# dkogan/libdogleg

Measured on AMD Instinct MI355X. Metric: trust-region steps/sec (fp64) at fixed (Nmeas,Nstate,nnz), higher is better.
Workload: dtype f64

## Files before the change

### include/dlg_backend.h

```cpp
#ifndef DLG_BACKEND_H
#define DLG_BACKEND_H

#include <stddef.h>

#ifdef __cplusplus
extern "C" {
#endif

typedef struct dlg_backend dlg_backend_t;

enum
{
  DLG_OK           = 0,
  DLG_ERR_HIP      = 1,
  DLG_ERR_ARG      = 2,
  DLG_ERR_STATE    = 3,
  DLG_ERR_NOMEM    = 4,
  DLG_ERR_NODEVICE = 5,
  DLG_ERR_COMM     = 6
};

enum { DLG_DENSE = 0, DLG_SPARSE = 1, DLG_DENSE_PRODUCTS = 2 };
enum { DLG_FLAG_JTJ_PACKED = 1, DLG_FLAG_JTJ_UPPER = 2 };
enum { DLG_KIND_CAUCHY_TO_EDGE = 0, DLG_KIND_GAUSSNEWTON = 1, DLG_KIND_INTERPOLATED = 2 };
// ... 15 lines not shown

typedef int (*dlg_allreduce_fn)(void* buf, size_t count, void* cookie);
int  dlg_backend_set_shard(dlg_backend_t* b, int row0, int row1,
                           dlg_allreduce_fn fn, void* cookie);
int  dlg_backend_set_allreduce(dlg_backend_t* b, dlg_allreduce_fn fn, void* cookie);
int  dlg_backend_set_partition(dlg_backend_t* b, int rank, int nranks);
int  dlg_partition_rows(dlg_backend_t* b, int* nrows, const int** rows);
int  dlg_point_gather_device(dlg_backend_t* b, int slot, const double* x_full_dev, const double* J_full_dev,
                             const int* colptr_host);
int  dlg_partition_stats(dlg_backend_t* b, long* stats, int nstats);
int  dlg_sparse_partition_probe(int N, int M, const int* colptr, const int* rowidx, int rank, int nranks,
                                long* stats, int nstats, char* row_owner);
int  dlg_rccl_unique_id(void* out128);
int  dlg_backend_init_rccl(dlg_backend_t* b, int rank, int nranks, const void* unique_id128);
int  dlg_backend_set_rccl(dlg_backend_t* b, void* nccl_comm);
int  dlg_backend_share_rccl(dlg_backend_t* b, dlg_backend_t* owner);
int  dlg_backend_comm_size(dlg_backend_t* b, int* nranks);
int  dlg_backend_has_rccl(dlg_backend_t* b);
int  dlg_backend_set_noop_comm(dlg_backend_t* b, int on);

int  dlg_run_steps(dlg_backend_t* b, int from, int to, int nsteps, int ncopy, const double* const* x_dev,
                   const double* const* J_dev, int first_copy, double trustregion, double lambda0,
                   double* out9, int* kind_out);

int  dlg_backend_reset(dlg_backend_t* b);
int  dlg_backend_device(dlg_backend_t* b);
int  dlg_sparse_pattern_matches(dlg_backend_t* b, const int* colptr, const int* rowidx);
int  dlg_sparse_drop_pattern(dlg_backend_t* b);

int  dlg_sparse_set_pattern(dlg_backend_t* b, const int* colptr, const int* rowidx);
int  dlg_sparse_stats(dlg_backend_t* b, long* nnz_JtJ_lower, long* nnz_L,
                      int* n_supernodes, int* n_levels, double* factor_flops);

int  dlg_sparse_region_probe(int N, int M, const int* colptr, const int* rowidx, int ncu, long* stats, int nstats);

int  dlg_sparse_schedule(dlg_backend_t* b, int* n_levels, int* persist_level0, int* persist_items);

int  dlg_sparse_symbolic_probe(int N, int M, const int* colptr, const int* rowidx, int row0,
                               int row1, long* stats, int nstats, int* perm_out);

int  dlg_point_set_p(dlg_backend_t* b, int slot, const double* p_host);
int  dlg_point_upload(dlg_backend_t* b, int slot, const double* x_host,
                      const double* J_host);
int  dlg_point_upload_products(dlg_backend_t* b, int slot, double norm2x,
                               const double* Jtx_host, const double* JtJ_host);
int  dlg_point_bind_device(dlg_backend_t* b, int slot, const double* x_dev,
                           const double* J_dev);
int  dlg_point_eval(dlg_backend_t* b, int slot, double* norm2_x, double* Jtx_absmax);
int  dlg_backend_set_speculation(dlg_backend_t* b, int on);
typedef void (*dlg_between_fn)(void* cookie);
int  dlg_backend_set_between(dlg_backend_t* b, dlg_between_fn fn, void* cookie);
int  dlg_backend_between_redone(dlg_backend_t* b);
int  dlg_point_eval_early(dlg_backend_t* b, int slot, const double* x_dev, const double* J_dev, int* done);
int  dlg_backend_set_defer_tail(dlg_backend_t* b, int on);
int  dlg_step_tail_pending(dlg_backend_t* b);
int  dlg_backend_ei_source(dlg_backend_t* b, int* from_solved_system, double* pivot_ratio);
int  dlg_step_tail(dlg_backend_t* b, double* expected_improvement);
int  dlg_backend_time_allreduce(dlg_backend_t* b, size_t count, int iters, double* us_each);

int  dlg_cauchy(dlg_backend_t* b, int slot, double* norm2_updateCauchy);

int  dlg_factorize(dlg_backend_t* b, int slot, double lambda, int* ok);

int  dlg_solve_gn(dlg_backend_t* b, int slot, double* norm2_updateGN);

int  dlg_gauss_newton(dlg_backend_t* b, int slot, double* lambda_io, double* norm2_updateGN);
// ... 92 lines not shown
```

### libdogleg_amd/capi.py

```python
import ctypes as C
import os
import numpy as np

from .ctypes_defs import (Parameters2, CholmodSparse, Trace, TraceBuffer, BatchResult, JacobianReport, JacobianEntry,
                          CB_SPARSE, CB_DENSE, CB_PRODUCTS, dptr, iptr)

HERE = os.path.dirname(os.path.abspath(__file__))
LIB_PATH = os.environ.get("DLG_TEST_LIB") or os.path.join(HERE, "libdogleg_amd.so")

DLG_OK = 0
DLG_DENSE, DLG_SPARSE, DLG_DENSE_PRODUCTS = 0, 1, 2
FLAG_PACKED, FLAG_UPPER = 1, 2
KIND_CAUCHY, KIND_GN, KIND_INTERP = 0, 1, 2
VEC_P, VEC_X, VEC_JTX, VEC_CAUCHY, VEC_GN, VEC_STEP, VEC_J, VEC_X_OWN, VEC_J_OWN = range(9)

ALLREDUCE_FN = C.CFUNCTYPE(C.c_int, C.c_void_p, C.c_size_t, C.c_void_p)

BACKEND_SYMBOLS = [
    "dlg_last_error", "dlg_device_count", "dlg_backend_create", "dlg_backend_destroy",
    "dlg_backend_set_stream", "dlg_backend_get_stream", "dlg_backend_set_shard",
    "dlg_sparse_set_pattern", "dlg_sparse_stats", "dlg_sparse_schedule", "dlg_point_set_p", "dlg_point_upload",
    "dlg_point_upload_products", "dlg_point_bind_device", "dlg_point_eval", "dlg_cauchy",
    "dlg_factorize", "dlg_solve_gn", "dlg_gauss_newton", "dlg_cauchy_gauss_newton", "dlg_make_step",
    "dlg_expected_improvement", "dlg_step", "dlg_take_step", "dlg_solve_with_factor",
    "dlg_point_download", "dlg_factor_download_dense", "dlg_point_device_ptr",
    "dlg_kernel_syrk_lower", "dlg_kernel_potrf_lower", "dlg_probe_mfma_f64", "dlg_probe_mfma_f64_clock", "dlg_probe_mfma_f64_waves",
    "dlg_probe_hbm_copy", "dlg_set_trace", "dlg_mem_alloc", "dlg_mem_free", "dlg_host_alloc",
    "dlg_host_free", "dlg_mem_upload",
    "dlg_mem_download", "dlg_mem_zero", "dlg_device_sync", "dlg_sparse_symbolic_probe",
    "dlg_backend_set_profiling", "dlg_backend_get_profile", "dlg_backend_get_profile_early",
    "dlg_backend_set_allreduce", "dlg_backend_set_partition", "dlg_partition_rows", "dlg_partition_stats",
    "dlg_sparse_partition_probe", "dlg_rccl_unique_id", "dlg_backend_init_rccl", "dlg_backend_set_rccl",
    "dlg_backend_comm_size", "dlg_backend_has_rccl", "dlg_backend_set_noop_comm", "dlg_solve_multi", "dlg_pseudoinverse_chunk", "dlg_backend_set_speculation", "dlg_backend_set_defer_tail", "dlg_step_tail",
    "dlg_step_tail_pending", "dlg_backend_ei_source", "dlg_backend_set_between", "dlg_backend_between_redone", "dlg_point_eval_early",
    "dlg_backend_share_rccl", "dlg_point_gather_device", "dlg_backend_reset", "dlg_backend_device",
    "dlg_sparse_pattern_matches", "dlg_sparse_drop_pattern", "dlg_sparse_region_probe", "dlg_run_steps", "dlg_backend_time_allreduce",
    "dlg_feature_leverage", "dlg_outlierness_factors", "dlg_leverage_query", "dlg_leverage_stats",
    "dlg_covariance_blocks", "dlg_marginal_variances", "dlg_covariance_stats", "dlg_covariance_plan_seconds",
    "dlg_covariance_plan_probe", "dlg_covariance_entries", "dlg_covariance_entries_stats", "dlg_covariance_entries_probe",
    "dlg_query_covariance", "dlg_query_covariance_stats", "dlg_query_covariance_plan_seconds", "dlg_query_covariance_plan_probe",
]
PROF_NAMES = ["K1_jtx", "K3K8_norm2Jv", "K4_kernel", "K4_total", "K5_factor", "K6_solve", "K7_step", "vec"]
DOGLEG_SYMBOLS = [
    "dogleg_getDefaultParameters", "dogleg_setMaxIterations",
    "dogleg_setTrustregionUpdateParameters", "dogleg_setDebug", "dogleg_setInitialTrustregion",
    "dogleg_setThresholds", "dogleg_optimize", "dogleg_optimize2", "dogleg_optimize_dense",
    "dogleg_optimize_dense2", "dogleg_optimize_dense_products", "dogleg_computeJtJfactorization",
    "dogleg_freeContext", "dogleg_testGradient", "dogleg_testGradient_dense",
    "dogleg_testGradient_dense_products",
    "dogleg_optimize_device2", "dogleg_amd_backend", "dogleg_amd_point_slot",
    "dogleg_amd_set_communicator", "dogleg_amd_set_allreduce", "dogleg_amd_clear_communicator",
    "dogleg_amd_rccl_unique_id", "dogleg_amd_rank", "dogleg_amd_release_cache",
    "dogleg_amd_id_file_publish", "dogleg_amd_id_file_wait", "dogleg_amd_last_solve_timing",
    "dogleg_getOutliernessFactors", "dogleg_markOutliers", "dogleg_reportOutliers",
    "dogleg_getOutliernessTrace_newFeature_sparse",
    "dogleg_amd_covariance_blocks", "dogleg_amd_marginal_variances", "dogleg_amd_covariance_entries",
    "dogleg_amd_query_covariance",
    "dogleg_amd_optimize_dense_batch", "dogleg_amd_batch_last_stats",
    "dogleg_amd_dense_batch_uncertainty", "dogleg_amd_batch_uncertainty_last_stats",
    "dogleg_amd_jacobian_colouring", "dogleg_amd_check_jacobian_device", "dogleg_amd_check_jacobian_device_batch",
    "dogleg_amd_testGradient_device", "dogleg_amd_check_jacobian_last_stats",
]

_lib = None


class DlgError(RuntimeError):
    pass


def lib():
    global _lib
    if _lib is not None:
# ... 99 lines not shown
    L.dogleg_getDefaultParameters.restype = None
    L.dogleg_optimize2.restype = C.c_double
    L.dogleg_optimize2.argtypes = [D, C.c_uint, C.c_uint, C.c_uint, V, V, PP, V]
    L.dogleg_optimize.restype = C.c_double
    L.dogleg_optimize.argtypes = [D, C.c_uint, C.c_uint, C.c_uint, V, V, V]
    L.dogleg_optimize_dense2.restype = C.c_double
    L.dogleg_optimize_dense2.argtypes = [D, C.c_uint, C.c_uint, V, V, PP, V]
    L.dogleg_optimize_dense.restype = C.c_double
    L.dogleg_optimize_dense.argtypes = [D, C.c_uint, C.c_uint, V, V, V]
    L.dogleg_optimize_dense_products.restype = C.c_double
    L.dogleg_optimize_dense_products.argtypes = [D, C.c_uint, V, V, PP, V]
    L.dogleg_freeContext.argtypes = [V]
    L.dogleg_freeContext.restype = None
    L.dogleg_optimize_device2.restype = C.c_double
    L.dogleg_optimize_device2.argtypes = [D, C.c_uint, C.c_uint, C.c_uint, I, I, V, V, PP, V]
    L.dogleg_amd_backend.restype = V
    L.dogleg_amd_backend.argtypes = [V]
    L.dogleg_amd_point_slot.restype = C.c_int
    L.dogleg_amd_point_slot.argtypes = [V, V]
    L.dogleg_amd_set_communicator.argtypes = [C.c_int, C.c_int, C.c_int, V]
    L.dogleg_amd_set_allreduce.argtypes = [C.c_int, C.c_int, C.c_int, V, V]
    L.dogleg_amd_clear_communicator.restype = None
    L.dogleg_amd_rccl_unique_id.argtypes = [V]
    L.dogleg_amd_rank.argtypes = [V, I]
    L.dogleg_amd_id_file_publish.argtypes = [C.c_char_p, V, C.c_char_p]
    L.dogleg_amd_id_file_wait.argtypes = [C.c_char_p, V, C.c_char_p, C.c_int]
    L.dlg_backend_share_rccl.argtypes = [V, V]
    L.dlg_sparse_region_probe.argtypes = [C.c_int, C.c_int, I, I, C.c_int, C.POINTER(C.c_long), C.c_int]
    L.dlg_run_steps.argtypes = [V, C.c_int, C.c_int, C.c_int, C.c_int, C.POINTER(V), C.POINTER(V), C.c_int, C.c_double, C.c_double, D, I]
    L.dlg_backend_reset.argtypes = [V]
    L.dlg_backend_device.argtypes = [V]
    L.dlg_sparse_pattern_matches.argtypes = [V, I, I]
    L.dlg_sparse_drop_pattern.argtypes = [V]
    L.dogleg_amd_release_cache.restype = None
    if hasattr(L, "dogleg_amd_optimize_dense_batch"):
        L.dogleg_amd_optimize_dense_batch.argtypes = [D, C.c_uint, C.c_uint, C.c_uint, V, V, PP, C.POINTER(BatchResult)]
        L.dogleg_amd_batch_last_stats.argtypes = [D, C.c_int]
    if hasattr(L, "dogleg_amd_dense_batch_uncertainty"):
        L.dogleg_amd_dense_batch_uncertainty.argtypes = [D, C.c_uint, C.c_uint, C.c_uint, V, V, D, D, D, D, D, C.c_int, I]
        L.dogleg_amd_batch_uncertainty_last_stats.argtypes = [D, C.c_int]
    if hasattr(L, "dogleg_amd_check_jacobian_device"):
        JR, JE = C.POINTER(JacobianReport), C.POINTER(JacobianEntry)
        L.dogleg_amd_jacobian_colouring.argtypes = [C.c_uint, C.c_uint, I, I, I]
        L.dogleg_amd_check_jacobian_device.argtypes = [D, C.c_uint, C.c_uint, C.c_uint, I, I, V, V, C.c_double, C.c_double,
                                                       C.c_double, C.c_int, JR, D, JE, C.c_int]
        L.dogleg_amd_check_jacobian_device_batch.argtypes = [D, C.c_uint, C.c_uint, C.c_uint, V, V, C.c_double, C.c_double,
                                                             C.c_double, JR, JE, C.c_int, C.POINTER(C.c_longlong)]
        L.dogleg_amd_testGradient_device.argtypes = [C.c_uint, D, C.c_uint, C.c_uint, C.c_uint, I, I, V, V]
        L.dogleg_amd_testGradient_device.restype = None
        L.dogleg_amd_check_jacobian_last_stats.argtypes = [D, C.c_int]
    L.dogleg_amd_last_solve_timing.argtypes = [D, I]
    L.dlg_point_gather_device.argtypes = [V, C.c_int, V, V, I]
    L.dogleg_setMaxIterations.argtypes = [C.c_int]
    L.dogleg_setDebug.argtypes = [C.c_int]
    L.dogleg_setInitialTrustregion.argtypes = [C.c_double]
    L.dogleg_setThresholds.argtypes = [C.c_double, C.c_double, C.c_double]
    L.dogleg_setTrustregionUpdateParameters.argtypes = [C.c_double] * 4
    _lib = L
    return L


def _ck(rc, what=""):
    if rc != DLG_OK:
        raise DlgError(f"{what} failed (code {rc}): {lib().dlg_last_error().decode()}")


# ... 165 lines not shown

def symbolic_probe(N, M, Jp, Ji, row0=0, row1=None, want_perm=False):
    L = lib()
    Jp = np.ascontiguousarray(Jp, dtype=np.int32)
    Ji = np.ascontiguousarray(Ji, dtype=np.int32)
    st = (C.c_long * len(SYM_STAT_NAMES))()
    perm = np.zeros(N, dtype=np.int32) if want_perm else None
    _ck(L.dlg_sparse_symbolic_probe(N, M, iptr(Jp), iptr(Ji), row0, M if row1 is None else row1,
                                    st, len(SYM_STAT_NAMES), iptr(perm) if want_perm else None),
        "symbolic probe")
    d = {k: st[i] for i, k in enumerate(SYM_STAT_NAMES)}
    return (d, perm) if want_perm else d


PART_STAT_NAMES = ["cut_level", "supernodes_above_cut", "supernodes_mine", "rows_mine", "reduced_doubles",
                   "panel_doubles", "nnz_mine"]


def partition_probe(N, M, Jp, Ji, rank, nranks):
    L = lib()
    Jp = np.ascontiguousarray(Jp, dtype=np.int32)
    Ji = np.ascontiguousarray(Ji, dtype=np.int32)
    st = (C.c_long * len(PART_STAT_NAMES))()
    own = np.zeros(M, dtype=np.uint8)
    _ck(L.dlg_sparse_partition_probe(N, M, iptr(Jp), iptr(Ji), rank, nranks, st, len(PART_STAT_NAMES),
                                     own.ctypes.data_as(C.c_char_p)), "partition probe")
    return {k: st[i] for i, k in enumerate(PART_STAT_NAMES)}, own.astype(bool)


REGION_STAT_NAMES = ["level0", "supernodes", "workgroups", "lds_bytes", "sliced_workgroups", "hbm_update_matrices",
                     "schedule_hash", "level_params_hash"]


def region_probe(N, M, Jp, Ji, ncu=256):
    L = lib()
    Jp = np.ascontiguousarray(Jp, dtype=np.int32)
    Ji = np.ascontiguousarray(Ji, dtype=np.int32)
    st = (C.c_long * len(REGION_STAT_NAMES))()
    _ck(L.dlg_sparse_region_probe(N, M, iptr(Jp), iptr(Ji), ncu, st, len(REGION_STAT_NAMES)), "region probe")
    return {k: (st[i] & (2**64 - 1) if k.endswith("_hash") else st[i]) for i, k in enumerate(REGION_STAT_NAMES)}


def rccl_unique_id():
    buf = (C.c_char * 128)()
    _ck(lib().dlg_rccl_unique_id(C.cast(buf, C.c_void_p)), "rccl_unique_id")
    return bytes(buf)


class DeviceArray:

    def __init__(self, arr=None, nbytes=None, dtype=np.float64):
        L = lib()
        if arr is not None:
            arr = np.ascontiguousarray(arr)
            nbytes, dtype = arr.nbytes, arr.dtype
        self.nbytes, self.dtype = nbytes, np.dtype(dtype)
        self.ptr = L.dlg_mem_alloc(nbytes)
        if not self.ptr:
            raise DlgError(L.dlg_last_error().decode())
        if arr is not None:
            _ck(L.dlg_mem_upload(self.ptr, arr.ctypes.data, nbytes), "upload")
        else:
            _ck(L.dlg_mem_zero(self.ptr, nbytes), "memset")

    def numpy(self, shape=None):
        out = np.zeros(self.nbytes // self.dtype.itemsize, dtype=self.dtype)
# ... 99 lines not shown
        rows = C.POINTER(C.c_int)()
        _ck(self.L.dlg_partition_rows(self.h, C.byref(n), C.byref(rows)), "partition_rows")
        return np.ctypeslib.as_array(rows, shape=(n.value,)).copy() if n.value else np.zeros(0, dtype=np.int32)

    def partition_stats(self):
        st = (C.c_long * len(PART_STAT_NAMES))()
        _ck(self.L.dlg_partition_stats(self.h, st, len(PART_STAT_NAMES)), "partition_stats")
        return {k: st[i] for i, k in enumerate(PART_STAT_NAMES)}

    def init_rccl(self, rank, nranks, unique_id):
        buf = C.create_string_buffer(unique_id, 128)
        _ck(self.L.dlg_backend_init_rccl(self.h, rank, nranks, C.cast(buf, C.c_void_p)), "init_rccl")

    def set_noop_comm(self, on=True):
        _ck(self.L.dlg_backend_set_noop_comm(self.h, 1 if on else 0), "set_noop_comm")

    def comm_size(self):
        n = C.c_int()
        _ck(self.L.dlg_backend_comm_size(self.h, C.byref(n)), "comm_size")
        return n.value

    def set_pattern(self, Jp, Ji):
        Jp = np.ascontiguousarray(Jp, dtype=np.int32)
        Ji = np.ascontiguousarray(Ji, dtype=np.int32)
        _ck(self.L.dlg_sparse_set_pattern(self.h, iptr(Jp), iptr(Ji)), "set_pattern")

    def stats(self):
        a, b = C.c_long(), C.c_long()
        c, d = C.c_int(), C.c_int()
        e = C.c_double()
        _ck(self.L.dlg_sparse_stats(self.h, C.byref(a), C.byref(b), C.byref(c), C.byref(d), C.byref(e)),
            "stats")
        return dict(nnz_JtJ_lower=a.value, nnz_L=b.value, n_supernodes=c.value, n_levels=d.value,
                    factor_flops=e.value)

    def schedule(self):
        a, b, c = C.c_int(), C.c_int(), C.c_int()
        _ck(self.L.dlg_sparse_schedule(self.h, C.byref(a), C.byref(b), C.byref(c)), "schedule")
        return dict(n_levels=a.value, persist_level0=b.value, persist_items=c.value)

    def set_p(self, slot, p):
        p = np.ascontiguousarray(p, dtype=np.float64)
        _ck(self.L.dlg_point_set_p(self.h, slot, dptr(p)), "set_p")

    def upload(self, slot, x, J):
        x = np.ascontiguousarray(x, dtype=np.float64)
        J = np.ascontiguousarray(J, dtype=np.float64)
        self._keep = [x, J]
        _ck(self.L.dlg_point_upload(self.h, slot, dptr(x), dptr(J)), "upload")

    def upload_products(self, slot, norm2x, Jtx, JtJ):
        Jtx = np.ascontiguousarray(Jtx, dtype=np.float64)
        JtJ = np.ascontiguousarray(JtJ, dtype=np.float64)
        self._keep = [Jtx, JtJ]
        _ck(self.L.dlg_point_upload_products(self.h, slot, norm2x, dptr(Jtx), dptr(JtJ)), "upload")

    def bind_device(self, slot, x_ptr, J_ptr):
        _ck(self.L.dlg_point_bind_device(self.h, slot, C.c_void_p(x_ptr), C.c_void_p(J_ptr)), "bind")

    def eval(self, slot):
        a, b = C.c_double(), C.c_double()
        _ck(self.L.dlg_point_eval(self.h, slot, C.byref(a), C.byref(b)), "eval")
        return a.value, b.value

    def cauchy(self, slot):
        a = C.c_double()
        _ck(self.L.dlg_cauchy(self.h, slot, C.byref(a)), "cauchy")
# ... 204 lines not shown
```

### libdogleg_amd/csrc/panel_factor.h

```cpp
#pragma once
#include <hip/hip_runtime.h>

#ifndef DLG_PF_STAMP
#define DLG_PF_DECL
#define DLG_PF_STAMP(i)
#define DLG_PF_PIN(x)
#define DLG_PF_DONE
#endif
#ifndef DLG_PF_EVT
#define DLG_PF_EVT(J, e)
#endif
#ifndef DLG_PF_WLOG
#define DLG_PF_WLOG(J, t, e)
#endif

__device__ __forceinline__ double dlg_rsqrt(double d)
{
  double y = __builtin_amdgcn_rsq(d);
  y = y*(1.5 - 0.5*d*y*y);
  y = y*(1.5 - 0.5*d*y*y);
  return y;
}

typedef double dlg_pf_v4d __attribute__((ext_vector_type(4)));
// ... 976 lines not shown
      case 2: badcol = bd_factor_member<2>(P, ldp, c0, rdiag); break;
      case 3: badcol = bd_factor_member<3>(P, ldp, c0, rdiag); break;
      case 4: badcol = bd_factor_member<4>(P, ldp, c0, rdiag); break;
      case 5: badcol = bd_factor_member<5>(P, ldp, c0, rdiag); break;
      case 6: badcol = bd_factor_member<6>(P, ldp, c0, rdiag); break;
      case 7: badcol = bd_factor_member<7>(P, ldp, c0, rdiag); break;
      default: badcol = bd_factor_member<8>(P, ldp, c0, rdiag); break;
    }
    if(badcol >= 0) atomicMin(info, col0 + c0 + badcol);
  }
  __syncthreads();
  for(int r = w + tid; r < nrows; r += NT)
  {
    for(int m = 0; m < nmem; m++)
    {
      const int c0 = mcol[m], nb = mcol[m+1] - c0;
      switch(nb)
      {
        case 1: bd_solve_row<1>(P, ldp, r, c0, rdiag); break;
        case 2: bd_solve_row<2>(P, ldp, r, c0, rdiag); break;
        case 3: bd_solve_row<3>(P, ldp, r, c0, rdiag); break;
        case 4: bd_solve_row<4>(P, ldp, r, c0, rdiag); break;
        case 5: bd_solve_row<5>(P, ldp, r, c0, rdiag); break;
        case 6: bd_solve_row<6>(P, ldp, r, c0, rdiag); break;
        case 7: bd_solve_row<7>(P, ldp, r, c0, rdiag); break;
        default: bd_solve_row<8>(P, ldp, r, c0, rdiag); break;
      }
    }
  }
  __syncthreads();
}

template <int NB, int DS = 8>
__device__ __forceinline__ int bd_factor_member_g(double* __restrict__ G, int ldg, int c0, double* rdiag,
                                                  double* __restrict__ Dg)
{
  double D[NB][NB];
#pragma unroll
  for(int c = 0; c < NB; c++)
#pragma unroll
    for(int q = 0; q <= c; q++) D[c][q] = G[(c0 + c) + (size_t)(c0 + q)*ldg];
  int badcol = -1;
#pragma unroll
  for(int c = 0; c < NB; c++)
  {
    double d = D[c][c];
    if(!(d > 0.0)) { if(badcol < 0) badcol = c; d = 1.0; }
    const double inv = dlg_rsqrt(d);
    rdiag[c0 + c] = inv;
#pragma unroll
    for(int i = c + 1; i < NB; i++) D[i][c] *= inv;
#pragma unroll
    for(int j = c + 1; j < NB; j++)
#pragma unroll
      for(int i = j; i < NB; i++) D[i][j] -= D[i][c]*D[j][c];
    D[c][c] = d*inv;
  }
#pragma unroll
  for(int c = 0; c < NB; c++)
#pragma unroll
    for(int q = 0; q <= c; q++) { G[(c0 + c) + (size_t)(c0 + q)*ldg] = D[c][q]; if(q < DS) Dg[(c0 + c)*DS + q] = D[c][q]; }
  return badcol;
}
template <int NB, int DS = 8>
__device__ __forceinline__ void bd_solve_row_c(double* Pb, int ldp, int r, int c0, const double* rdiag,
                                               const double* __restrict__ Dg)
{
  double x[NB], Lm[NB][NB], rd[NB];
#pragma unroll
  for(int c = 0; c < NB; c++)
  {
    x[c] = Pb[r + (c0 + c)*ldp]; rd[c] = rdiag[c0 + c];
#pragma unroll
    for(int q = 0; q < c; q++) Lm[c][q] = Dg[(c0 + c)*DS + q];
  }
#pragma unroll
  for(int c = 0; c < NB; c++)
  {
    double v = x[c];
#pragma unroll
    for(int q = 0; q < c; q++) v -= x[q]*Lm[c][q];
    x[c] = v*rd[c];
  }
#pragma unroll
  for(int c = 0; c < NB; c++) Pb[r + (c0 + c)*ldp] = x[c];
}
template <int NT, int DS = 8>
__device__ __forceinline__ void bd_compact_members(double* __restrict__ G, int ldg, int w, int tid,
                                                   const int* __restrict__ mcol_g, int nmem, int bdw,
                                                   int* mcol, double* rdiag, double* __restrict__ Dg,
                                                   int* __restrict__ info, int col0)
{
  for(int m = tid; m <= nmem; m += NT) mcol[m] = (m < nmem) ? (bdw > 0 ? m*bdw : mcol_g[m]) : w;
  for(int m = tid; m < nmem; m += NT)
  {
    const int c0 = bdw > 0 ? m*bdw : mcol_g[m];
    const int nb = (m + 1 < nmem ? (bdw > 0 ? (m + 1)*bdw : mcol_g[m + 1]) : w) - c0;
    int badcol;
    switch(nb)
    {
      case 1: badcol = bd_factor_member_g<1, DS>(G, ldg, c0, rdiag, Dg); break;
      case 2: badcol = bd_factor_member_g<2, DS>(G, ldg, c0, rdiag, Dg); break;
      case 3: badcol = bd_factor_member_g<3, DS>(G, ldg, c0, rdiag, Dg); break;
      case 4: badcol = bd_factor_member_g<4, DS>(G, ldg, c0, rdiag, Dg); break;
      case 5: badcol = bd_factor_member_g<5, DS>(G, ldg, c0, rdiag, Dg); break;
      case 6: badcol = bd_factor_member_g<6, DS>(G, ldg, c0, rdiag, Dg); break;
      case 7: badcol = bd_factor_member_g<7, DS>(G, ldg, c0, rdiag, Dg); break;
      default: badcol = bd_factor_member_g<8, DS>(G, ldg, c0, rdiag, Dg); break;
    }
    if(badcol >= 0) atomicMin(info, col0 + c0 + badcol);
  }
}
template <int NT, int NB, int DS>
__device__ __forceinline__ void bd_compact_rows_flat(double* Pb, int ldp, int nr, int w, int tid, int nmem,
                                                     const double* rdiag, const double* __restrict__ Dg)
{
  const int q = NT / nr, rem = NT - q*nr;
  int m = tid / nr, r = tid - m*nr;
  while(m < nmem)
  {
    bd_solve_row_c<NB, DS>(Pb, ldp, w + r, m*NB, rdiag, Dg);
    r += rem; m += q;
    if(r >= nr) { r -= nr; m++; }
  }
}
template <int NT, int DS = 8>
__device__ __forceinline__ void bd_compact_rows(double* Pb, int ldp, int nrows, int w, int tid, int nmem,
                                                const int* mcol, const double* rdiag, const double* __restrict__ Dg, int bdw = 0)
{
#ifndef DLG_BD_ROWS_BY_THREAD
  if(bdw > 0 && bdw <= 4 && w == nmem*bdw && nrows > w)
  {
    const int nr = nrows - w;
    switch(bdw)
    {
      case 1: bd_compact_rows_flat<NT, 1, DS>(Pb, ldp, nr, w, tid, nmem, rdiag, Dg); break;
      case 2: bd_compact_rows_flat<NT, 2, DS>(Pb, ldp, nr, w, tid, nmem, rdiag, Dg); break;
      case 3: bd_compact_rows_flat<NT, 3, DS>(Pb, ldp, nr, w, tid, nmem, rdiag, Dg); break;
      default: bd_compact_rows_flat<NT, 4, DS>(Pb, ldp, nr, w, tid, nmem, rdiag, Dg); break;
    }
    __syncthreads();
// ... 25 lines not shown
```

### libdogleg_amd/csrc/sparse_factor.hip

```cpp
#include "sparse_internal.h"
#include "panel_factor.h"
#include "factor_tail.h"

namespace {
#ifdef DLG_FL_PROFILE
constexpr int FL_PROF_WG = 4096;
__device__ long long g_fl_prof[32*FL_PROF_WG*8];
__device__ long long g_fl_add[FL_PROF_WG*4];
#define FL_ADD_STAMP(k) do { if(HANDOFF && threadIdx.x == 0 && blockIdx.x < FL_PROF_WG) g_fl_add[blockIdx.x*4 + (k)] = wall_clock64(); } while(0)
#define FL_STAMP(k) do { if(threadIdx.x == 0 && blockIdx.x < FL_PROF_WG) g_fl_prof[((prof_lvl & 31)*FL_PROF_WG + blockIdx.x)*8 + (k)] = wall_clock64(); } while(0)
#else
#define FL_STAMP(k)
#define FL_ADD_STAMP(k)
#endif

template <int NT, bool UT_LDS, bool HANDOFF = false>
__device__ __forceinline__ void mf_add_children(double* P, double* Wt, int ntri, int nch, int ch0,
                                                MfChild rc, const MfChild* __restrict__ mf_rec,
                                                const double* uscr, const uint16_t* __restrict__ mf_dst, int tid,
                                                int* pr_flag = nullptr, int pr_epoch = 0, DlgHandoff ho = DlgHandoff{nullptr, 0, 0}, int z0 = 0)
{
  constexpr int MF_SLOTS = (NT >= 512) ? 20 : 16;
  const int lane = tid & 63;
  for(int e = z0 + tid; e < ntri; e += NT) Wt[e] = 0.0;
// ... 170 lines not shown
  FL_ADD_STAMP(1);
#ifdef DLG_FL_PROFILE
  if(threadIdx.x == 0 && blockIdx.x < FL_PROF_WG) g_fl_add[blockIdx.x*4 + 3] = 1000 + (bup ? 1 : 0) + 10*cnB + 100*(fl[0] == want);
#endif
  if(!bup) wait_flags(ciB, cnB);
  __syncthreads();
  FL_ADD_STAMP(2);
  if(!bup) load_child(WB, npB, bX, bY);
  add_half(dB, npB, 0, bX); add_half(dB, npB, H, bY);
  __syncthreads();
}

template <int NT, bool LEAF = false>
__global__ void __launch_bounds__(NT, LEAF ? 4 : 1) k_factor_level(const FwItem* __restrict__ items,
                                                     const MfChild* __restrict__ mf_rec,
                                                     const int* __restrict__ sn_bd_col,
                                                     const uint16_t* __restrict__ mf_dst,
                                                     double* __restrict__ Lx,
                                                     double* __restrict__ top_scr,
                                                     int* __restrict__ info,
                                                     double* uscr, int mode,
                                                     int* pr_flag, int pr_epoch, DlgHandoff ho, int64_t pr_acc)
{
  extern __shared__ __attribute__((aligned(16))) double P[];
  __shared__ int sbad, s_skip;
  constexpr int DS = LEAF ? 4 : 8;
  constexpr int CP_FLIGHT = LEAF ? 16 : 32;
#ifdef DLG_FL_PROFILE
  const int prof_lvl = mode >> 8;
  FL_STAMP(0);
#endif
  const bool stage_leaf_u = (mode & 4) != 0;
  const bool b16 = (mode & 16) != 0;
  mode &= 3;
  const FwItem it = items[blockIdx.x];
  const int r0 = it.r0, w = it.w, nrows = it.nrows;
  double* G = Lx + it.lx;
  const int tid = threadIdx.x, lane = tid & 63;
  const int nloc = w + (it.r1 - r0);
  const int shift = r0;
  const int64_t top = it.top;
  const int mb = nloc - w, ntri = mb*(mb + 1)/2;
  const bool cmp = it.nbd > 0 && top < 0;
  const int ldp = cmp ? ((mb + 1) & ~1) : ((nloc + 1) & ~1);
  double* Pb = cmp ? P - w : P;
  const int row0c = cmp ? w : 0;
  const bool has_u = mode != 0 && top < 0;
  const bool sliced = !LEAF && it.sliced != 0;
  const bool u_lds = has_u && (sliced || ((it.nch > 0 || stage_leaf_u) &&
                     (cmp ? (size_t)(ldp*w + ntri + 1 + DS*w)*sizeof(double) <= (size_t)FAC_LDS_BUDGET : it.jsp >= 0)));
  const int usp = (u_lds && !cmp && !sliced) ? it.jsp : mb;
  const int sl_pad = sliced ? (it.eA & 1) : 0;
  const int nlin = sliced ? it.eB - it.eA + sl_pad : usp*mb - usp*(usp - 1)/2;
  double* Ug = has_u ? uscr + it.u_off : nullptr;
  double* Us = P + ldp*w;
  const int ush = sliced ? sl_pad - it.eA : 0;
  double* Dg = Us + (u_lds ? nlin + 1 : 0);
  __shared__ int s_mcol[LEAF ? 68 : 260];
  __shared__ double s_rdiag[LEAF ? 64 : 256];
  MfChild rc = {0, 0, 0, 0};
  const bool mf_acc = !LEAF && mode == 2 && it.nch > 0;
  if(mf_acc) rc = mf_rec[it.ch0 + min(lane, it.nch - 1)];
  if(tid == 0) { sbad = 0x7fffffff; s_skip = __hip_atomic_load(info, __ATOMIC_RELAXED, __HIP_MEMORY_SCOPE_AGENT) != 0x7fffffff; }
  if(pr_flag && tid == 0 && blockIdx.x == gridDim.x - 1)
    __hip_atomic_store(pr_flag + gridDim.x, pr_epoch, __ATOMIC_RELAXED, __HIP_MEMORY_SCOPE_AGENT);
  if(cmp)
  {
    __syncthreads();
    if(s_skip)
    {
      if(pr_flag && tid == 0) __hip_atomic_store(pr_flag + blockIdx.x, pr_epoch, __ATOMIC_RELAXED, __HIP_MEMORY_SCOPE_AGENT);
      return;
    }
    bd_compact_members<NT, DS>(G, nrows, w, tid, sn_bd_col + it.bd0, it.nbd, it.bdw, s_mcol, s_rdiag, Dg, &sbad, it.col0);
  }
  const int cp_rows = min(NT, (nloc - row0c + 63) & ~63), cp_ng = NT/cp_rows, cp_g = tid/cp_rows;
#ifndef DLG_LEAF_NO_GLDS
  if((LEAF && cmp) || (!LEAF && !cmp && !sliced && shift == 0))
  {
    const int ntot = ldp*w;
    const double* g0 = cmp ? G + (w + shift) : G;
    for(int k = tid >> 6; 128*k < ntot; k += NT/64)
    {
      const int e = 128*k + 2*lane;
      if(e < ntot)
      {
        const int j = e / ldp, r = e - j*ldp;
        __builtin_amdgcn_global_load_lds((const __attribute__((address_space(1))) void*)(g0 + (size_t)j*nrows + r),
                                         (__attribute__((address_space(3))) void*)(P + 128*k), 16, 0, 0);
      }
    }
  }
  else
#endif
  {
  for(int i = row0c + tid - cp_g*cp_rows; i < nloc && cp_g < cp_ng; i += cp_rows)
  {
    const double* gp = G + (i < w ? i : i + shift);
    for(int j0 = cp_g; j0 < w; j0 += CP_FLIGHT*cp_ng)
    {
      double v[CP_FLIGHT];
#pragma unroll
      for(int u = 0; u < CP_FLIGHT; u++) v[u] = (j0 + u*cp_ng < w) ? gp[(size_t)(j0 + u*cp_ng)*nrows] : 0.0;
#pragma unroll
      for(int u = 0; u < CP_FLIGHT; u++) if(j0 + u*cp_ng < w) Pb[i + (j0 + u*cp_ng)*ldp] = v[u];
    }
  }
  }
  __syncthreads();
  FL_STAMP(1);
  const int nrep = (pr_flag && it.rsv2 > 1) ? it.rsv2 : 1;
  if(nrep > 1 && it.rep < nrep - 1 && tid == 0) __hip_atomic_store(pr_flag + blockIdx.x, -pr_epoch, __ATOMIC_RELAXED, __HIP_MEMORY_SCOPE_AGENT);
  if(s_skip)
  {
    if(pr_flag && tid == 0) __hip_atomic_store(pr_flag + blockIdx.x, pr_epoch, __ATOMIC_RELAXED, __HIP_MEMORY_SCOPE_AGENT);
    return;
  }
  if(mf_acc && usp < mb)
    for(int jw = usp + (tid >> 6); jw < mb; jw += NT/64)
      for(int i = lane; i < mb - jw; i += 64) P[(mb - jw)*ldp + i] = 0.0;
  if(mf_acc)
  {
    const bool two = NT >= 512 && it.nch == 2 && __builtin_amdgcn_readlane(rc.npad, 0) <= 20*NT && __builtin_amdgcn_readlane(rc.npad, 1) <= 20*NT &&
                     (__builtin_amdgcn_readlane(rc.rsv, 0) >> 20) <= 8 && (__builtin_amdgcn_readlane(rc.rsv, 1) >> 20) <= 8;
    if(pr_flag && u_lds && two) mf_add_two_pipelined<NT>(P, Us, nlin, rc, uscr, mf_dst, tid, pr_flag, pr_epoch, ho);
    else if(pr_flag && u_lds) mf_add_children<NT, true, true>(P, Us, nlin, it.nch, it.ch0, rc, mf_rec, uscr, mf_dst, tid, pr_flag, pr_epoch, ho);
    else if(pr_flag)     mf_add_children<NT, false, true>(P, Ug + pr_acc, (nrep > 1 && !sliced) ? it.eB : ntri, it.nch, it.ch0, rc, mf_rec, uscr, mf_dst, tid, pr_flag, pr_epoch, ho,
                                                          (nrep > 1 && !sliced) ? it.eA : 0);
    else if(u_lds)  mf_add_children<NT, true >(P, Us, nlin, it.nch, it.ch0, rc, mf_rec, uscr, mf_dst, tid);
    else            mf_add_children<NT, false>(P, Ug, ntri, it.nch, it.ch0, rc, mf_rec, uscr, mf_dst, tid);
  }
  FL_STAMP(2);
  if(cmp) bd_compact_rows<NT, DS>(Pb, ldp, nloc, w, tid, it.nbd, s_mcol, s_rdiag, Dg, it.bdw);
  else if(LEAF) { }
  else if(it.nbd > 0) panel_factor_blockdiag<NT>(P, ldp, nloc, w, tid, sn_bd_col + it.bd0, it.nbd, &sbad, it.col0, s_mcol, s_rdiag);
  else if(NT >= 256 && b16 && nloc <= 16*PF_B16_MAXT) panel_factor_b16<(NT >= 256 ? NT : 256)>(P, ldp, nloc, w, tid, &sbad, it.col0);
// ... 59 lines not shown
      for(int i = lane; i < mb - jw; i += 64)
      {
        if(pr_flag) __hip_atomic_store((gwptr_t)(dst + i), src[i], __ATOMIC_RELAXED, __HIP_MEMORY_SCOPE_AGENT);
        else dst[i] = src[i];
      }
    }
  }
  if(pr_flag)
  {
    asm volatile("s_waitcnt vmcnt(0)" ::: "memory");
    __syncthreads();
    if(tid == 0) __hip_atomic_store(pr_flag + blockIdx.x, pr_epoch, __ATOMIC_RELAXED, __HIP_MEMORY_SCOPE_AGENT);
  }
  FL_STAMP(7);
  const bool store_panel = it.rep == nrep - 1;
  if(nrep > 1 && store_panel)
  {
    if(tid < nrep - 1)
    {
      int spins = 0;
      for(;;)
      {
        const int v = __hip_atomic_load(pr_flag + ((int)blockIdx.x - (nrep - 1) + tid), __ATOMIC_RELAXED, __HIP_MEMORY_SCOPE_AGENT);
        if(v == pr_epoch || v == -pr_epoch) break;
        __builtin_amdgcn_s_sleep(1);
        if(++spins > ho.spins) { atomicOr(ho.status, DLG_HANDOFF_FACTOR); break; }
      }
    }
    __syncthreads();
  }
  for(int i = row0c + tid - cp_g*cp_rows; i < nloc && cp_g < cp_ng && store_panel; i += cp_rows)
  {
    double* gp; size_t gs;
    if(i >= w)        { gp = G + (i + shift); gs = (size_t)nrows; }
    else if(top < 0)  { gp = G + i; gs = (size_t)nrows; }
    else if(r0 == 0)  { gp = top_scr + top + i; gs = (size_t)w; }
    else continue;
    const int jend = (usp < mb && i < w) ? i + 1 : w;
    for(int j0 = cp_g; j0 < jend; j0 += 16*cp_ng)
    {
      double v[16];
#pragma unroll
      for(int u = 0; u < 16; u++) v[u] = (j0 + u*cp_ng < jend) ? Pb[i + (j0 + u*cp_ng)*ldp] : 0.0;
#pragma unroll
      for(int u = 0; u < 16; u++) if(j0 + u*cp_ng < jend) gp[(size_t)(j0 + u*cp_ng)*gs] = v[u];
    }
  }
  FL_STAMP(5);
#ifdef DLG_FL_PROFILE
  if(threadIdx.x == 0 && blockIdx.x < FL_PROF_WG)
    g_fl_prof[((prof_lvl & 31)*FL_PROF_WG + blockIdx.x)*8 + 6] = (long long)w | ((long long)nrows << 12) | ((long long)it.nch << 24) | ((long long)(u_lds ? 1 : 0) << 36) | ((long long)(has_u ? 1 : 0) << 37) | ((long long)(it.r1 - it.r0) << 40) | ((long long)(it.rep & 15) << 52) | ((long long)(it.pad & 63) << 56);
#endif
}
__global__ void __launch_bounds__(TPB) k_copy_top(const int* __restrict__ ms_sn, const int* __restrict__ sn_c0,
                                                  const int* __restrict__ sn_rowptr,
                                                  const int64_t* __restrict__ sn_lx,
                                                  const int64_t* __restrict__ sn_top,
                                                  double* __restrict__ Lx,
                                                  const double* __restrict__ top_scr, const int* __restrict__ info)
{
  if(*info != 0x7fffffff) return;
  const int s = ms_sn[blockIdx.x];
  const int w = sn_c0[s+1] - sn_c0[s];
  const int nrows = sn_rowptr[s+1] - sn_rowptr[s];
  double* G = Lx + sn_lx[s];
  const double* T = top_scr + sn_top[s];
  for(int e = threadIdx.x; e < w*w; e += TPB) { const int j = e / w, i = e - j*w; G[i + (size_t)j*nrows] = T[e]; }
// ... 590 lines not shown
    }
    if(nwg == 0) continue;
    for(int g = FL_PROF_WG - 1, shown = 0; g >= 0 && shown < (getenv("DLG_FL_DUMP_ALL") ? FL_PROF_WG : 20); g--)
    {
      const long long* q = &h[(l*FL_PROF_WG + g)*8];
      if(q[5] == 0 || q[7] == 0) continue;
      shown++;
      {
        std::vector<long long> ha(FL_PROF_WG*4);
        static bool got = false; static std::vector<long long> hadd;
        if(!got) { hadd.resize(FL_PROF_WG*4); hipMemcpyFromSymbol(hadd.data(), HIP_SYMBOL(g_fl_add), sizeof(long long)*hadd.size()); got = true; }
        if(hadd[g*4 + 0]) fprintf(stderr, "   add %3d: child0 seen %6lld child0 added %6lld last child seen %6lld dbg %lld\n", g, hadd[g*4] - t0, hadd[g*4 + 1] - t0, hadd[g*4 + 2] - t0, hadd[g*4 + 3]);
      }
      fprintf(stderr, "   wg %3d (w %3lld rows %4lld nch %lld u_lds %lld lvl %lld rep %lld): start %6lld flag up %6lld panel in %6lld added %6lld factored %6lld tail %6lld flag+stored %6lld\n",
              g, q[6] & 4095, (q[6] >> 12) & 4095, (q[6] >> 24) & 4095, (q[6] >> 36) & 1, (q[6] >> 56) & 63, (q[6] >> 52) & 15, q[0] - t0, q[7] - t0, q[1] - t0, q[2] - t0, q[3] - t0, q[4] - t0, q[5] - t0);
    }
    const long long* q = &h[(l*FL_PROF_WG + last)*8];
    fprintf(stderr, "level %2d: %3d wg, span %7lld | last wg %3d (w %3lld rows %4lld slice %4lld nch %2lld u_lds %lld has_u %lld): start +%6lld load %6lld add %6lld factor %6lld tail %6lld store %6lld | mean: load %6.0f add %6.0f factor %6.0f tail %6.0f store %6.0f\n",
            l, nwg, tend - t0, last, q[6] & 4095, (q[6] >> 12) & 4095, (q[6] >> 40) & 4095, (q[6] >> 24) & 4095, (q[6] >> 36) & 1, (q[6] >> 37) & 1,
            q[0] - t0, q[1] - q[0], q[2] - q[1], q[3] - q[2], q[4] - q[3], q[5] - q[4],
            mean[0]/nwg, mean[1]/nwg, mean[2]/nwg, mean[3]/nwg, mean[4]/nwg);
  }
  std::vector<long long> z(h.size(), 0);
  hipMemcpyToSymbol(HIP_SYMBOL(g_fl_prof), z.data(), sizeof(long long)*z.size());
}
#endif
int sparse_factor_levels(dlg_backend* b, int part)
{
  SparseSym* Y = b->sym;
  const SymHost& H = Y->H;
  hipStream_t st = b->stream;
  const bool split = Y->top.level0 > 0 && H.nlevels >= 2 && H.part_nranks <= 1 && H.fw_lvl_ptr[1] > H.fw_lvl_ptr[0];
  if(part == 2 && !split) return DLG_OK;
  if(part != 2)
  {
  if(H.part_nranks > 1 && H.cut_level < 0) DLG_CHECK(sparse_partition_reduce(b));
  if(Y->top.level0 == 0 || H.nlevels < 2) DLG_CHECK(sparse_fin_side_gate(b));
  }
  for(int l = 0; l < H.nlevels; l++)
  {
    const bool launched_before = part == 2 && l == 0;

    const int n = H.fw_lvl_ptr[l+1] - H.fw_lvl_ptr[l];
    const bool gate_here = (l == Y->top.level0 && Y->top.flag) || (l == Y->lo.level0 && Y->lo.flag);
    if(l > 0 && n < 256 && !gate_here) dlg_fork_point(b);
    if(l == Y->lo.level0 && Y->lo.flag)
    {
      PrRegion& R = Y->lo;
      ++R.epoch;
      if(l > 0 && n < 256) dlg_fork_gate(b, R.flag + R.nwg, R.epoch);
      {
        DlgRegionTurn turn(b);
        launch_region(b, R, l);
      }
      l = R.level1;
      if(H.part_nranks > 1 && l == H.cut_level) { DLG_LAUNCH_CHECK(); DLG_CHECK(sparse_partition_reduce(b)); }
      continue;
    }
    if(l == Y->top.level0)
    {
      PrRegion& R = Y->top;
      ++R.epoch;
      if(gate_here && l > 0) dlg_fork_gate(b, R.flag + R.nwg, R.epoch);
      DlgRegionTurn turn(b);
      launch_region(b, R, l);
      break;
    }
    if(n > 0 && !launched_before)
    {
      const int fmode = ((l >= H.mf_level0) ? 2 : Y->fac.syrk_fused[l]) + 4*Y->fac.stage[l] + FMODE_B16 + 256*(l & 31);
      launch_factor_level(Y->fac.nt[l], Y->fac.leaf[l], n, Y->fac.lds[l], st, Y, Y->fw_item + H.fw_lvl_ptr[l], Y->mf_rec, Y->mf_dst,
                          fmode, (int*)nullptr, 0, DlgHandoff{nullptr, 0, 0}, (int64_t)0);
    }
    if(part == 1 && split && l == 0) { Y->fac_pending = true; DLG_LAUNCH_CHECK(); return DLG_OK; }
    const int nu = H.uw_lvl_ptr[l+1] - H.uw_lvl_ptr[l];
    const bool gather_next = nu > 0 && H.upd_syrk[l] && Y->fac.upd_nw[l] > 0;
    const int fin_ep = (l == 0 && gather_next) ? Y->fin_side_owed : 0;
    if(fin_ep) Y->fin_side_owed = 0;
    if(l == 0) DLG_CHECK(sparse_fin_side_gate(b));
    if(gather_next)
    {
      const int ns = H.xl_ptr[l+1] - H.xl_ptr[l];
      if(Y->fac.syrk_fused[l] || ns == 0) {  }
      else if(Y->fac.syrk_nt[l] == 256)
        hipLaunchKernelGGL(HIP_KERNEL_NAME(k_update_syrk<256>), dim3(ns), dim3(256), Y->fac.syrk_lds[l], st,
                           Y->xl_sn + H.xl_ptr[l], Y->sn_c0, Y->sn_rowptr, Y->sn_lx, Y->u_off, Y->Lx, Y->uscr,
                           Y->fac.syrk_kc[l]);
      else
        hipLaunchKernelGGL(HIP_KERNEL_NAME(k_update_syrk<1024>), dim3(ns), dim3(1024), Y->fac.syrk_lds[l], st,
                           Y->xl_sn + H.xl_ptr[l], Y->sn_c0, Y->sn_rowptr, Y->sn_lx, Y->u_off, Y->Lx, Y->uscr,
                           Y->fac.syrk_kc[l]);
      hipLaunchKernelGGL(HIP_KERNEL_NAME(k_update_gather<TPB>), dim3(nu), dim3(TPB), Y->fac.upd_lds[l], st, H.uw_lvl_ptr[l],
                         Y->uw_flat, Y->usub, Y->usub_u, Y->relpos, Y->Lx, Y->upart, Y->uscr,
                         Y->fac.upd_nw[l], Y->d_info,
                         fin_ep ? (const int*)(Y->fin_flag + 1) : (const int*)nullptr, fin_ep,
                         reinterpret_cast<int*>(b->d_scal + (dlg_backend::NSCAL - 2)));
    }
    else if(nu > 0 && Y->fac.upd_coop[l] == 2)
      hipLaunchKernelGGL(k_update_mfma, dim3(nu), dim3(TPB), Y->fac.upd_lds[l], st, H.uw_lvl_ptr[l],
                         Y->uw_item, Y->uw_s0, Y->uw_s1, Y->uw_part, Y->ui_t, Y->ui_col, Y->ui_nc,
                         Y->usub, Y->relpos, Y->sn_rowptr, Y->sn_lx, Y->Lx, Y->upart, Y->fac.upd_nw[l], (const int*)Y->d_info);
    else if(nu > 0 && Y->fac.upd_coop[l])
      hipLaunchKernelGGL(k_update_coop, dim3(nu), dim3(TPB), 0, st, H.uw_lvl_ptr[l],
                         Y->uw_item, Y->uw_s0, Y->uw_s1, Y->uw_part, Y->ui_t, Y->ui_col, Y->ui_nc,
                         Y->usub, Y->relpos, Y->sn_rowptr, Y->sn_lx, Y->Lx, Y->upart, (const int*)Y->d_info);
    else if(nu > 0)
      hipLaunchKernelGGL(k_update_level, dim3(nu), dim3(TPB), Y->fac.upd_lds[l], st, H.uw_lvl_ptr[l],
                         Y->uw_item, Y->uw_s0, Y->uw_s1, Y->uw_part, Y->ui_t, Y->ui_col, Y->ui_nc,
                         Y->usub, Y->relpos, Y->sn_rowptr, Y->sn_lx, Y->Lx, Y->upart, Y->fac.upd_nw[l], (const int*)Y->d_info);
// ... 31 lines not shown
```

### libdogleg_amd/csrc/sparse_host.hip

```cpp
#include "sparse_internal.h"
#include <thread>
#include <mutex>
#include <memory>
#include <string>
#include <algorithm>
#include <cstring>
#include <chrono>

int sparse_create(dlg_backend* b) { (void)b; return DLG_OK; }

size_t sparse_local_nnz(const dlg_backend* b) { return b->sym ? b->sym->nnz_loc : (size_t)b->nnz; }

void sparse_destroy(dlg_backend* b)
{
  SparseSym* Y = b->sym;
  if(!Y) return;
  if(b->aux_stream) (void)hipStreamSynchronize(b->aux_stream);
  if(Y->ev_spec) (void)hipEventDestroy(Y->ev_spec);
  if(Y->ev_spec_fork) (void)hipEventDestroy(Y->ev_spec_fork);
  for(void* p : Y->allocs) if(p) (void)hipFree(p);
  sparse_leverage_free(Y);
  if(b->cov) { if(b->stream) (void)hipStreamSynchronize(b->stream); for(int i = 0; i < COV_NPLAN; i++) cov_plan_release(b->cov[i]); }
  b->cov_last = -1;
  selinv_release(b);
// ... 106 lines not shown
  {
    key = pattern_key(b, colptr, rowidx);
    Y->pat_key = key;
    std::lock_guard<std::mutex> lk(g_sym_mu);
    const SymCacheEntry* c = g_sym_cache.get();
    if(c && c->key == key && c->N == b->N && c->M == b->M && c->nnz == b->nnz && c->row0 == b->row0 && c->row1 == b->row1 &&
       c->part_rank == b->part_rank && c->part_nranks == b->part_nranks &&
       !memcmp(c->cp.data(), colptr, sizeof(int)*((size_t)b->M + 1)) && !memcmp(c->ri.data(), rowidx, sizeof(int)*(size_t)b->nnz))
    { Y->H = c->H; cached = true; }
  }
  if(!cached)
  {
    if(sym_analyze(Y->H, b->N, b->M, colptr, rowidx, b->row0, b->row1, err, sizeof(err), b->part_rank, b->part_nranks))
    { dlg_set_error("symbolic analysis: %s", err); return DLG_ERR_ARG; }
    if(use_cache)
    {
      std::unique_ptr<SymCacheEntry> e(new (std::nothrow) SymCacheEntry());
      if(e)
      {
        e->key = key; e->N = b->N; e->M = b->M; e->nnz = b->nnz; e->row0 = b->row0; e->row1 = b->row1;
        e->part_rank = b->part_rank; e->part_nranks = b->part_nranks;
        e->cp.assign(colptr, colptr + b->M + 1); e->ri.assign(rowidx, rowidx + b->nnz);
        e->H = Y->H;
        std::lock_guard<std::mutex> lk(g_sym_mu);
        g_sym_cache = std::move(e);
      }
    }
  }
  SymHost& H = Y->H;
  lap(cached ? "symbolic analysis (copied: same pattern as the last one)" : "symbolic analysis (host)");
  const bool partition = H.part_nranks > 1;
  if(partition) b->mloc = (int)H.part_rows.size();
  UP(sn_c0); UP(sn_rowptr); UP(sn_rows); UP(sn_scr); UP(lvl_sn); UP(sn_lx); UP(diagpos);
  UP(ui_t); UP(ui_col); UP(ui_nc); UP(ui_ptr); UP(usub); UP(relpos); UP(u_off); UP(usub_u); UP(fw_item); UP(mf_rec); UP(mf_dst);
  UP(uw_item); UP(uw_s0); UP(uw_s1); UP(uw_part); UP(uf_item); UP(uf_n); UP(uf_off);
  UP(oblk); UP(contrib); UP(jtx_task); UP(jtx_fin_ptr); UP(jtx_fin_blk);
  UP(asm_rho); UP(asm_pair); UP(asm_slot); UP(asm_batch); UP(asm_ctask); UP(asm_cfin);
  if(H.asm_jtx_ok)
  {
    UP(jf_ptr); UP(jf_ent); UP(jf_var0); UP(jf_w); UP(jf_short);
    {
      std::vector<int> rec(4*H.jf_long.size());
      for(size_t k = 0; k < H.jf_long.size(); k++)
      { const int v = H.jf_long[k]; rec[4*k] = H.jf_ptr[v]; rec[4*k+1] = H.jf_ptr[v+1]; rec[4*k+2] = H.jf_var0[v]; rec[4*k+3] = H.jf_w[v]; }
      DLG_CHECK(upload(Y->jf_long, rec)); Y->allocs.push_back(Y->jf_long);
      const size_t nl = std::max<size_t>(1, H.jf_long.size());
      DLG_HIP(hipMalloc(&Y->jf_lpart, sizeof(double)*16*JFL_SEG*nl)); Y->allocs.push_back(Y->jf_lpart);
      DLG_HIP(hipMalloc(&Y->jf_lcnt, sizeof(int)*nl)); Y->allocs.push_back(Y->jf_lcnt);
      DLG_HIP(hipMemset(Y->jf_lcnt, 0, sizeof(int)*nl));
    }
    DLG_HIP(hipMalloc(&Y->jtp, sizeof(double)*16*std::max<size_t>(1, H.asm_mtask.size()))); Y->allocs.push_back(Y->jtp);
  }
  UP(asm_shape); UP(asm_kg); UP(asm_mtask); UP(asm_tdest); UP(asm_fin2); UP(asm_fin2_list); UP(asm_run); UP(asm_pdest);
  {
    std::vector<uint32_t> pent(128*std::max<size_t>(1, H.asm_shape.size()), 0u);
    Y->asm_pent_ok = true;
    for(size_t q = 0; q < H.asm_shape.size(); q++)
    {
      const AsmShape& sh = H.asm_shape[q];
      std::vector<uint32_t> e;
      bool fits = true;
      auto word = [&](int kind, int mm, int n) {
        if(sh.pa[mm] > 15 || sh.pnI[mm] > 15 || sh.pslot[mm] > 15) fits = false;
        return (uint32_t)kind | (uint32_t)mm << 2 | (uint32_t)n << 6 | (uint32_t)(sh.pslot[mm] & 15) << 10 | (uint32_t)(sh.pa[mm] & 15) << 14 |
               (uint32_t)sh.paccoff[mm] << 18 | (uint32_t)(sh.pnI[mm] & 15) << 26 |
               (uint32_t)((sh.pslot[mm] == sh.dslot && sh.pa[mm] < n) ? 1u : 0u) << 30; };
// ... 30 lines not shown
      for(int s2 = 0; s2 < H.nsn; s2++)
      {
        const bool keep = H.sn_level[s2] == 0 && H.sn_bd_ptr[s2+1] > H.sn_bd_ptr[s2] && H.sn_top[s2] < 0 && H.nlevels >= 2;
        if(keep) { kept += H.sn_lx[s2+1] - H.sn_lx[s2]; continue; }
        if(!off.empty() && off.back() + len.back() == H.sn_lx[s2]) len.back() += H.sn_lx[s2+1] - H.sn_lx[s2];
        else { off.push_back(H.sn_lx[s2]); len.push_back(H.sn_lx[s2+1] - H.sn_lx[s2]); }
      }
      if(!off.empty() && off.back() + len.back() == H.lx_size) len.back() += 8;
      else { off.push_back(H.lx_size); len.push_back(8); }
      Y->n_clr = (int)off.size();
      Y->clr_partial_ok = kept*2 > H.lx_size && Y->n_clr <= 65535 && H.asm_cfin.empty() && H.asm_ctask.empty() && !getenv("DOGLEG_AMD_FULL_CLEAR");
      DLG_CHECK(upload(Y->clr_off, off)); Y->allocs.push_back(Y->clr_off);
      DLG_CHECK(upload(Y->clr_len, len)); Y->allocs.push_back(Y->clr_len);
    }
    {
      std::vector<int64_t> dp; std::vector<int> dc;
      for(int k = 0; k < H.N; k++) if(H.sn_level[H.col_sn[k]] == 0) { dp.push_back(H.diagpos[k]); dc.push_back(k); }
      Y->n_leaf_diag = (int)dp.size();
      if(Y->n_leaf_diag > 0)
      {
        DLG_CHECK(upload(Y->leaf_diag, dp)); Y->allocs.push_back(Y->leaf_diag);
        DLG_CHECK(upload(Y->leaf_diag_col, dc)); Y->allocs.push_back(Y->leaf_diag_col);
      }
    }
    DLG_HIP(hipMalloc(&Y->fin_flag, sizeof(int)*2)); Y->allocs.push_back(Y->fin_flag);
    DLG_HIP(hipMemsetAsync(Y->fin_flag, 0, sizeof(int)*2, b->stream));
  }
  UP(rl_ptr); UP(rl_pos); UP(perm); UP(col_sn); UP(sn_owner); UP(xl_sn); UP(fw_sn); UP(fw_r0); UP(fw_r1); UP(ms_sn); UP(sn_top); UP(sn_bd_ptr); UP(sn_bd_col);
  {
    std::vector<int64_t> ap((size_t)H.N);
    for(int k = 0; k < H.N; k++)
    {
      const int s2 = H.col_sn[k];
      const int64_t nrows = H.sn_rowptr[s2+1] - H.sn_rowptr[s2];
      ap[k] = H.sn_lx[s2] + (nrows - 1) + (int64_t)(k - H.sn_c0[s2])*nrows;
    }
    DLG_CHECK(upload(Y->augpos, ap)); Y->allocs.push_back(Y->augpos);
    std::vector<int64_t> av((size_t)H.N);
    for(int k = 0; k < H.N; k++) av[(size_t)H.perm[k]] = ap[k];
    std::vector<char> listed((size_t)H.N, 0);
    for(int pass = 0; pass < 2; pass++)
      for(int v : (pass ? H.jf_long : H.jf_short))
        for(int q = 0; q < H.jf_w[v]; q++) listed[(size_t)H.jf_var0[v] + q] = 1;
    DLG_CHECK(upload(Y->aug_of_var, av)); Y->allocs.push_back(Y->aug_of_var);
    DLG_CHECK(upload(Y->jf_listed, listed)); Y->allocs.push_back(Y->jf_listed);
  }
  {
    std::vector<int> fs, fl;
    for(int f = 0; f + 1 < (int)H.jtx_fin_ptr.size(); f++)
      (H.jtx_fin_ptr[f+1] - H.jtx_fin_ptr[f] > 256 ? fl : fs).push_back(f);
    Y->n_fin_short = (int)fs.size(); Y->n_fin_long = (int)fl.size();
    DLG_CHECK(upload(Y->jtx_fin_short, fs)); Y->allocs.push_back(Y->jtx_fin_short);
    DLG_CHECK(upload(Y->jtx_fin_long, fl)); Y->allocs.push_back(Y->jtx_fin_long);
  }
  {
    const int mloc = dlg_mloc(b);
    std::vector<int> jp(mloc + 1), ji;
    if(partition)
    {
      jp[0] = 0;
      for(int k = 0; k < mloc; k++) { const int r = H.part_rows[k]; jp[k+1] = jp[k] + (colptr[r+1] - colptr[r]); }
      ji.resize((size_t)jp[mloc]);
      for(int k = 0; k < mloc; k++) { const int r = H.part_rows[k]; memcpy(&ji[jp[k]], rowidx + colptr[r], sizeof(int)*(size_t)(colptr[r+1] - colptr[r])); }
      Y->nnz_loc = (size_t)jp[mloc];
    }
    else
    {
      const int q0 = colptr[b->row0], q1 = colptr[b->row1];
// ... 240 lines not shown
      (void)sparse_note_breakdown(b);
      b->factor_doomed = true;
      *ok = 0;
      return DLG_OK;
    }
  }
  DLG_CHECK(sparse_factor_levels(b, b->factor_ahead ? 1 : 0));
  if(pf.e) { dlg_prof_end(b, pf.id, pf.e); pf.e = nullptr; }
  if(b->defer_factor_sync) { *ok = 1; return DLG_OK; }
  DLG_HIP(hipMemcpyAsync(Y->h_info, Y->d_info, sizeof(int), hipMemcpyDeviceToHost, st));
  DLG_HIP(hipStreamSynchronize(st));
  *ok = sparse_factor_ok(b);
  return DLG_OK;
}
bool sparse_factor_pending(const dlg_backend* b) { return b->sym && b->sym->fac_pending; }
int sparse_norm2_chunks(const dlg_backend* b) { return b->sym ? b->sym->n_nv_chunks : 0; }
int sparse_factorize_rest(dlg_backend* b, bool* was_pending)
{
  SparseSym* Y = b->sym;
  *was_pending = Y && Y->fac_pending;
  if(!*was_pending) return DLG_OK;
  Y->fac_pending = false;
  b->prof_cont = true;
  struct Cont { dlg_backend* b; ~Cont() { b->prof_cont = false; } } cont{b};
  DlgProfScope pf(b, DLG_PROF_K5_FACTOR);
  return sparse_factor_levels(b, 2);
}
double sparse_current_lambda(const dlg_backend* b) { return b->sym ? b->sym->cur_lambda : 0.0; }
const double* sparse_pivot_minmax(const dlg_backend* b, int* n)
{
  *n = b->sym ? b->sym->n_diag_mm : 0;
  return (b->sym && b->sym->n_diag_mm > 0) ? b->sym->diag_mm : nullptr;
}
void sparse_hold_factor(dlg_backend* b)
{
  SparseSym* Y = b->sym;
  Y->held_Lx = Y->Lx; Y->held_aug = Y->aug_rhs; Y->held_lambda = Y->cur_lambda;
}
void sparse_release_held(dlg_backend* b) { if(b->sym) b->sym->held_Lx = nullptr; }
int sparse_restore_factor(dlg_backend* b, bool* restored, bool rearm)
{
  SparseSym* Y = b->sym;
  *restored = false;
  Y->fac_pending = false;
  if(!Y->held_Lx || Y->held_Lx != Y->Lx_spec) { Y->held_Lx = nullptr; return DLG_OK; }
  std::swap(Y->Lx, Y->Lx_spec);
  Y->spare_zeroed = false; Y->spare_dirty = true;
  Y->aug_rhs = Y->held_aug; Y->cur_lambda = Y->held_lambda; Y->held_Lx = nullptr;
  static const int k_armed = 0x7fffffff;
  if(rearm) DLG_HIP(hipMemcpyAsync(Y->d_info, &k_armed, sizeof(int), hipMemcpyHostToDevice, b->stream));
  Y->info_clean = false; Y->info_armed = false;
  *restored = true;
  return DLG_OK;
}
bool sparse_factor_ok(const dlg_backend* b) { return *b->sym->h_info == 0x7fffffff; }
namespace { __global__ void k_lower_word(int* word, int v) { if(threadIdx.x == 0) __hip_atomic_store(word, v, __ATOMIC_RELAXED, __HIP_MEMORY_SCOPE_AGENT); } }
int sparse_abandon_enqueued(dlg_backend* b)
{
  SparseSym* Y = b->sym;
  if(!Y || !Y->d_info || !b->copy_stream || !b->ev_copy) return DLG_OK;
  hipLaunchKernelGGL(k_lower_word, dim3(1), dim3(64), 0, b->copy_stream, Y->d_info, 0);
  DLG_LAUNCH_CHECK();
  DLG_HIP(hipEventRecord(b->ev_copy, b->copy_stream));
  DLG_HIP(hipStreamWaitEvent(b->stream, b->ev_copy, 0));
  hipLaunchKernelGGL(k_lower_word, dim3(1), dim3(64), 0, b->stream, Y->d_info, 0x7fffffff);
  DLG_LAUNCH_CHECK();
  Y->info_clean = false; Y->info_armed = false; Y->fac_pending = false;
  return DLG_OK;
}

extern "C" int dlg_sparse_symbolic_probe(int N, int M, const int* colptr, const int* rowidx, int row0,
                                         int row1, long* stats, int nstats, int* perm_out)
{
  SymHost H;
  char err[512];
  if(sym_analyze(H, N, M, colptr, rowidx, row0, row1, err, sizeof(err)))
  { dlg_set_error("symbolic analysis: %s", err); return DLG_ERR_ARG; }
  const long v[] = { (long)H.nvb, (long)H.nsn, (long)H.nlevels, (long)H.nnz_JtJ_lower, (long)H.nnz_L,
                     (long)H.lx_size, (long)H.factor_flops, (long)H.max_panel, (long)H.asm_ctask.size(),
                     (long)H.ui_t.size(), (long)H.relpos.size(), (long)H.oblk.size(),
                     (long)H.contrib.size(), (long)H.usub.size(), (long)H.scr_size,
                     (long)H.jtx_task.size(), (long)H.asm_mtask.size(), (long)H.asm_kg.size(),
                     (long)H.asm_shape.size() };
  if(getenv("DOGLEG_AMD_SYM_DEBUG"))
    for(int l = 0; l + 1 < (int)H.uw_lvl_ptr.size(); l++)
    {
      long nu = 0, direct = 0, part = 0, subs = 0;
      for(int u = H.uw_lvl_ptr[l]; u < H.uw_lvl_ptr[l+1]; u++)
      {
        const int item = H.uw_item[u], t = H.ui_t[item];
        const long slab = (long)(H.sn_rowptr[t+1] - H.sn_rowptr[t])*H.ui_nc[item];
        nu++; subs += H.uw_s1[u] - H.uw_s0[u];
        (H.uw_part[u] < 0 ? direct : part) += slab;
      }
      if(nu) fprintf(stderr, "update level %d: %ld units, %ld sub-tasks, slabs applied directly %ld doubles, partial slabs %ld doubles, U scratch %ld doubles, two-phase %d\n",
                     l, nu, subs, direct, part, (long)H.uscr_size, (int)H.upd_syrk[l]);
    }
  for(int i = 0; i < nstats && i < (int)(sizeof(v)/sizeof(v[0])); i++) stats[i] = v[i];
  if(perm_out) memcpy(perm_out, H.perm.data(), sizeof(int)*(size_t)N);
  return DLG_OK;
// ... 2 lines not shown
```

### libdogleg_amd/csrc/sparse_internal.h

```cpp
#pragma once
#include "dlg_internal.h"
#include "sparse_symbolic.h"
#include "sparse_region.h"

namespace {
constexpr int JFL_SEG = 16;
constexpr int NV_CHUNK = 2048;

constexpr int TPB = 256;
constexpr int LDS_BUDGET = SYM_LDS_BUDGET;
constexpr int FAC_LDS_BUDGET = SYM_FAC_LDS_BUDGET;

__device__ __forceinline__ double wave_sum(double v)
{
#pragma unroll
  for(int o = 32; o > 0; o >>= 1) v += __shfl_down(v, o, 64);
  return v;
}

template <int NT, int U, class LoadF, class StoreF>
__device__ __forceinline__ void batched_copy(int total, int tid, LoadF ld, StoreF st)
{
  for(int base = 0; base < total; base += U*NT)
  {
// ... 2 lines not shown
    for(int u = 0; u < U; u++) { const int idx = base + u*NT + tid; v[u] = (idx < total) ? ld(idx) : 0.0; }
#pragma unroll
    for(int u = 0; u < U; u++) { const int idx = base + u*NT + tid; if(idx < total) st(idx, v[u]); }
  }
}

template <class T> int upload(T*& dev, const std::vector<T>& h)
{
  dev = nullptr;
  const size_t bytes = sizeof(T)*(h.size() ? h.size() : 1);
  DLG_HIP(hipMalloc(&dev, bytes));
  if(!h.empty()) DLG_HIP(hipMemcpy(dev, h.data(), sizeof(T)*h.size(), hipMemcpyHostToDevice));
  return DLG_OK;
}

}

struct GatherUnit { int64_t lt, part; int s0, s1, nrows_t, nc; };
struct SolveItem { int c0, w, nrows, rowoff; int64_t lx; int bd0, nbd; int pflag, rsv; };

struct PrRegion
{
  int level0 = 1 << 30, level1 = -1, lds = 0, stage = 0, nwg = 0;
  FwItem* item = nullptr; MfChild* rec = nullptr; uint16_t* dst = nullptr;
  int* flag = nullptr; int epoch = 0;
};

struct SparseSym
{
  SymHost H;
  uint64_t pat_key = 0;
  int *sn_c0 = nullptr, *sn_rowptr = nullptr, *sn_rows = nullptr, *sn_scr = nullptr, *lvl_sn = nullptr;
  int64_t *sn_lx = nullptr, *diagpos = nullptr;
  int *ui_t = nullptr, *ui_col = nullptr, *ui_nc = nullptr, *ui_ptr = nullptr;
  SymSub* usub = nullptr; int* relpos = nullptr;
  int *uw_item = nullptr, *uw_s0 = nullptr, *uw_s1 = nullptr, *uf_item = nullptr, *uf_n = nullptr;
  int64_t *uw_part = nullptr, *uf_off = nullptr;
  GatherUnit* uw_flat = nullptr;
  double* upart = nullptr; double* uscr = nullptr; int64_t *u_off = nullptr, *usub_u = nullptr;
  SolveItem* slv_item = nullptr; FwItem* fw_item = nullptr; MfChild* mf_rec = nullptr; uint16_t* mf_dst = nullptr;
  SymOutBlock* oblk = nullptr; SymContrib* contrib = nullptr;
  SymTask *jtx_task = nullptr;
  int *jtx_fin_ptr = nullptr, *jtx_fin_blk = nullptr;
  int *jtx_fin_short = nullptr, *jtx_fin_long = nullptr; int n_fin_short = 0, n_fin_long = 0;
  AsmRho* asm_rho = nullptr; AsmPair* asm_pair = nullptr; AsmSlot* asm_slot = nullptr;
  AsmBatch* asm_batch = nullptr; AsmTask* asm_ctask = nullptr; AsmFin* asm_cfin = nullptr;
  bool asm_pent_ok = false;
  uint32_t* asm_pent = nullptr;
  AsmShape* asm_shape = nullptr; AsmKG* asm_kg = nullptr; AsmMTask* asm_mtask = nullptr; int* asm_tdest = nullptr;
  int *jf_ptr = nullptr, *jf_ent = nullptr, *jf_var0 = nullptr, *jf_w = nullptr, *jf_short = nullptr, *jf_long = nullptr;
  double* jf_lpart = nullptr; int* jf_lcnt = nullptr;
  const double* fin_pending_rhs = nullptr; const double* spec_aug_rhs = nullptr; bool info_clean = false;
  double* fin_pending_Lx = nullptr;
  bool spare_dirty = false, spare_zeroed = false; hipStream_t spare_stream = nullptr;
  double* jtp = nullptr;
  AsmFin2* asm_fin2 = nullptr; int64_t* asm_fin2_list = nullptr; AsmRun* asm_run = nullptr; int* asm_pdest = nullptr;
  int *rl_ptr = nullptr, *rl_pos = nullptr, *perm = nullptr, *col_sn = nullptr;
  int *fw_sn = nullptr, *fw_r0 = nullptr, *fw_r1 = nullptr, *ms_sn = nullptr; int64_t* sn_top = nullptr;
  int *sn_bd_ptr = nullptr, *sn_bd_col = nullptr;
  double* top_scr = nullptr;
  const double* aug_rhs = nullptr;
  int *Jp = nullptr, *Ji = nullptr;
  int *gat_rows = nullptr, *gat_src = nullptr;
  int *nv_chunk = nullptr; int n_nv_chunks = 0;
  double *Lx = nullptr, *scr = nullptr, *ywork = nullptr, *asm_part = nullptr, *jtx_part = nullptr;
  int *d_info = nullptr, *h_info = nullptr;
// ... 12 lines not shown
  int64_t* augpos = nullptr;
  int *xl_sn = nullptr;
  double* held_Lx = nullptr; const double* held_aug = nullptr; double held_lambda = 0.0;
  double cur_lambda = 0.0;
  double *ms_scr = nullptr, *ms_y = nullptr; int ms_lds_f = 0, ms_lds_b = 0;
  typedef ReachPlan LevPlan;
  LevPlan lev[2];
  int* lev_iperm = nullptr; std::vector<int> lev_jp, lev_ji; int lev_lds = 0;
  double* Lx_spec = nullptr; hipEvent_t ev_spec = nullptr, ev_spec_fork = nullptr;
  bool spec_inflight = false, spec_valid = false; int spec_slot = -1; const double* spec_J = nullptr;
  int64_t touch_off = 0, touch_n = 0;
  int bw_level0 = 1 << 30, bw_lds = 0, bw_n = 0;
  SolveItem* slv_item_pr = nullptr; int* bwd_flag = nullptr; int bwd_epoch = 0; double* bwd_xh = nullptr;
  PrRegion top, lo; double* pr_acc = nullptr;
  int64_t* clr_off = nullptr; int64_t* clr_len = nullptr; int n_clr = 0; bool clr_partial_ok = false; double* lz_ok[2] = {nullptr, nullptr};
  int64_t* aug_of_var = nullptr; char* jf_listed = nullptr;
  int aug_fused_epoch = 0; const double* spec_aug_fused = nullptr;
  int* fin_flag = nullptr; int fin_epoch = 0, fin_side_owed = 0; bool fin_side_sched_ok = false; hipStream_t fin_main = nullptr;
  int bwd_xb_cap = 12288;
  double* diag_mm = nullptr; int n_diag_mm = 0;
  std::vector<void*> allocs;
};

int sparse_assemble(dlg_backend* b, int s, double lambda);
int sparse_partition_reduce(dlg_backend* b);
int sparse_assemble_speculative(dlg_backend* b, int s);
int sparse_eval_assemble(dlg_backend* b, int s, int* done);
int sparse_assemble_finish(dlg_backend* b);
int sparse_zero_spare(dlg_backend* b, hipStream_t ordered_for);
void sparse_spec_invalidate(dlg_backend* b, int s);
int sparse_factor_setup(dlg_backend* b);
int sparse_factor_levels(dlg_backend* b, int part = 0);
int sparse_solve_setup(dlg_backend* b);
```

### libdogleg_amd/csrc/sparse_multi.hip

```cpp
#include "sparse_internal.h"
#include <algorithm>
#include <cfloat>
#include <cstdint>

namespace {
constexpr int MR = 16;
constexpr int MS_WMAX = 128;
typedef double ms_v4d __attribute__((ext_vector_type(4)));
__device__ __forceinline__ int tri(int i, int j) { return i*(i + 1)/2 + j; }

__device__ __forceinline__ void ms_stage_top(const double* __restrict__ L, int nrows, int w, double* Lt, double* dinv, int tid)
{
  for(int e = tid; e < w*w; e += TPB)
  {
    const int j = e / w, i = e - j*w;
    if(i >= j) { const double v = L[i + (size_t)j*nrows]; Lt[tri(i, j)] = v; if(i == j) dinv[j] = 1.0/v; }
  }
}

__global__ void __launch_bounds__(TPB) k_msolve_fwd_level(const int* __restrict__ lvl_sn,
                                                          const int* __restrict__ sn_c0,
                                                          const int* __restrict__ sn_rowptr,
                                                          const int64_t* __restrict__ sn_lx,
                                                          const int* __restrict__ sn_scr,
// ... 418 lines not shown
  const size_t e = (size_t)blockIdx.x*TPB + threadIdx.x;
  if(e >= (size_t)N*MR) return;
  const int k = (int)(e / MR), c = (int)(e % MR);
  il[e] = (var[(size_t)ch*MR + c] == k) ? 1.0 : 0.0;
}
__global__ void __launch_bounds__(TPB) k_cov_pick(const int* __restrict__ var, const int* __restrict__ pptr,
                                                  const int* __restrict__ prod, const int64_t* __restrict__ goff, int ch,
                                                  const double* __restrict__ X, double* __restrict__ gram)
{
  const int t = threadIdx.x, q0 = pptr[ch];
  if(t >= pptr[ch+1] - q0) return;
  const int a = prod[q0 + t] / MR, c = prod[q0 + t] % MR;
  gram[goff[ch] + t] = X[(size_t)var[(size_t)ch*MR + a]*MR + c];
}

size_t ms_lds_fwd(int w) { return sizeof(double)*(size_t)(((w*(w + 1)/2 + 1) & ~1) + ((w + 1) & ~1) + 2*w*MR); }
size_t ms_lds_bwd(int w) { return ms_lds_fwd(w) + sizeof(double)*(size_t)(w*(MS_CH + 1) + MS_CH*MR); }
}

int sparse_multi_width_ok(const dlg_backend* b)
{
  const SymHost& H = b->sym->H;
  for(int s = 0; s < H.nsn; s++) if(H.sn_c0[s+1] - H.sn_c0[s] > MS_WMAX) return 0;
  return H.part_nranks <= 1;
}
int sparse_multi_rhs() { return MR; }

int sparse_solve_multi(dlg_backend* b, double* d_il)
{
  SparseSym* Y = b->sym;
  if(!Y) { dlg_set_error("dlg_sparse_set_pattern must be called first"); return DLG_ERR_STATE; }
  const SymHost& H = Y->H;
  hipStream_t st = b->stream;
  if(!Y->ms_scr)
  {
    DLG_HIP(hipMalloc(&Y->ms_scr, sizeof(double)*((size_t)H.scr_size + 1)*MR)); Y->allocs.push_back(Y->ms_scr);
    DLG_HIP(hipMalloc(&Y->ms_y, sizeof(double)*(size_t)H.N*MR)); Y->allocs.push_back(Y->ms_y);
    int wmax = 1;
    for(int s = 0; s < H.nsn; s++) wmax = std::max(wmax, H.sn_c0[s+1] - H.sn_c0[s]);
    Y->ms_lds_f = (int)ms_lds_fwd(wmax); Y->ms_lds_b = (int)ms_lds_bwd(wmax);
    DLG_HIP(hipFuncSetAttribute(reinterpret_cast<const void*>(&k_msolve_fwd_level), hipFuncAttributeMaxDynamicSharedMemorySize, Y->ms_lds_f));
    DLG_HIP(hipFuncSetAttribute(reinterpret_cast<const void*>(&k_msolve_bwd_level), hipFuncAttributeMaxDynamicSharedMemorySize, Y->ms_lds_b));
  }
  for(int l = 0; l < H.nlevels; l++)
  {
    const int n = H.xl_ptr[l+1] - H.xl_ptr[l];
    if(n > 0)
      hipLaunchKernelGGL(k_msolve_fwd_level, dim3(n), dim3(TPB), Y->ms_lds_f, st, Y->xl_sn + H.xl_ptr[l], Y->sn_c0,
                         Y->sn_rowptr, Y->sn_lx, Y->sn_scr, Y->rl_ptr, Y->rl_pos, Y->perm, Y->Lx, d_il, Y->ms_scr, Y->ms_y);
  }
  for(int l = H.nlevels - 1; l >= 0; l--)
  {
    const int n = H.xl_ptr[l+1] - H.xl_ptr[l];
    if(n > 0)
      hipLaunchKernelGGL(k_msolve_bwd_level, dim3(n), dim3(TPB), Y->ms_lds_b, st, Y->xl_sn + H.xl_ptr[l], Y->sn_c0,
                         Y->sn_rowptr, Y->sn_rows, Y->sn_lx, Y->perm, Y->Lx, Y->ms_y, d_il);
  }
  DLG_LAUNCH_CHECK();
  return DLG_OK;
}
int multi_cols_to_interleaved(dlg_backend* b, const double* d_cols, int ncols, double* d_il)
{
  hipLaunchKernelGGL(k_cols_to_interleaved, dim3(dlg_cdiv((long)b->N*MR, TPB)), dim3(TPB), 0, b->stream, d_cols, b->N, ncols, d_il);
  DLG_LAUNCH_CHECK();
  return DLG_OK;
}
int multi_interleaved_to_cols(dlg_backend* b, const double* d_il, int ncols, double* d_cols)
{
  hipLaunchKernelGGL(k_interleaved_to_cols, dim3(dlg_cdiv((long)b->N*ncols, TPB)), dim3(TPB), 0, b->stream, d_il, b->N, ncols, d_cols);
  DLG_LAUNCH_CHECK();
  return DLG_OK;
}
int sparse_jt_chunk_interleaved(dlg_backend* b, int s, int row0, int ncols, double* d_il)
{
  SparseSym* Y = b->sym;
  DLG_HIP(hipMemsetAsync(d_il, 0, sizeof(double)*(size_t)b->N*MR, b->stream));
  hipLaunchKernelGGL(k_jt_chunk_sparse, dim3(ncols), dim3(TPB), 0, b->stream, Y->Jp, Y->Ji, b->slot[s].Jin(), row0, ncols, d_il);
  DLG_LAUNCH_CHECK();
  return DLG_OK;
}

void reach_plan_release(ReachPlan& P)
{
  for(void* q : {(void*)P.pair_sn, (void*)P.pair_ch, (void*)P.cp_ptr, (void*)P.wl, (void*)P.pair_off, (void*)P.gram, (void*)P.scr})
    if(q) (void)hipFree(q);
  P = ReachPlan();
}
namespace {
constexpr int64_t LEV_BATCH_ROWS = (int64_t)1 << 21;
// ... 93 lines not shown
  for(int c = 0; c < MR; c++) { const int x = K.var[(size_t)ch*MR + c]; if(x >= 0) st.push_back(H.col_sn[H.iperm[x]]); }
}
void query_starts(const SymHost& H, const CovPack& K, int ch, std::vector<int>& st)
{
  for(int q = K.qrp[K.crow[ch]]; q < K.qrp[K.crow[ch+1]]; q++) st.push_back(H.col_sn[H.iperm[K.qvar[q]]]);
}
template <class F> int reach_slots(dlg_backend* b, CovPlan& P, F starts)
{
  const SymHost& H = b->sym->H;
  const CovPack& K = P.K;
  DLG_CHECK(reach_setup(b));
  ReachHost R;
  reach_build(H, K.nch, [&](int ch, std::vector<int>& st) { starts(H, K, ch, st); }, R);
  DLG_CHECK(reach_upload(R, K.nch, P.R));
  std::vector<int64_t> goff(R.pair_sn.size() + 1, 0);
  for(size_t q = 0; q < R.pair_sn.size(); q++) { const int ch = R.pair_ch[q]; goff[q+1] = goff[q] + (K.pptr[ch+1] - K.pptr[ch]); }
  DLG_CHECK(upload(P.goff, goff));
  DLG_HIP(hipMalloc(&P.gram, sizeof(double)*(size_t)std::max<int64_t>(goff.back(), 1)));
  return DLG_OK;
}
int chunk_slots(CovPlan& P)
{
  const CovPack& K = P.K;
  std::vector<int> slot_ptr(K.nch + 1);
  std::vector<int64_t> goff(K.nch + 1);
  for(int ch = 0; ch <= K.nch; ch++) { slot_ptr[ch] = ch; goff[ch] = K.pptr[ch]; }
  DLG_CHECK(upload(P.slot_ptr, slot_ptr)); DLG_CHECK(upload(P.goff, goff));
  DLG_HIP(hipMalloc(&P.gram, sizeof(double)*(size_t)std::max(K.pptr.back(), 1)));
  return DLG_OK;
}
template <class Rhs> int reach_run(dlg_backend* b, CovPlan& P, const Rhs& rhs)
{
  SparseSym* Y = b->sym;
  DLG_CHECK(reach_setup(b));
  const ReachPlan& R = P.R;
  reach_for_each_level(R, Y->H.nlevels, [&](const int* wl, int n) {
    hipLaunchKernelGGL(k_cov_fwd_level<Rhs>, dim3(n), dim3(TPB), Y->lev_lds, b->stream, wl, R.pair_sn, R.pair_ch, R.pair_off,
                       R.cp_ptr, Y->sn_c0, Y->sn_rowptr, Y->sn_rows, Y->sn_lx, Y->Lx, rhs, P.pptr, P.prod, P.goff, R.scr, P.gram);
  });
  DLG_LAUNCH_CHECK();
  return DLG_OK;
}

int lev_plan_build(dlg_backend* b, int fs, int nf)
{
  SparseSym* Y = b->sym;
  const SymHost& H = Y->H;
  SparseSym::LevPlan& P = Y->lev[fs - 1];
  if(P.nf == nf) return DLG_OK;
  DLG_HIP(hipStreamSynchronize(b->stream));
  reach_plan_release(P);
  DLG_CHECK(reach_setup(b));
  const int nrow = nf*fs, nch = dlg_cdiv(nrow, MR);
  ReachHost R;
  reach_build(H, nch, [&](int ch, std::vector<int>& st) {
    for(int row = ch*MR; row < std::min(nrow, ch*MR + MR); row++)
      for(int q = Y->lev_jp[row]; q < Y->lev_jp[row+1]; q++) st.push_back(H.col_sn[H.iperm[Y->lev_ji[q]]]);
  }, R);
  DLG_CHECK(reach_upload(R, nch, P));
  DLG_HIP(hipMalloc(&P.gram, sizeof(double)*LEV_NP*(size_t)std::max(P.npair, 1)));
  P.nf = nf;
  return DLG_OK;
}

void cov_req_vars(int r0, int nr, int c0, int nc, std::vector<int>& v)
{
  v.clear();
  for(int i = 0; i < nr; i++) v.push_back(r0 + i);
  for(int j = 0; j < nc; j++) v.push_back(c0 + j);
  std::sort(v.begin(), v.end());
  v.erase(std::unique(v.begin(), v.end()), v.end());
// ... 246 lines not shown
    DLG_CHECK(reach_slots(b, P, query_starts));
    std::vector<int> pv(K.qvar.size());
    for(size_t q = 0; q < pv.size(); q++) pv[q] = H.iperm[K.qvar[q]];
    return upload(P.qvar, pv);
  }
  DLG_CHECK(upload(P.qvar, K.qvar));
  if(route == ROUTE_DENSE) DLG_CHECK(dense_cov_setup(b, P));
  return chunk_slots(P);
}
int sparse_query_reach_run(dlg_backend* b, CovPlan& P) { return reach_run(b, P, RhsCsr{P.crow, P.qrp, P.qvar, P.qval}); }
extern "C" int dlg_query_covariance_plan_probe(int N, int M, const int* colptr, const int* rowidx, int nq, const int* qrow,
                                               const int* rowptr, const int* var, int* chunk_of_query, long* stats, int nstats)
{
  SymHost H;
  char err[512];
  if(sym_analyze(H, N, M, colptr, rowidx, 0, M, err, sizeof(err))) { dlg_set_error("symbolic analysis: %s", err); return DLG_ERR_ARG; }
  CovPack K;
  DLG_CHECK(query_pack(N, nq, qrow, rowptr, var, K, "dlg_query_covariance_plan_probe"));
  ReachHost R;
  reach_build(H, K.nch, [&](int ch, std::vector<int>& st) { query_starts(H, K, ch, st); }, R);
  if(chunk_of_query) for(int k = 0; k < nq; k++) chunk_of_query[k] = K.req_ch[k];
  const long v[] = { (long)K.nch, (long)R.pair_sn.size(), (long)K.maxvar };
  for(int i = 0; i < nstats && i < 3; i++) stats[i] = v[i];
  return DLG_OK;
}

void sparse_leverage_free(SparseSym* Y) { for(auto& P : Y->lev) reach_plan_release(P); }

int sparse_leverage_reach(dlg_backend* b, int s, int fs, int nf, double** d_gram, const int** d_slot_ptr, long* visits)
{
  SparseSym* Y = b->sym;
  if(!Y) { dlg_set_error("dlg_sparse_set_pattern must be called first"); return DLG_ERR_STATE; }
  DLG_CHECK(lev_plan_build(b, fs, nf));
  SparseSym::LevPlan& P = Y->lev[fs - 1];
  reach_for_each_level(P, Y->H.nlevels, [&](const int* wl, int n) {
    hipLaunchKernelGGL(k_lev_fwd_level, dim3(n), dim3(TPB), Y->lev_lds, b->stream, wl, P.pair_sn, P.pair_ch, P.pair_off,
                       P.cp_ptr, Y->sn_c0, Y->sn_rowptr, Y->sn_rows, Y->sn_lx, Y->lev_iperm, Y->Jp, Y->Ji, b->slot[s].Jin(),
                       Y->Lx, nf*fs, fs, P.scr, P.gram);
  });
  DLG_LAUNCH_CHECK();
  *d_gram = P.gram; *d_slot_ptr = P.cp_ptr;
  if(visits) *visits = P.visits;
  return DLG_OK;
}
int sparse_leverage_stats(const dlg_backend* b, int fs, long* nchunks, long* visits, int* nsn)
{
  const SparseSym* Y = b->sym;
  if(!Y || fs < 1 || fs > 2 || Y->lev[fs - 1].nf < 0) { dlg_set_error("no leverage plan is held for feature size %d", fs); return DLG_ERR_STATE; }
  *nchunks = Y->lev[fs - 1].nch; *visits = Y->lev[fs - 1].visits; *nsn = Y->H.nsn;
  return DLG_OK;
}
int lev_gram_rows(dlg_backend* b, int s, int row0, int nrows, int fs, const double* d_il, double* d_gram)
{
  SparseSym* Y = b->sym;
  hipLaunchKernelGGL(k_lev_gram_rows, dim3(1), dim3(64), 0, b->stream, Y->Jp, Y->Ji, b->slot[s].Jin(), row0, nrows, fs, d_il, d_gram);
  DLG_LAUNCH_CHECK();
  return DLG_OK;
}
int lev_finish(dlg_backend* b, int s, int nf, int fs, const int* d_slot_ptr, const double* d_gram, double scale, int mode, double* d_out)
{
  if(nf <= 0) return DLG_OK;
  hipLaunchKernelGGL(k_lev_finish, dim3(dlg_cdiv(nf, TPB)), dim3(TPB), 0, b->stream, nf, fs, d_slot_ptr, d_gram, b->slot[s].xin(),
                     scale, mode, d_out);
  DLG_LAUNCH_CHECK();
  return DLG_OK;
}
```

### libdogleg_amd/csrc/sparse_region.cpp

```cpp
#include "sparse_region.h"
#include <algorithm>
#include <cstdio>
#include <cstdlib>

namespace {
constexpr int FAC_LDS = SYM_FAC_LDS_BUDGET;
long panel_doubles(long w, long rows, bool cmp, bool leaf)
{
  return cmp ? ((rows - w + 1) & ~1L)*w + (leaf ? 4 : 8)*w : ((rows + 1) & ~1L)*w;
}

std::vector<int> cut_tile_columns(int T, int want)
{
  std::vector<int> cut;
  for(int cap = (T*(T + 1)/2 + want - 1)/std::max(want, 1); ; cap++)
  {
    cut.assign(1, 0);
    int load = 0;
    for(int t = 0; t < T; t++)
    {
      if(load > 0 && load + (T - t) > cap) { cut.push_back(t); load = 0; }
      load += T - t;
    }
    cut.push_back(T);
// ... 228 lines not shown
          cut = cut_tile_columns(T, want_h);
          nrep = std::max(1, (int)cut.size() - 1);
          hbm_rep = nrep > 1;
        }
      }
      first[i] = (int)R.item.size(); count[i] = nrep;
      for(int r = 0; r < nrep; r++)
      {
        it = H.fw_item[i];
        it.rep = r; it.tj0 = (nrep == 1) ? 0 : cut[r]; it.tj1 = (nrep == 1 || r == nrep - 1) ? (1 << 20) : cut[r+1];
        it.rsv2 = nrep;
        it.pad = l;
        if(hbm_rep || (nrep > 1 && slice_ok))
        {
          const long jA = col(it.tj0), jB = (r == nrep - 1) ? mb : col(it.tj1);
          const long eA = sym_w_linear(mb, jA), eB = sym_w_linear(mb, jB);
          it.eA = (int)eA; it.eB = (int)eB;
          if(hbm_rep)
          {
            it.sliced = 0;
            lds_need = std::max(lds_need, (pan + 2)*8);
            it.ch0 = write_children(H, it, jA, jB, pan, [&](long jw, long df) { return 0x8000 | (sym_w_linear(mb, jw) + df); },
                                    first, count, R.rec, R.dst);
          }
          else
          {
            const long slp = eA & 1, wt = pan + slp;
            it.sliced = 1;
            lds_need = std::max(lds_need, (pan + slp + (eB - eA) + 2)*8);
            it.ch0 = write_children(H, it, jA, jB, wt + (eB - eA), [&](long jw, long df) { return wt + (sym_w_linear(mb, jw) - eA) + df; },
                                    first, count, R.rec, R.dst);
          }
        }
        R.item.push_back(it);
      }
    }
  }
  for(size_t k = 0; k < H.mf_rec.size(); k++) R.rec[k].rsv = child_workgroups(R.rec[k].rsv, first, count);
  R.nwg = (int)R.item.size();
  R.lds = (int)std::max<long>(lds, lds_need);
  if(K.timing) fprintf(stderr, "%d workgroups, %d bytes of LDS, multifrontal from level %d)\n", R.nwg, R.lds, H.mf_level0);
  return R;
}

int region_check(const SymHost& H, const RegionPlan& R, long* stats, char* err, size_t len)
{
  long nsliced = 0, nhbm = 0;
  auto fail = [&](const char* what, size_t g) { snprintf(err, len, "one-launch region: %s (workgroup %zu)", what, g); return 1; };
  std::vector<long> covered;
  for(size_t g = 0; g < R.item.size(); g++)
  {
    const FwItem& it = R.item[g];
    const long mb = it.nrows - it.w, pan = panel_doubles(it.w, it.nrows, false, false), ntri = mb*(mb + 1)/2;
    const long T = (mb + 15) >> 4;
    const long jA = std::min<long>(16L*it.tj0, mb), jB = it.tj1 >= T ? mb : std::min<long>(16L*it.tj1, mb);
    const bool stretch_ok = it.eA == jA*mb - jA*(jA - 1)/2 && it.eB == jB*mb - jB*(jB - 1)/2;
    if(it.rep == 0) covered.assign((size_t)std::max<long>(T, 1), 0);
    for(long t = std::min<long>(it.tj0, T); t < std::min<long>(it.tj1, T); t++) covered[(size_t)t]++;
    long lds_end;
    if(it.sliced)
    {
      nsliced++;
      if(!stretch_ok) return fail("slice bounds do not match its tile columns", g);
      lds_end = pan + (it.eA & 1) + (it.eB - it.eA) + 1;
    }
    else
    {
// ... 9 lines not shown
    if(lds_end*8 > R.lds) return fail("its LDS need exceeds the launch's", g);
    if(R.lds > FAC_LDS) return fail("the launch's LDS exceeds the budget", g);
    for(int k = 0; k < it.nch; k++)
    {
      if((size_t)(it.ch0 + k) >= R.rec.size()) return fail("children record out of range", g);
      const MfChild& rc2 = R.rec[it.ch0 + k];
      if(rc2.rsv >= 0)
      {
        const long ci = rc2.rsv & 0xfffff, cn = rc2.rsv >> 20;
        if(cn < 1 || ci + cn > (long)g) return fail("a child's workgroups do not precede their parent", g);
      }
      if(rc2.dst_off < 0 || (size_t)(rc2.dst_off + rc2.npad) > R.dst.size()) return fail("destination list out of range", g);
      if(rc2.u_off < 0 || rc2.u_off + rc2.npad > H.uscr_size) return fail("a child's update matrix outside the scratch", g);
      for(long e = 0; e < rc2.npad; e++)
      {
        const long d = R.dst[(size_t)(rc2.dst_off + e)];
        if(it.sliced || it.jsp >= 0) { if(d >= pan + (it.sliced ? (it.eA & 1) + (it.eB - it.eA) : sym_w_linear(mb, it.jsp)) + 1) return fail("a destination behind the workgroup's LDS", g); }
        else if(!(d & 0x8000) ? d >= pan + 1 : (d & 0x7fff) > ntri) return fail("a destination outside panel / update matrix", g);
        else if((d & 0x8000) && it.rsv2 > 1 && ((d & 0x7fff) < it.eA || (d & 0x7fff) >= it.eB)) return fail("an HBM replica adds to an entry it does not own", g);
      }
    }
    const bool last = g + 1 == R.item.size() || R.item[g + 1].rep == 0;
    if(last && mb > 0 && it.u_off >= 0)
      for(long t = 0; t < T; t++) if(covered[(size_t)t] != 1) return fail("a tile column of the update matrix is not formed exactly once", g);
  }
  if(stats) { stats[0] = nsliced; stats[1] = nhbm; }
  return 0;
}

uint64_t region_plan_hash(const RegionPlan& R)
{
  Fnv f;
  f.add(R.level0, R.lds, R.stage, R.nwg);
  for(const FwItem& it : R.item)
    f.add(it.s, it.r0, it.r1, it.w, it.nrows, it.col0, it.bd0, it.nbd, it.lx, it.top, it.u_off, it.ch0, it.nch, it.bdw, it.jsp,
          it.rep, it.tj0, it.tj1, it.pad, it.sliced, it.eA, it.eB, it.rsv2);
  for(const MfChild& r : R.rec) f.add(r.u_off, r.dst_off, r.npad, r.rsv);
  for(uint16_t d : R.dst) f.add(d);
  return f.h;
}

uint64_t fac_levels_hash(const FacLevels& L)
{
  Fnv f;
  for(size_t l = 0; l < L.nt.size(); l++)
    f.add(L.nt[l], L.lds[l], L.leaf[l], L.stage[l], L.upd_coop[l], L.upd_lds[l], L.upd_nw[l],
          L.syrk_lds[l], L.syrk_nt[l], L.syrk_kc[l], L.syrk_fused[l], L.fin_ny[l]);
  return f.h;
}
```

### libdogleg_amd/csrc/sparse_region.h

```cpp
#pragma once
#include "sparse_symbolic.h"
#include <cstddef>

struct RegionKnobs
{
  int ncu, cap, rmax;
  bool slices, persist;
  bool lower, timing;
};
RegionKnobs region_knobs_env(int ncu);

struct FacLevels { std::vector<int> nt, lds, leaf, stage, upd_coop, upd_lds, upd_nw, syrk_lds, syrk_nt, syrk_kc, syrk_fused, fin_ny; };
int fac_level_params(const SymHost& H, FacLevels& L, char* err, size_t len);

struct RegionPlan
{
  int level0 = 0, level1 = -1, lds = 0, stage = 0, nwg = 0;
  bool acc_any = false;
  std::vector<FwItem> item;
  std::vector<MfChild> rec;
  std::vector<uint16_t> dst;
};
RegionPlan region_plan(const SymHost& H, const FacLevels& L, int lo_min, int hi, const RegionKnobs& K);
int region_check(const SymHost& H, const RegionPlan& R, long* stats, char* err, size_t len);
uint64_t region_plan_hash(const RegionPlan& R);
uint64_t fac_levels_hash(const FacLevels& L);
```

### libdogleg_amd/csrc/sparse_selinv.hip

```cpp
#include "sparse_internal.h"
#include <algorithm>
#include <chrono>
#include <cstdint>

namespace {
constexpr int SMR = 16;
constexpr int SEL_WLDS = 128;
typedef double sel_v4d __attribute__((ext_vector_type(4)));
__device__ __forceinline__ int sel_tri(int i, int j) { return i*(i + 1)/2 + j; }

size_t sel_prep_lds(int w)
{
  const size_t lt = w <= SEL_WLDS ? (size_t)((w*(w + 1)/2 + 1) & ~1) : 0;
  return sizeof(double)*(lt + (size_t)((w + 1) & ~1) + 2*(size_t)w*SMR);
}

__global__ void __launch_bounds__(TPB) k_selinv_prep(const SelTask* __restrict__ task, const int* __restrict__ sn_c0,
                                                     const int* __restrict__ sn_rowptr, const int64_t* __restrict__ sn_lx,
                                                     const double* __restrict__ Lx, double* __restrict__ Yb)
{
  extern __shared__ __attribute__((aligned(16))) double lds[];
  const SelTask T = task[blockIdx.x];
  const int s = T.s, cb = T.ti;
  const int w = sn_c0[s+1] - sn_c0[s], nrows = sn_rowptr[s+1] - sn_rowptr[s], r = nrows - w - 1;
// ... 134 lines not shown
}

__global__ void __launch_bounds__(TPB) k_selinv_pick(long n, const int64_t* __restrict__ pos, const double* __restrict__ src,
                                                     double* __restrict__ out)
{
  const long e = (long)blockIdx.x*TPB + threadIdx.x;
  if(e < n) out[e] = src[pos[e]];
}

int64_t sel_pos(const SymHost& H, int u, int v)
{
  const int pu = H.iperm[u], pv = H.iperm[v], c = std::min(pu, pv), rr = std::max(pu, pv);
  const int s = H.col_sn[c], c0 = H.sn_c0[s], w = H.sn_c0[s+1] - c0, nrows = H.sn_rowptr[s+1] - H.sn_rowptr[s];
  const int jc = c - c0;
  int ir;
  if(rr < c0 + w)
  {
    ir = rr - c0;
    const int b0 = H.sn_bd_ptr[s], b1 = H.sn_bd_ptr[s+1];
    if(b1 > b0)
    {
      const int* m0 = H.sn_bd_col.data() + b0;
      const int* m1 = H.sn_bd_col.data() + b1;
      if(std::upper_bound(m0, m1, ir) != std::upper_bound(m0, m1, jc)) return -1;
    }
  }
  else
  {
    const int* rows = H.sn_rows.data() + H.sn_rowptr[s];
    const int* it = std::lower_bound(rows + w, rows + nrows - 1, rr);
    if(it == rows + nrows - 1 || *it != rr) return -1;
    ir = (int)(it - rows);
  }
  return H.sn_lx[s] + ir + (int64_t)jc*nrows;
}

int sel_lookup(const dlg_backend* b, long n, const int* row, const int* col, std::vector<int64_t>& pos, const char* who)
{
  const int N = b->N;
  const SymHost* H = b->type == DLG_SPARSE ? &b->sym->H : nullptr;
  pos.resize(n);
  for(long e = 0; e < n; e++)
  {
    const int u = row[e], v = col[e];
    if(u < 0 || v < 0 || u >= N || v >= N)
    { dlg_set_error("%s: entry %ld (%d, %d) is outside the %d variables", who, e, u, v, N); return DLG_ERR_ARG; }
    if(!H) { pos[e] = (int64_t)std::max(u, v) + (int64_t)std::min(u, v)*N; continue; }
    pos[e] = sel_pos(*H, u, v);
    if(pos[e] < 0)
    {
      dlg_set_error("%s: entry %ld (%d, %d) is not in the structure of the factor; take blocks off it from dlg_covariance_blocks",
                    who, e, u, v);
      return DLG_ERR_ARG;
    }
  }
  return DLG_OK;
}

int sel_plan(dlg_backend* b, SelInv& X)
{
  SparseSym* Y = b->sym;
  const SymHost& H = Y->H;
  const int nsn = H.nsn;
  std::vector<int> parent(nsn, -1), dep(nsn, 0), nchild(nsn, 0), prel(nsn, -1);
  for(int s = nsn - 1; s >= 0; s--)
  {
    const int w = H.sn_c0[s+1] - H.sn_c0[s], r = H.sn_rowptr[s+1] - H.sn_rowptr[s] - w - 1;
// ... 11 lines not shown
  X.tb_ptr.assign(1, 0); X.tc_ptr.assign(1, 0);
  X.fsize[0] = X.fsize[1] = 0;
  int wmax = 1;
  for(int d = 0; d < nd; d++)
  {
    int64_t at = 0;
    for(int s : by[d])
      if(nchild[s] > 0) { const int64_t ns = H.sn_rowptr[s+1] - H.sn_rowptr[s] - 1; foff[s] = at; at += ns*ns; }
    X.fsize[d & 1] = std::max(X.fsize[d & 1], at);
    for(int s : by[d])
    {
      const int w = H.sn_c0[s+1] - H.sn_c0[s], r = H.sn_rowptr[s+1] - H.sn_rowptr[s] - w - 1;
      for(int ti = 0; 16*ti < r; ti++) for(int tj = 0; 16*tj < w; tj++) task.push_back({s, ti, tj, 0});
    }
    X.tb_ptr.push_back((int)task.size());
    for(int s : by[d])
    {
      const int w = H.sn_c0[s+1] - H.sn_c0[s];
      for(int ti = 0; 16*ti < w; ti++) for(int tj = 0; tj <= ti; tj++) task.push_back({s, ti, tj, 0});
    }
    X.tc_ptr.push_back((int)task.size());
  }
  for(int s = 0; s < nsn; s++)
  {
    const int w = H.sn_c0[s+1] - H.sn_c0[s];
    wmax = std::max(wmax, w);
    for(int cb = 0; cb < w; cb += SMR) prep.push_back({s, cb, 0, 0});
  }
  X.ndepth = nd; X.nprep = (int)prep.size();
  X.prep_lds = (int)std::max(sel_prep_lds(std::min(wmax, SEL_WLDS)), sel_prep_lds(wmax));
  DLG_HIP(hipFuncSetAttribute(reinterpret_cast<const void*>(&k_selinv_prep), hipFuncAttributeMaxDynamicSharedMemorySize, X.prep_lds));
  DLG_CHECK(upload(X.prep, prep)); DLG_CHECK(upload(X.task, task));
  DLG_CHECK(upload(X.par, parent)); DLG_CHECK(upload(X.prel, prel)); DLG_CHECK(upload(X.foff, foff));
  X.sx_n = H.lx_size;
  DLG_HIP(hipMalloc(&X.Sx, sizeof(double)*(size_t)std::max<int64_t>(X.sx_n, 1)));
  DLG_HIP(hipMalloc(&X.Yb, sizeof(double)*(size_t)std::max<int64_t>(X.sx_n, 1)));
  for(int i = 0; i < 2; i++) DLG_HIP(hipMalloc(&X.F[i], sizeof(double)*(size_t)std::max<int64_t>(X.fsize[i], 1)));
  X.sparse_ready = true;
  return DLG_OK;
}

int sel_sweep(dlg_backend* b, SelInv& X)
{
  SparseSym* Y = b->sym;
  hipStream_t st = b->stream;
  hipLaunchKernelGGL(k_selinv_prep, dim3(X.nprep), dim3(TPB), X.prep_lds, st, X.prep, Y->sn_c0, Y->sn_rowptr, Y->sn_lx, Y->Lx, X.Yb);
  for(int d = 0; d < X.ndepth; d++)
  {
    const int nb = X.tb_ptr[d+1] - X.tc_ptr[d], nc = X.tc_ptr[d+1] - X.tb_ptr[d+1];
    const int wpg = TPB/64;
    if(nb > 0)
      hipLaunchKernelGGL(k_selinv_level, dim3(dlg_cdiv(nb, wpg)), dim3(TPB), 0, st, X.task + X.tc_ptr[d], nb, 0, Y->sn_c0,
                         Y->sn_rowptr, Y->sn_lx, Y->relpos, X.par, X.prel, X.foff, X.F[(d + 1) & 1], X.F[d & 1], X.Yb, X.Sx);
    if(nc > 0)
      hipLaunchKernelGGL(k_selinv_level, dim3(dlg_cdiv(nc, wpg)), dim3(TPB), 0, st, X.task + X.tb_ptr[d+1], nc, 1, Y->sn_c0,
                         Y->sn_rowptr, Y->sn_lx, Y->relpos, X.par, X.prel, X.foff, X.F[(d + 1) & 1], X.F[d & 1], X.Yb, X.Sx);
  }
  DLG_LAUNCH_CHECK();
  return DLG_OK;
}

void sel_free_query(SelInv& X)
{
  if(X.qpos) (void)hipFree(X.qpos);
  if(X.qout) (void)hipFree(X.qout);
  X.qpos = nullptr; X.qout = nullptr; X.qkey.clear(); X.nq = 0;
}
}

void selinv_release(dlg_backend* b)
{
  if(!b->selinv) return;
  if(b->stream) (void)hipStreamSynchronize(b->stream);
  SelInv& X = *b->selinv;
  sel_free_query(X);
  for(void* q : {(void*)X.prep, (void*)X.task, (void*)X.par, (void*)X.prel, (void*)X.foff, (void*)X.Sx, (void*)X.Yb,
                 (void*)X.F[0], (void*)X.F[1], (void*)X.dvar, (void*)X.dystart, (void*)X.Linv_rm, (void*)X.Sig, (void*)X.dwork})
    if(q) (void)hipFree(q);
  delete b->selinv;
  b->selinv = nullptr;
}

int selinv_entries(dlg_backend* b, long n, const int* row, const int* col, double* out_host, const char* who)
{
  if(!b->selinv) b->selinv = new SelInv;
  SelInv& X = *b->selinv;
  const bool sparse = b->type == DLG_SPARSE;
  const auto t0 = std::chrono::steady_clock::now();
  bool built = false;
// ... 82 lines not shown
```

### libdogleg_amd/csrc/sparse_solve.hip

```cpp
#include "sparse_internal.h"

namespace {
#ifdef DLG_FL_PROFILE
__device__ long long g_bw_prof[64*8];
__device__ long long g_bw_chain[256*8];
#define BW_STAMP(k) do { if(threadIdx.x == 0 && blockIdx.x == 0) g_bw_prof[(prof_lvl & 63)*8 + (k)] = clock64(); \
                         if(threadIdx.x == 0 && pr_flag && blockIdx.x < 256) g_bw_chain[blockIdx.x*8 + (k)] = wall_clock64(); } while(0)
#else
#define BW_STAMP(k)
#endif

__global__ void __launch_bounds__(TPB) k_solve_fwd_level(const int* __restrict__ lvl_sn,
                                                         const int* __restrict__ sn_c0,
                                                         const int* __restrict__ sn_rowptr,
                                                         const int64_t* __restrict__ sn_lx,
                                                         const int* __restrict__ sn_scr,
                                                         const int* __restrict__ rl_ptr,
                                                         const int* __restrict__ rl_pos,
                                                         const int* __restrict__ perm,
                                                         const double* __restrict__ Lx,
                                                         const double* __restrict__ rhs,
                                                         double* __restrict__ scr,
                                                         double* __restrict__ ywork)
{
// ... 63 lines not shown
}
template <int BWD_NT, bool BD_ONLY>
__global__ void __launch_bounds__(BWD_NT, BD_ONLY ? 4 : 1) k_solve_bwd_level(const SolveItem* __restrict__ items,
                                                            const int* __restrict__ sn_rows,
                                                            const int* __restrict__ perm,
                                                            const double* __restrict__ Lx,
                                                            double* __restrict__ ywork,
                                                            double* __restrict__ out, int use_aug,
                                                            const int* __restrict__ sn_bd_col, int top_lds, int xb_cap,
                                                            int* pr_flag, int pr_epoch, const int* __restrict__ info, DlgHandoff ho,
                                                            double* xh, int xh_n, double* __restrict__ mm)
{
  extern __shared__ __attribute__((aligned(16))) double lds[];
  __shared__ int s_skip;
  double dmin = 1e300, dmax = 0.0;
  if(threadIdx.x == 0) s_skip = *info != 0x7fffffff;
  constexpr int NW = BWD_NT/64;
  typedef const __attribute__((address_space(1))) double* gcd_t;
  typedef __attribute__((address_space(1))) double* gd_t;
  auto ldx = [&](const double* p) -> double { return pr_flag ? __hip_atomic_load((gcd_t)p, __ATOMIC_RELAXED, __HIP_MEMORY_SCOPE_AGENT) : *p; };
  constexpr unsigned long long X_EMPTY = 0x7FF8DEADBEEF0002ull;
  typedef __attribute__((address_space(1))) unsigned long long* gu_t;
  const bool xh_on = pr_flag != nullptr && xh != nullptr && ho.skew == 0;
  unsigned long long* xcur = reinterpret_cast<unsigned long long*>(xh) + (size_t)(pr_epoch & 1)*xh_n;
  auto put_xh = [&](int col, double v) {
    if(xh_on) __hip_atomic_store((gu_t)(xcur + col), (unsigned long long)__double_as_longlong(v), __ATOMIC_RELAXED, __HIP_MEMORY_SCOPE_AGENT); };
  auto take_xh = [&](int col) -> double {
    unsigned long long u; int spins = 0;
    while((u = __hip_atomic_load((gu_t)(xcur + col), __ATOMIC_RELAXED, __HIP_MEMORY_SCOPE_AGENT)) == X_EMPTY)
    { __builtin_amdgcn_s_sleep(1); if(++spins > ho.spins) { atomicOr(ho.status, DLG_HANDOFF_SOLVE); u = 0; break; } }
    return __longlong_as_double((long long)u); };

  const int prof_lvl = top_lds >> 8; (void)prof_lvl;
  top_lds &= 1;
  BW_STAMP(0);
  const SolveItem it = items[blockIdx.x];
  const int c0 = it.c0, w = it.w, nrows = it.nrows;
  if(xh_on && (int)threadIdx.x < w) reinterpret_cast<unsigned long long*>(xh)[(size_t)(1 - (pr_epoch & 1))*xh_n + c0 + threadIdx.x] = X_EMPTY;
  const int* rows = sn_rows + it.rowoff;
  const double* L = Lx + it.lx;
  const int tid = threadIdx.x, lane = tid & 63, wv = tid >> 6;
  const int r = nrows - w - 1;
  const int nblk = (w + 7) >> 3;
  const bool xb_lds = r <= xb_cap;
  double* xb = lds;
  double* xs = lds + (xb_lds ? ((r + 1) & ~1) : 0);
  double* T = xs + 256;
  double* rhs = T + nblk*64;
  double* xp = rhs + 16;
  double* Lt = xp + 8*256;
  const int ldt = w | 1;
  const int MW = (w + 15) & ~15;
  double* Mx = Lt + (top_lds ? w*ldt : 0);
  const int nmem = BD_ONLY ? max(it.nbd, 1) : it.nbd;
  const int myrow = (tid < r) ? rows[w + tid] : 0;
  double myrhs = 0.0; int myperm = 0;
  if(tid < w) { myrhs = use_aug ? L[(nrows - 1) + (size_t)tid*nrows] : ywork[c0 + tid]; myperm = perm[c0 + tid]; }
  constexpr bool LEAN = BWD_NT == 256;
  constexpr int MV_SLOTS = LEAN ? 20 : 24;
  const int mv_cols = min(BWD_NT, max(w, 64)), mv_parts = BWD_NT/mv_cols;
  const int mv_j = tid % mv_cols, mv_p = tid/mv_cols;
  const int mv_len = (r + mv_parts - 1)/mv_parts;
  const int mv_i0 = mv_p*mv_len, mv_i1 = min(r, mv_i0 + mv_len);
  const bool mv_thread = mv_len <= MV_SLOTS && xb_lds;
  const bool mv_on = mv_thread && mv_j < w && mv_p < mv_parts;
  const double* mv_L = L + (size_t)min(mv_j, w - 1)*nrows + w;
  double mv[MV_SLOTS];
  {
    typedef double bw_v2d __attribute__((ext_vector_type(2)));
    typedef bw_v2d bw_v2d_u __attribute__((aligned(8)));
#pragma unroll
    for(int q = 0; q < MV_SLOTS; q += 2)
    {
      if(mv_on && mv_i0 + q + 1 < mv_i1) { const bw_v2d t = *reinterpret_cast<const bw_v2d_u*>(mv_L + mv_i0 + q); mv[q] = t.x; mv[q + 1] = t.y; }
      else { mv[q] = (mv_on && mv_i0 + q < mv_i1) ? mv_L[mv_i0 + q] : 0.0; mv[q + 1] = 0.0; }
    }
  }
  if(!BD_ONLY)
  for(int e = tid; e < (nmem > 0 ? 0 : nblk*64); e += BWD_NT)
  {
    const int j0 = (e >> 6)*8, a = (e >> 3) & 7, b = e & 7;
    const bool valid = a >= b && j0 + a < w;
    double v = valid ? L[(j0 + a) + (size_t)(j0 + b)*nrows] : 0.0;
    if(a == b && valid) { dmin = fmin(dmin, v); dmax = fmax(dmax, v); }
    if(a == b) v = valid ? 1.0/v : 1.0;
    T[e] = v;
  }
  if(!BD_ONLY && top_lds && nmem == 0)
  {
    const int cp_rows = min(BWD_NT, (w + 63) & ~63), cp_ng = BWD_NT/cp_rows, cp_g = tid/cp_rows;
    for(int i = tid - cp_g*cp_rows; i < w && cp_g < cp_ng; i += cp_rows)
      for(int j0 = cp_g; j0 <= i; j0 += 16*cp_ng)
      {
        double v[16];
#pragma unroll
        for(int u = 0; u < 16; u++) v[u] = (j0 + u*cp_ng <= i) ? L[i + (size_t)(j0 + u*cp_ng)*nrows] : 0.0;
#pragma unroll
        for(int u = 0; u < 16; u++) if(j0 + u*cp_ng <= i) Lt[i + (j0 + u*cp_ng)*ldt] = v[u];
      }
  }
  double Lm[8][8];
  int m0 = 0, nbm = 0;
  if(nmem > 0 && tid < nmem)
  {
    if(it.rsv > 0) { m0 = tid*it.rsv; nbm = it.rsv; }
    else
    {
      const int* mcol = sn_bd_col + it.bd0;
      m0 = mcol[tid]; nbm = ((tid + 1 < nmem) ? mcol[tid + 1] : w) - m0;
    }
  }
  if(nmem > 0)
  {
#pragma unroll
    for(int a = 0; a < 8; a++)
#pragma unroll
      for(int b = 0; b <= a; b++) Lm[a][b] = (a < nbm) ? L[(m0 + a) + (size_t)(m0 + b)*nrows] : (a == b ? 1.0 : 0.0);
    if(mm)
    {
#pragma unroll
      for(int a = 0; a < 8; a++) if(a < nbm) { dmin = fmin(dmin, Lm[a][a]); dmax = fmax(dmax, Lm[a][a]); }
    }
  }
  if(mm && (nmem > 0 ? 64*wv < nmem : wv < nblk))
  {
#pragma unroll
    for(int o = 32; o > 0; o >>= 1) { dmin = fmin(dmin, __shfl_down(dmin, o, 64)); dmax = fmax(dmax, __shfl_down(dmax, o, 64)); }
    if(lane == 0) { mm[(8*blockIdx.x + wv)*2] = dmin; mm[(8*blockIdx.x + wv)*2 + 1] = dmax; }
  }
  BW_STAMP(1);
  const bool premul = it.rsv != 0 && !BD_ONLY && nmem == 0 && pr_flag != nullptr && it.pflag >= 0;
  if(premul)
  {
    __syncthreads();
    double ti[8];
    const bool ton = tid < 8*nblk;
    if(ton)
    {
      const double* Tb = T + (tid >> 3)*64;
      const int c = tid & 7;
      double Lb[8][8];
#pragma unroll
      for(int a = 0; a < 8; a++)
#pragma unroll
        for(int b2 = 0; b2 <= a; b2++) Lb[a][b2] = Tb[a*8 + b2];
#pragma unroll
      for(int i = 0; i < 8; i++)
      {
        double v = 0.0;
#pragma unroll
// ... 71 lines not shown
  BW_STAMP(2);
  double tinv[8];
  const bool tinv_on = !BD_ONLY && nmem == 0 && tid < 8*nblk && !premul;
  if(tinv_on)
  {
    const double* Tb = T + (tid >> 3)*64;
    const int c = tid & 7;
    double Lb[8][8];
#pragma unroll
    for(int a = 0; a < 8; a++)
#pragma unroll
      for(int b = 0; b <= a; b++) Lb[a][b] = Tb[a*8 + b];
#pragma unroll
    for(int i = 0; i < 8; i++)
    {
      double v = 0.0;
#pragma unroll
      for(int k = 0; k < i; k++) v -= (k >= c) ? Lb[i][k]*tinv[k] : 0.0;
      tinv[i] = (i == c) ? Lb[i][i] : ((i > c) ? v*Lb[i][i] : 0.0);
    }
  }
  if(mv_thread)
  {
    double acc = 0.0;
#pragma unroll
    for(int q = 0; q < MV_SLOTS; q++) acc += mv[q]*((mv_i0 + q < mv_i1) ? xb[mv_i0 + q] : 0.0);
    if(mv_on) xp[mv_p*256 + mv_j] = acc;
  }
  else
  {
    for(int e = 256 + tid; e < mv_parts*256; e += BWD_NT) xp[e] = 0.0;
    for(int jg = 4*wv; jg < w; jg += 4*NW)
    {
      const double* Lj = L + (size_t)jg*nrows + w;
      const int nc = min(4, w - jg);
      double acc[4] = {0.0, 0.0, 0.0, 0.0};
#pragma unroll 2
      for(int i = lane; i < r; i += 64)
      {
        const double x = xb_lds ? xb[i] : ldx(ywork + rows[w + i]);
#pragma unroll
        for(int c = 0; c < 4; c++) acc[c] += ((c < nc) ? Lj[i + (size_t)c*nrows] : 0.0)*x;
      }
#pragma unroll
      for(int c = 0; c < 4; c++)
      {
        const double sum = wave_sum(acc[c]);
        if(lane == 0 && c < nc) xp[jg + c] = sum;
      }
    }
  }
  __syncthreads();
  BW_STAMP(3);
  if(tinv_on)
  {
    double* Tb = T + (tid >> 3)*64;
    const int c = tid & 7;
#pragma unroll
    for(int i = 0; i < 8; i++) if(i >= c) Tb[i*8 + c] = tinv[i];
  }
  if(nmem > 0)
  {
    if(tid < w)
    {
      double sum = 0.0;
      for(int p = 0; p < mv_parts; p++) sum += xp[p*256 + tid];
      xs[tid] = myrhs - sum;
    }
    __syncthreads();
    if(LEAN)
    {
      if(tid < nmem)
        for(int a = nbm - 1; a >= 0; a--)
        {
          const double* Lc = L + (size_t)(m0 + a)*nrows + m0;
          double v = xs[m0 + a];
          for(int b = a + 1; b < nbm; b++) v -= Lc[b]*xs[m0 + b];
          xs[m0 + a] = v/Lc[a];
        }
    }
    else if(tid < nmem)
    {
      double xk[8];
#pragma unroll
      for(int a = 7; a >= 0; a--)
      {
        double v = (a < nbm) ? xs[m0 + a] : 0.0;
#pragma unroll
        for(int b = a + 1; b < 8; b++) v -= Lm[b][a]*xk[b];
        xk[a] = v/Lm[a][a];
      }
#pragma unroll
      for(int a = 0; a < 8; a++) if(a < nbm) xs[m0 + a] = xk[a];
    }
    __syncthreads();
    if(tid < w)
    {
      put_xh(c0 + tid, xs[tid]);
      if(pr_flag) __hip_atomic_store((gd_t)(ywork + c0 + tid), xs[tid], __ATOMIC_RELAXED, __HIP_MEMORY_SCOPE_AGENT);
      else ywork[c0 + tid] = xs[tid];
      out[myperm] = xs[tid];
    }
    if(pr_flag)
    {
      asm volatile("s_waitcnt vmcnt(0)" ::: "memory");
      __syncthreads();
      if(tid == 0) __hip_atomic_store(pr_flag + blockIdx.x, pr_epoch, __ATOMIC_RELAXED, __HIP_MEMORY_SCOPE_AGENT);
    }
// ... 196 lines not shown
  SparseSym* Y = b->sym;
  const SymHost& H = Y->H;
  const long xb_cap = env_int("DOGLEG_AMD_BWD_XB_CAP", 12288);
  Y->bwd_xb_cap = (int)xb_cap;
  Y->slv_lds.assign(H.nlevels, 0); Y->bwd_lds.assign(H.nlevels, 0); Y->bwd_nt.assign(H.nlevels, 512); Y->bwd_bd.assign(H.nlevels, 0); Y->bwd_pmx.assign(H.nlevels, 0);
  for(int l = 0; l < H.nlevels; l++)
  {
    long maxw = 0, mb = 0;
    for(int i = H.lvl_ptr[l]; i < H.lvl_ptr[l+1]; i++)
    {
      const int s = H.lvl_sn[i];
      const long wv = H.sn_c0[s+1] - H.sn_c0[s], nr = H.sn_rowptr[s+1] - H.sn_rowptr[s];
      if(wv > maxw) maxw = wv;
      const long rb = nr - wv - 1;
      const long need = (rb <= xb_cap ? rb + 3 : 0) + 256 + ((wv + 7)/8)*64 + 16 + 8*256;
      if(need > mb) mb = need;
    }
    if(maxw > 256) { dlg_set_error("supernode of width %ld is too wide for the backward-solve kernel", maxw); return DLG_ERR_ARG; }
    Y->slv_lds[l] = (int)(maxw*(maxw | 1)*8);
    if(Y->slv_lds[l] > LDS_BUDGET) { dlg_set_error("supernode of width %ld is too wide for the solve kernels", maxw); return DLG_ERR_ARG; }
    if(mb*8 > LDS_BUDGET) { dlg_set_error("supernode too large for the backward-solve kernel (%ld doubles)", mb); return DLG_ERR_ARG; }
    Y->bwd_lds[l] = (int)(mb*8);
    Y->bwd_pmx[l] = 0;
    {
      long pm = 0;
      for(int i = H.lvl_ptr[l]; i < H.lvl_ptr[l+1]; i++)
      {
        const int s = H.lvl_sn[i];
        const long wv = H.sn_c0[s+1] - H.sn_c0[s];
        if(H.sn_bd_ptr[s+1] == H.sn_bd_ptr[s]) pm = std::max(pm, ((wv + 7)/8)*8*((wv + 15) & ~15L));
      }
      if(pm > 0 && !getenv("DOGLEG_AMD_NO_PREMUL") && (long)Y->bwd_lds[l] + pm*8 <= LDS_BUDGET) Y->bwd_pmx[l] = (int)(pm*8);
    }
    Y->bwd_nt[l] = (maxw <= 128 && H.lvl_ptr[l+1] - H.lvl_ptr[l] >= 512) ? 256 : 512;
    bool allbd = true;
    for(int i = H.lvl_ptr[l]; i < H.lvl_ptr[l+1]; i++) { const int s = H.lvl_sn[i]; if(H.sn_bd_ptr[s+1] == H.sn_bd_ptr[s]) allbd = false; }
    Y->bwd_bd[l] = allbd ? 1 : 0;
    if(Y->bwd_nt[l] != 512 || Y->bwd_bd[l]) Y->bwd_pmx[l] = 0;
    Y->bwd_lds[l] += Y->bwd_pmx[l];
  }
  {
    std::vector<SolveItem> items(H.xl_sn.size());
    for(int k = 0; k < (int)H.xl_sn.size(); k++)
    {
      const int s = H.xl_sn[k];
      SolveItem& it = items[k];
      it = solve_item(H, s);
      it.rsv = Y->bwd_pmx[H.sn_level[s]] ? 1 : 0;
      if(it.nbd > 0)
      {
        const int* mc = &H.sn_bd_col[it.bd0];
        const int wd0 = (it.nbd > 1 ? mc[1] : it.w) - mc[0];
        bool same = mc[0] == 0;
        for(int m = 0; m < it.nbd && same; m++) if(((m + 1 < it.nbd) ? mc[m+1] : it.w) - mc[m] != wd0 || mc[m] != m*wd0) same = false;
        it.rsv = same ? wd0 : 0;
      }
    }
    DLG_CHECK(upload(Y->slv_item, items)); Y->allocs.push_back(Y->slv_item);
    std::vector<double> none(16*std::max<size_t>(items.size(), 1));
    for(size_t i = 0; i < none.size(); i += 2) { none[i] = 1e300; none[i + 1] = 0.0; }
    DLG_CHECK(upload(Y->diag_mm, none)); Y->allocs.push_back(Y->diag_mm);
    Y->n_diag_mm = 8*(int)items.size();
  }
  {
    int64_t lo = -1, hi = 0;
    for(int i = H.lvl_ptr[0]; i < H.lvl_ptr[1]; i++)
    {
      const int s = H.lvl_sn[i];
      const int64_t a = H.sn_lx[s], e = a + (int64_t)(H.sn_rowptr[s+1] - H.sn_rowptr[s])*(H.sn_c0[s+1] - H.sn_c0[s]);
      if(lo < 0 || a < lo) lo = a;
      if(e > hi) hi = e;
    }
    Y->touch_off = 0; Y->touch_n = 0;
    if(lo >= 0 && H.nlevels >= 3 && hi - lo >= (1 << 20) && (hi - lo)*8 <= (int64_t)200 << 20)
    { Y->touch_off = lo & ~(int64_t)1; Y->touch_n = (hi - Y->touch_off) & ~(int64_t)1; }
  }
  Y->bw_level0 = H.nlevels; Y->bw_n = 0;
  if(!getenv("DOGLEG_AMD_NO_PERSIST") && H.nlevels >= 2)
  {
    int ncu = 256;
    { int dev = 0; if(hipGetDevice(&dev) == hipSuccess) (void)hipDeviceGetAttribute(&ncu, hipDeviceAttributeMultiprocessorCount, dev); }
    const int cap = env_int("DOGLEG_AMD_PERSIST_MAX", 2*ncu);
    int total = 0, l0 = H.nlevels, ldsb = 0;
    for(int l = H.nlevels - 1; l >= 1; l--)
    {
      const int n = H.xl_ptr[l+1] - H.xl_ptr[l];
      if(n == 0 || total + n > cap || Y->bwd_nt[l] != 512 || Y->bwd_bd[l]) break;
      total += n; l0 = l; ldsb = std::max(ldsb, Y->bwd_lds[l]);
    }

    if(H.nlevels - l0 >= 2)
    {
      std::vector<SolveItem> items;
      std::vector<int> pos(H.nsn, -1);
      for(int l = H.nlevels - 1; l >= l0; l--)
        for(int k = H.xl_ptr[l]; k < H.xl_ptr[l+1]; k++)
        {
          const int s = H.xl_sn[k];
          SolveItem it = solve_item(H, s);
          it.rsv = Y->bwd_pmx[l] ? 1 : 0;
          if(it.nbd > 0) it.rsv = 0;
          if(it.nrows - it.w - 1 > 0)
// ... 2 lines not shown
            const int ps = H.col_sn[prow];
            it.pflag = pos[ps];
            if(it.pflag < 0) { dlg_set_error("internal error: the parent of supernode %d is not part of the persistent backward launch", s); return DLG_ERR_ARG; }
          }
          pos[s] = (int)items.size();
          items.push_back(it);
        }
      Y->bw_level0 = l0; Y->bw_n = (int)items.size(); Y->bw_lds = std::max(ldsb, 84*1024);
      DLG_CHECK(upload(Y->slv_item_pr, items)); Y->allocs.push_back(Y->slv_item_pr);
      std::vector<unsigned long long> empty(2*(size_t)H.N, 0x7FF8DEADBEEF0002ull);
      DLG_HIP(hipMalloc(&Y->bwd_xh, sizeof(double)*empty.size())); Y->allocs.push_back(Y->bwd_xh);
      DLG_HIP(hipMemcpy(Y->bwd_xh, empty.data(), sizeof(double)*empty.size(), hipMemcpyHostToDevice));
      DLG_HIP(hipMalloc(&Y->bwd_flag, sizeof(int)*items.size())); Y->allocs.push_back(Y->bwd_flag);
      DLG_HIP(hipMemsetAsync(Y->bwd_flag, 0, sizeof(int)*items.size(), b->stream));
      Y->bwd_epoch = 0;
    }
  }
  for(const void* k : { (const void*)&k_solve_fwd_level, (const void*)&k_solve_bwd_level<256, false>,
                        (const void*)&k_solve_bwd_level<256, true>, (const void*)&k_solve_bwd_level<512, false> })
    DLG_HIP(hipFuncSetAttribute(k, hipFuncAttributeMaxDynamicSharedMemorySize, LDS_BUDGET));
  return DLG_OK;
}

static double* bwd_diag_mm(const dlg_backend* b, int l)
{
  const SparseSym* Y = b->sym;
  return (Y->diag_mm && !b->knobs.ei_jpass) ? Y->diag_mm + 16*(size_t)Y->H.xl_ptr[l] : (double*)nullptr;
}
static void launch_bwd_level(dlg_backend* b, int nt, bool bd, int grid, int lds, const SolveItem* items, double* out, int use_aug,
                             int l, int* flag, int epoch, double* xh, int nxh)
{
  SparseSym* Y = b->sym;
  double* mm = bwd_diag_mm(b, l);
#define DLG_BW_LAUNCH(...) hipLaunchKernelGGL(HIP_KERNEL_NAME(k_solve_bwd_level<__VA_ARGS__>), dim3(grid), dim3(nt), lds, b->stream, \
                                              items, Y->sn_rows, Y->perm, Y->Lx, Y->ywork, out, use_aug, Y->sn_bd_col, 256*l, Y->bwd_xb_cap, \
                                              flag, epoch, Y->d_info, dlg_handoff(b, 1 << 21), xh, nxh, mm)
  if(nt == 256 && bd) DLG_BW_LAUNCH(256, true);
  else if(nt == 256) DLG_BW_LAUNCH(256, false);
  else { nt = 512; DLG_BW_LAUNCH(512, false); }
#undef DLG_BW_LAUNCH
}

int sparse_solve(dlg_backend* b, const double* rhs, double* out)
{
  SparseSym* Y = b->sym;
  if(!Y) { dlg_set_error("dlg_sparse_set_pattern must be called first"); return DLG_ERR_STATE; }
  const SymHost& H = Y->H;
  hipStream_t st = b->stream;
  const int use_aug = (Y->aug_rhs != nullptr && Y->aug_rhs == rhs) ? 1 : 0;
  if(H.part_nranks > 1 && !use_aug)
  { dlg_set_error("with a subtree partition only the right-hand side that rode along with the factorisation (Jt x) can be solved for"); return DLG_ERR_STATE; }
  for(int l = 0; l < H.nlevels && !use_aug; l++)
  {
    const int n = H.xl_ptr[l+1] - H.xl_ptr[l];
    if(n > 0)
      hipLaunchKernelGGL(k_solve_fwd_level, dim3(n), dim3(TPB), Y->slv_lds[l], st, Y->xl_sn + H.xl_ptr[l],
                         Y->sn_c0, Y->sn_rowptr, Y->sn_lx, Y->sn_scr, Y->rl_ptr, Y->rl_pos, Y->perm,
                         Y->Lx, rhs, Y->scr, Y->ywork);
  }
  if(H.part_nranks > 1) DLG_HIP(hipMemsetAsync(out, 0, sizeof(double)*(size_t)H.N, st));
  int ltop = H.nlevels - 1;
  if(Y->bw_level0 < H.nlevels)
  {
    DlgRegionTurn turn(b);
    launch_bwd_level(b, 512, false, Y->bw_n, Y->bw_lds, Y->slv_item_pr, out, use_aug, Y->bw_level0, Y->bwd_flag, ++Y->bwd_epoch, Y->bwd_xh, H.N);
    ltop = Y->bw_level0 - 1;
  }
  for(int l = ltop; l >= 0; l--)
  {
    const int n = H.xl_ptr[l+1] - H.xl_ptr[l];
    if(n > 0) launch_bwd_level(b, Y->bwd_nt[l], Y->bwd_bd[l], n, Y->bwd_lds[l], Y->slv_item + H.xl_ptr[l], out, use_aug, l, (int*)nullptr, 0, (double*)nullptr, 0);
  }
  DLG_LAUNCH_CHECK();
  if(H.part_nranks > 1)
  {
    const bool room = out == b->slot[0].gn || out == b->slot[1].gn;
    const double* extra = room ? b->fold_scalar : nullptr;
    hipLaunchKernelGGL(k_mask_vec, dim3(dlg_cdiv(H.N, TPB)), dim3(TPB), 0, st, out, Y->colmask, H.N, extra);
    DLG_LAUNCH_CHECK();
    DLG_CHECK(dlg_allreduce_dev(b, out, (size_t)H.N + (extra ? 1 : 0)));
    if(extra) { b->fold_result = out + H.N; b->fold_scalar = nullptr; }
  }
  return DLG_OK;
}
```

### libdogleg_amd/csrc/sparse_symbolic.cpp

```cpp
#include "sparse_symbolic.h"
#include <algorithm>
#include <cstdio>
#include <cstdlib>
#include <cstring>
#include <chrono>
#include <thread>
#include <map>
#include <cmath>
#include <numeric>
#include <queue>
#include <array>

int env_int(const char* name, int dflt)
{
  const char* s = getenv(name);
  return (s && *s) ? atoi(s) : dflt;
}

namespace {

constexpr int VB_MAX   = 8;
constexpr int RB_MAX   = 8;
constexpr int CH_JTX   = 128;
constexpr int MAXCH_JTX = 2048;
constexpr int PANEL_CAP = 16384;
constexpr int SN_WMAX  = 256;

static int slice_cap() { return env_int("DOGLEG_AMD_SLICE_CAP", SYM_FAC_LDS_BUDGET/8 - 40); }

struct RowBlock { int r0, nrows, len, base, vptr, nvb; bool local; int lbase, lr0; };

struct Graph
{
// ... 163 lines not shown
      long pre = 0; int best = -1; double bestscore = 0;
      for(int l = 0; l < nl; l++)
      {
        const double before = (double)pre/(double)wt, after = (double)(wt - pre - lw[l])/(double)wt;
        pre += lw[l];
        if(l == 0 || l == nl-1) continue;
        if(before < 0.25 || after < 0.25) continue;
        const double score = (double)lw[l]*(1.0 + 0.5*fabs(before - after));
        if(best < 0 || score < bestscore) { best = l; bestscore = score; }
      }
      if(best < 0)
      {
        pre = 0;
        for(int l = 0; l < nl; l++) { pre += lw[l]; if(2*pre >= wt) { best = l; break; } }
        if(best <= 0) best = 1;
        if(best >= nl-1) best = nl-2;
      }
      std::vector<int> A(order.begin(), order.begin() + lvl_start[best]);
      std::vector<int> Sp(order.begin() + lvl_start[best], order.begin() + lvl_start[best+1]);
      std::vector<int> B(order.begin() + lvl_start[best+1], order.end());
      if(A.empty() || B.empty()) { std::sort(nodes.begin(), nodes.end()); order_leaf(nodes); continue; }
      std::sort(Sp.begin(), Sp.end());
      stack.push_back({std::move(Sp), true});
      stack.push_back({std::move(B), false});
      stack.push_back({std::move(A), false});
    }
  }
};

}

#define SYM_FAIL(...) do { snprintf(err, errlen, __VA_ARGS__); return 1; } while(0)

int sym_analyze(SymHost& S, int N, int M, const int* cp, const int* ri, int row0, int row1,
                char* err, int errlen, int part_rank, int part_nranks)
{
  const bool partition = part_nranks > 1;
  if(partition) { row0 = 0; row1 = M; }
  const bool sym_time = env_int("DOGLEG_AMD_SYM_DEBUG", 0) >= 2;
  auto sym_t0 = std::chrono::steady_clock::now();
  const char* sym_what = "setup";
  bool sym_parallel = false;
  auto sym_tick = [&](const char* next) {
    if(sym_parallel) return;
    if(sym_time)
    {
      const auto t1 = std::chrono::steady_clock::now();
      fprintf(stderr, "sym_analyze: %-40s %8.1f ms\n", sym_what, std::chrono::duration<double, std::milli>(t1 - sym_t0).count());
      sym_t0 = t1;
    }
    sym_what = next; };
#define SYM_TICK(name) sym_tick(name)

  S = SymHost();
  S.N = N; S.M = M; S.nnz = cp[M]; S.row0 = row0; S.row1 = row1;
  S.part_rank = partition ? part_rank : 0; S.part_nranks = partition ? part_nranks : 1;
  if(cp[0] != 0) SYM_FAIL("Jt column pointers must start at 0");

  SYM_TICK("1 var-blocks");
  std::vector<char> cut(N + 1, 0);
  cut[0] = cut[N] = 1;
  for(int r = 0; r < M; r++)
  {
    const int a = cp[r], b = cp[r+1];
    if(b < a) SYM_FAIL("Jt column pointers must be non-decreasing (row %d)", r);
    if(b - a > 65535) SYM_FAIL("measurement row %d has %d non-zeros; at most 65535 are supported", r, b - a);
    for(int q = a; q < b; q++)
    {
// ... 469 lines not shown
        }
        if(nsl > 1) { S.sn_top[s] = S.top_size; S.top_size += (int64_t)w*w; if(mine(s)) S.ms_sn.push_back(s); }
        if(!mine(s)) continue;
        const int per = (below + nsl - 1)/nsl;
        for(int k = 0; k < nsl; k++)
        {
          S.fw_sn.push_back(s); S.fw_r0.push_back(std::min(below, k*per)); S.fw_r1.push_back(std::min(below, (k+1)*per));
        }
        S.fw_lvl_ptr[l+1] += nsl;
      }
    }
    for(int l = 0; l < S.nlevels; l++) S.fw_lvl_ptr[l+1] += S.fw_lvl_ptr[l];
  }

  if(env_int("DOGLEG_AMD_SYM_DEBUG", 0))
  {
    for(int l = 0; l < S.nlevels; l++)
    {
      long n = 0, wsum = 0, rsum = 0, nofit = 0; int wmin = 1 << 30, wmax = 0, rmax = 0;
      for(int i = S.lvl_ptr[l]; i < S.lvl_ptr[l+1]; i++)
      {
        const int s = S.lvl_sn[i];
        const int w = S.sn_c0[s+1] - S.sn_c0[s], nr = S.sn_rowptr[s+1] - S.sn_rowptr[s];
        n++; wsum += w; rsum += nr; wmin = std::min(wmin, w); wmax = std::max(wmax, w); rmax = std::max(rmax, nr);
        const long mb = nr - w;
        (void)mb;
        if(sym_w_split(w, nr) < 0) nofit++;
      }
      fprintf(stderr, "level %2d: %5ld supernodes  w min/avg/max %d/%.1f/%d  nrows avg/max %.1f/%d  slices %d  update matrix not in LDS: %ld\n", l, n, wmin,
              (double)wsum/n, wmax, (double)rsum/n, rmax, S.fw_lvl_ptr[l+1] - S.fw_lvl_ptr[l], nofit);
    }
  }

  auto step8 = [&](char* err, int errlen) -> int {
  {
    struct Sub { int lvl, t, q, d, ka, rel; };
    std::vector<Sub> subs;
    S.mf_level0 = S.nlevels;
    {
      const int mf_req = env_int("DOGLEG_AMD_MF_LEVEL", 1), mf_maxm = 255;
      for(int l = S.nlevels - 1; mf_req >= 0 && l >= mf_req; l--)
      {
        bool ok = true;
        for(int i = S.lvl_ptr[l]; i < S.lvl_ptr[l+1] && ok; i++)
        {
          const int d = S.lvl_sn[i];
          const int mb = S.sn_rowptr[d+1] - S.sn_rowptr[d] - (S.sn_c0[d+1] - S.sn_c0[d]);
          if(S.sn_top[d] >= 0 || mb > mf_maxm) ok = false;
        }
        if(!ok) break;
        S.mf_level0 = l;
      }
    }
    S.sn_prel.assign(nsn, -1);
    std::vector<int> sn_parent(nsn, -1);
    for(int d = 0; d < nsn; d++)
    {
      const std::vector<int>& bl = st[sn_last(d)];
      if(bl.empty()) continue;
      const bool mf_src = S.sn_level[d] >= S.mf_level0;
      const int wd = S.sn_c0[d+1] - S.sn_c0[d];
      const int nrows_d = S.sn_rowptr[d+1] - S.sn_rowptr[d];
      size_t i = 0;
      int krow = wd;
      while(i < bl.size())
      {
// ... 141 lines not shown
        if(it.nbd > 0)
        {
          const int* mc = &S.sn_bd_col[it.bd0];
          const int wd0 = (it.nbd > 1 ? mc[1] : it.w) - mc[0];
          bool same = mc[0] == 0;
          for(int m = 0; m < it.nbd && same; m++) if(((m + 1 < it.nbd) ? mc[m+1] : it.w) - mc[m] != wd0) same = false;
          if(same) it.bdw = wd0;
        }
      }
    }
    std::sort(subs.begin(), subs.end(), [](const Sub& a, const Sub& b) {
      if(a.lvl != b.lvl) return a.lvl < b.lvl;
      if(a.t != b.t) return a.t < b.t;
      if(a.q != b.q) return a.q < b.q;
      return a.d < b.d; });
    S.ui_lvl_ptr.assign(S.nlevels + 1, 0);
    S.ui_ptr.push_back(0);
    std::vector<int> item_lvl;
    for(size_t i = 0; i < subs.size(); i++)
    {
      const Sub& u = subs[i];
      const bool newitem = (i == 0) || subs[i-1].lvl != u.lvl || subs[i-1].t != u.t || subs[i-1].q != u.q;
      if(newitem)
      {
        if(i != 0) S.ui_ptr.push_back((int)i);
        S.ui_t.push_back(u.t);
        S.ui_col.push_back(colstart[u.q] - S.sn_c0[u.t]);
        S.ui_nc.push_back(G.w[border[u.q]]);
        S.ui_lvl_ptr[u.lvl + 1]++;
        item_lvl.push_back(u.lvl);
      }
      const int nrows_d = S.sn_rowptr[u.d+1] - S.sn_rowptr[u.d];
      SymSub ss;
      ss.src = S.sn_lx[u.d] + u.ka; ss.rel = u.rel; ss.nrows_d = nrows_d;
      ss.wd = S.sn_c0[u.d+1] - S.sn_c0[u.d]; ss.m = nrows_d - u.ka;
      S.usub.push_back(ss);
      if(S.upd_syrk[u.lvl])
      {
        const int64_t mb = nrows_d - ss.wd, k0 = u.ka - ss.wd;
        S.usub_u.push_back(S.u_off[u.d] + k0*mb - k0*(k0 - 1)/2);
      }
      else S.usub_u.push_back(-1);
    }
    if(!subs.empty()) S.ui_ptr.push_back((int)subs.size());
    for(int l = 0; l < S.nlevels; l++) S.ui_lvl_ptr[l+1] += S.ui_lvl_ptr[l];
    S.uw_lvl_ptr.assign(S.nlevels + 1, 0); S.uf_lvl_ptr.assign(S.nlevels + 1, 0);
    S.upart_size = 0;
    const int nitems = (int)S.ui_t.size();
    const int unit_cost = 1024;
    const int unit_cost_gather = std::max(1, unit_cost/64);
    std::vector<int> cuts;
    for(int it = 0; it < nitems; it++)
    {
      const int s0 = S.ui_ptr[it], s1 = S.ui_ptr[it+1];
      const int lvl = item_lvl[it];
      const int t = S.ui_t[it];
      const int64_t slab = (int64_t)(S.sn_rowptr[t+1] - S.sn_rowptr[t])*S.ui_nc[it];
      cuts.clear(); cuts.push_back(s0);
      long acc = 0;
      for(int st = s0; st < s1; st++)
      {
        const SymSub& u = S.usub[st];
        const long c = S.upd_syrk[lvl] ? unit_cost_gather : ((u.wd <= 8) ? 1 : 64 + (long)u.wd*((u.m + 255)/256));
        if(acc > 0 && acc + c > unit_cost) { cuts.push_back(st); acc = 0; }
        acc += c;
      }
      cuts.push_back(s1);
// ... 12 lines not shown
          S.uw_item.push_back(it); S.uw_s0.push_back(cuts[k]); S.uw_s1.push_back(cuts[k+1]);
          S.uw_part.push_back(S.upart_size + (int64_t)k*slab);
          S.uw_lvl_ptr[lvl + 1]++;
        }
        S.upart_size += (int64_t)nch*slab;
      }
    }
    for(int l = 0; l < S.nlevels; l++) { S.uw_lvl_ptr[l+1] += S.uw_lvl_ptr[l]; S.uf_lvl_ptr[l+1] += S.uf_lvl_ptr[l]; }
  }

  return 0; };
  auto step9a = [&](char* err, int errlen) -> int {
  {
    std::vector<int> rptr(nvb + 1, 0);
    for(const RowBlock& b : rbs) if(b.local) for(int x = 0; x < b.nvb; x++) rptr[rb_vb[b.vptr + x] + 1]++;
    for(int v = 0; v < nvb; v++) rptr[v+1] += rptr[v];
    S.oblk.resize(nvb);
    S.contrib.resize(rptr[nvb]);
    std::vector<int> nx(rptr.begin(), rptr.end() - 1);
    for(int bi = 0; bi < nrb; bi++)
    {
      const RowBlock& b = rbs[bi];
      if(!b.local) continue;
      for(int x = 0; x < b.nvb; x++)
      {
        SymContrib c; c.base = b.lbase; c.r0 = b.lr0; c.len = (uint16_t)b.len;
        c.nrows = (uint8_t)b.nrows; c.pad = 0; c.offI = c.offJ = (uint16_t)rb_off[b.vptr + x];
        S.contrib[nx[rb_vb[b.vptr + x]]++] = c;
      }
    }
    for(int v = 0; v < nvb; v++)
    {
      const int q = bpos[v], t = sn_of_b[q];
      const int ld = S.sn_rowptr[t+1] - S.sn_rowptr[t];
      const int lc = colstart[q] - S.sn_c0[t];
      SymOutBlock o; memset(&o, 0, sizeof(o));
      o.dest = S.sn_lx[t] + lc + (int64_t)lc*ld; o.ld = ld; o.var0 = S.vb_start[v];
      o.nI = o.nJ = (uint8_t)G.w[v]; o.diag = 1;
      S.oblk[v] = o;
    }
    S.jtx_nparts = 0; S.jtx_fin_ptr.assign(1, 0); S.jtx_fin_blk.clear();
    S.jtx_covers_all = true;
    for(int v = 0; v < nvb; v++)
    {
      const int c0 = rptr[v], c1 = rptr[v+1];
      if(c1 == c0) { S.jtx_covers_all = false; continue; }
      int chunk = CH_JTX;
      if((c1 - c0 + chunk - 1)/chunk > MAXCH_JTX) chunk = (c1 - c0 + MAXCH_JTX - 1)/MAXCH_JTX;
      const int nch = (c1 - c0 + chunk - 1)/chunk;
      if(nch == 1) S.jtx_task.push_back({v, c0, c1, -1, S.vb_start[v], G.w[v]});
      else
      {
        for(int k = 0; k < nch; k++)
          S.jtx_task.push_back({v, c0 + k*chunk, std::min(c1, c0 + (k+1)*chunk), S.jtx_nparts + k, S.vb_start[v], G.w[v]});
        S.jtx_nparts += nch;
        S.jtx_fin_blk.push_back(v); S.jtx_fin_ptr.push_back(S.jtx_nparts);
      }
    }
  }

  return 0; };
  auto step9b = [&](char* err, int errlen) -> int {
  {
    constexpr int ACC_CAP = 256, SLOT_CAP = 32, STAGE_CAP = 512, TASK_BATCHES = 16;
    constexpr int RHO_PER_BATCH = 32, PAIRS_PER_BATCH = 256;
    std::vector<int> rptr(nvb + 1, 0);
    for(const RowBlock& b : rbs) if(b.local) for(int x = 0; x < b.nvb; x++) rptr[rb_vb[b.vptr + x] + 1]++;
    for(int v = 0; v < nvb; v++) rptr[v+1] += rptr[v];
    std::vector<int> rrb(rptr[nvb]), rx(rptr[nvb]);
    {
// ... 273 lines not shown
        const int fin0 = (int)S.asm_fin2.size();
        fin_lists.clear();
        for(int k = first_task; k < first_task + ntask; k++)
        {
          AsmMTask& T = S.asm_mtask[k];
          T.part = S.asm_part_size; S.asm_part_size += mtask_acc[k];
        }
        for(const Cls& C : classes)
        {
          int sidx = 0;
          for(const Ord& o : C.ords) if(o.P)
          {
            const AsmSlot& sl = S.asm_slot[C.slot0 + sidx]; sidx++;
            int f;
            if(fin_of[o.I] >= fin0 && fin_of[o.I] < (int)S.asm_fin2.size() && S.asm_fin2[fin_of[o.I]].dest == sl.dest) f = fin_of[o.I];
            else
            {
              f = (int)S.asm_fin2.size(); fin_of[o.I] = f;
              AsmFin2 F; F.dest = sl.dest; F.ld = ld; F.list0 = 0; F.nlist = 0; F.nI = sl.nI; F.nJ = (uint8_t)nJ;
              F.diag = sl.diag; F.to_part = 0;
              S.asm_fin2.push_back(F); fin_lists.emplace_back();
            }
            for(int k = first_task; k < first_task + ntask; k++)
            {
              const AsmMTask& T = S.asm_mtask[k];
              if(T.slot0 == C.slot0) fin_lists[f - fin0].push_back(T.part + sl.accoff);
            }
          }
        }
        if(carried)
        {
          if(fin_lists.empty())
          {
            AsmFin2 F; F.dest = S.sn_lx[t] + lc + (int64_t)lc*ld; F.ld = ld; F.list0 = 0; F.nlist = 0;
            F.nI = F.nJ = (uint8_t)nJ; F.diag = 1; F.to_part = 0;
            S.asm_fin2.push_back(F); fin_lists.emplace_back();
          }
          fin_lists[0].insert(fin_lists[0].begin(), rider_parts[J].begin(), rider_parts[J].end());
        }
        for(size_t f = 0; f < fin_lists.size(); f++)
        {
          S.asm_fin2[fin0 + f].list0 = (int)S.asm_fin2_list.size();
          S.asm_fin2[fin0 + f].nlist = (int)fin_lists[f].size();
          S.asm_fin2_list.insert(S.asm_fin2_list.end(), fin_lists[f].begin(), fin_lists[f].end());
        }
      }
      return true;
    };
    SYM_TICK("9b.2 column blocks");
    for(int pass = 0; pass < 2; pass++)
    for(int J = 0; J < nvb; J++)
    {
      const int r0 = rptr[J], r1 = rptr[J+1];
      if(r0 == r1 || (int)is_rider_blk[J] != pass) continue;
      const int qJ = bpos[J], t = sn_of_b[qJ];
      const int ld = S.sn_rowptr[t+1] - S.sn_rowptr[t];
      const int lc = colstart[qJ] - S.sn_c0[t];
      const int nJ = G.w[J];
      slots.clear();
      for(int e = r0; e < r1; e++)
      {
        const RowBlock& b = rbs[rrb[e]];
        for(int x = 0; x < b.nvb; x++)
        {
          const int I = rb_vb[b.vptr + x];
          if(bpos[I] < qJ || slot_stamp[I] == J) continue;
          slot_stamp[I] = J; slot_of[I] = (int)slots.size();
          int64_t dest;
          if(I == J) dest = S.sn_lx[t] + lc + (int64_t)lc*ld;
          else
          {
            const int ro = rowoff_in(t, bpos[I]);
            if(ro < 0) SYM_FAIL("internal error: JtJ block (%d,%d) missing from the factor structure", bpos[I], qJ);
            dest = S.sn_lx[t] + ro + (int64_t)lc*ld;
          }
          slots.push_back({I, dest, G.w[I], I == J ? 1 : 0});
        }
      }
      if(use_mfma && build_mfma(J, r0, r1, qJ, t, ld, lc, nJ, pass == 1)) continue;
      if(pass == 1) SYM_FAIL("internal error: no assembly schedule for dense column block %d", J);
      for(int e = r0; e < r1; e++) if(rb_host[rrb[e]] == J) { rb_host[rrb[e]] = -2; rb_rider[rrb[e]] = -1; }
      grp_of.assign(slots.size(), 0); acc_of.assign(slots.size(), 0);
      int ngrp = 0;
      {
        int acc = 0, cnt = 0;
        for(size_t k = 0; k < slots.size(); k++)
        {
          const int sz = slots[k].nI*nJ;
          if(cnt > 0 && (acc + sz > ACC_CAP || cnt >= SLOT_CAP)) { ngrp++; acc = 0; cnt = 0; }
          grp_of[k] = ngrp; acc_of[k] = acc; acc += sz; cnt++;
        }
        ngrp++;
      }
      for(int g = 0; g < ngrp; g++)
      {
        const int slot0 = (int)S.asm_slot.size();
        int acc_size = 0, nslots = 0;
        for(size_t k = 0; k < slots.size(); k++) if(grp_of[k] == g)
        {
          AsmSlot sl; sl.dest = slots[k].dest; sl.ld = ld; sl.accoff = (uint16_t)acc_of[k];
          sl.nI = (uint8_t)slots[k].nI; sl.diag = (uint8_t)slots[k].diag;
          S.asm_slot.push_back(sl); nslots++; acc_size = acc_of[k] + slots[k].nI*nJ;
        }
        const int first_task = (int)S.asm_ctask.size();
        bool task_open = false, batch_open = false;
        std::vector<int> seq0, seq;
        int nb_in_task = 0, stage_used = 0, rho_in_batch = 0, pairs_in_batch = 0;
// ... 184 lines not shown
    }
    for(int k = 0; k < N; k++) S.rl_ptr[k+1] += S.rl_ptr[k];
    S.rl_pos.resize(S.rl_ptr[N]);
    std::vector<int> nx(S.rl_ptr.begin(), S.rl_ptr.end() - 1);
    for(int d = 0; d < nsn; d++)
    {
      const int wd = S.sn_c0[d+1] - S.sn_c0[d];
      for(int k = S.sn_rowptr[d] + wd, j = 0; k < S.sn_rowptr[d+1] - 1; k++, j++)
        S.rl_pos[nx[S.sn_rows[k]]++] = S.sn_scr[d] + j;
    }
  }
  return 0; };
  SYM_TICK("8-10 schedules (4 threads)");
  {
    char e8[256] = "", e9a[256] = "", e9b[256] = "", e10[256] = "";
    int r8 = 0, r9a = 0, r9b = 0, r10 = 0;
    if(true)
    {
      sym_parallel = true;
      std::thread t8([&] { r8 = step8(e8, sizeof(e8)); });
      std::thread t9a([&] { r9a = step9a(e9a, sizeof(e9a)); });
      std::thread t10([&] { r10 = step10(e10, sizeof(e10)); });
      r9b = step9b(e9b, sizeof(e9b));
      t8.join(); t9a.join(); t10.join();
      sym_parallel = false;
    }
    else { r8 = step8(e8, sizeof(e8)); r9a = step9a(e9a, sizeof(e9a)); r9b = step9b(e9b, sizeof(e9b)); r10 = step10(e10, sizeof(e10)); }
    const char* em = r8 ? e8 : (r9a ? e9a : (r9b ? e9b : (r10 ? e10 : nullptr)));
    if(em) SYM_FAIL("%s", em);
  }
  SYM_TICK("done");
  return 0;
}
```

### libdogleg_amd/csrc/sparse_symbolic.h

```cpp
#pragma once
#include <cstdint>
#include <vector>

struct SymContrib
{
  int32_t  base;
  int32_t  r0;
  uint16_t len;
  uint8_t  nrows;
  uint8_t  pad;
  uint16_t offI;
  uint16_t offJ;
};
static_assert(sizeof(SymContrib) == 16, "SymContrib must be 16 bytes");

struct SymOutBlock
{
  int64_t dest;
  int32_t ld;
  int32_t var0;
  uint8_t nI, nJ, diag, pad;
  int32_t pad2;
};
static_assert(sizeof(SymOutBlock) == 24, "SymOutBlock layout");
// ... 89 lines not shown
  if(jsp*mb - jsp*(jsp - 1)/2 <= room) return (int)jsp;
  return -1;
}
inline long sym_w_linear(long mb, long jsp) { return jsp*mb - jsp*(jsp - 1)/2; }

struct FwItem
{
  int s, r0, r1, w;
  int nrows, col0;
  int bd0, nbd;
  int64_t lx, top, u_off;
  int ch0, nch;
  int bdw, jsp;
  int rep, tj0, tj1, pad;
  int sliced, eA, eB, rsv2;
};
struct MfChild { int64_t u_off, dst_off; int npad, rsv; };

struct SymHost
{
  int N = 0, M = 0, nnz = 0;
  int row0 = 0, row1 = 0;
  int part_rank = 0, part_nranks = 1, cut_level = -1;
  std::vector<int> sn_owner, xl_ptr, xl_sn, part_rows;
  int nvb = 0;
  std::vector<int> vb_start;
  std::vector<int> perm;
  std::vector<int> iperm;
  int nsn = 0;
  std::vector<int>     sn_c0;
  std::vector<int>     sn_rowptr;
  std::vector<int>     sn_rows;
  std::vector<int64_t> sn_lx;
  std::vector<int>     sn_scr;
  std::vector<int>     sn_level;
  int nlevels = 0;
  std::vector<int>     lvl_ptr;
  std::vector<int>     lvl_sn;
  std::vector<int>     sn_bd_ptr, sn_bd_col;
  std::vector<int>     fw_lvl_ptr, fw_sn, fw_r0, fw_r1;
  std::vector<int64_t> sn_top;
  std::vector<int>     ms_sn;
  int64_t top_size = 0;
  std::vector<int64_t> diagpos;
  std::vector<int>     col_sn;
  int64_t lx_size = 0;
  int     scr_size = 0;
  int     max_panel = 0;
  std::vector<int> ui_lvl_ptr;
  std::vector<int> ui_t, ui_col, ui_nc, ui_ptr;
  std::vector<SymSub> usub;
  std::vector<int> relpos;
  std::vector<int> uw_lvl_ptr;
  std::vector<int> uw_item, uw_s0, uw_s1;
  std::vector<int64_t> uw_part;
  std::vector<int> uf_lvl_ptr;
  std::vector<int> uf_item, uf_n;
  std::vector<int64_t> uf_off;
  int64_t upart_size = 0;
  std::vector<char>    upd_syrk;
  std::vector<int64_t> u_off;
  std::vector<int64_t> usub_u;
  int64_t uscr_size = 0;
  int mf_level0 = 0;
  std::vector<int> mf_cptr, mf_child;
  std::vector<int> sn_prel;
// ... 4 lines not shown
  std::vector<SymContrib>  contrib;
  std::vector<SymTask>     jtx_task;
  std::vector<int> jtx_fin_ptr, jtx_fin_blk;
  int jtx_nparts = 0;
  bool jtx_covers_all = false;
  std::vector<AsmRho>   asm_rho;
  std::vector<AsmPair>  asm_pair;
  std::vector<AsmSlot>  asm_slot;
  std::vector<AsmBatch> asm_batch;
  std::vector<AsmTask>  asm_ctask;
  std::vector<AsmFin>   asm_cfin;
  std::vector<AsmShape> asm_shape;
  std::vector<AsmKG>    asm_kg;
  std::vector<AsmMTask> asm_mtask;
  std::vector<AsmFin2>  asm_fin2;
  std::vector<int64_t>  asm_fin2_list;
  int asm_lds_len = 0;
  bool asm_td_inline = false;
  bool asm_ts_off = false;
  bool asm_jtx_ok = false;
  std::vector<int> jf_ptr, jf_ent, jf_var0, jf_w, jf_short, jf_long;
  std::vector<int>      fin2_stage;
  std::vector<AsmRun>   asm_run;
  std::vector<int>      asm_pdest;
  std::vector<int>      asm_tdest;
  int64_t asm_part_size = 0;
  std::vector<int> rl_ptr;
  std::vector<int> rl_pos;
  int64_t nnz_JtJ_lower = 0, nnz_L = 0;
  double  factor_flops = 0;
};

int sym_analyze(SymHost& S, int N, int M, const int* colptr, const int* rowidx, int row0, int row1,
                char* err, int errlen, int part_rank = 0, int part_nranks = 1);
```

Before: 1805.

## Store leaf supernode panels in compact block-diagonal layout

Adds a compact storage layout for level-0 (leaf) supernodes whose diagonal is block-diagonal with small members. Only each member's diagonal block plus the off-diagonal rows are stored, so the leading dimension shrinks and the factor kernels read and write less memory. The symbolic analysis, assembly destinations, factor kernels and backward paths are rewired to use the compact indexing. Forward solves that need the full layout get an expanded image built by a new kernel, which is regenerated whenever the factor changes. This adds conditional complexity and an extra expansion pass for some solves.

```diff
diff --git a/include/dlg_backend.h b/include/dlg_backend.h
--- a/include/dlg_backend.h
+++ b/include/dlg_backend.h
@@ -71,6 +71,11 @@
 int  dlg_sparse_stats(dlg_backend_t* b, long* nnz_JtJ_lower, long* nnz_L,
                       int* n_supernodes, int* n_levels, double* factor_flops);
 
+int  dlg_sparse_leaf_layout(dlg_backend_t* b);
+int  dlg_sparse_layout_probe(int N, int M, const int* colptr, const int* rowidx, int cap, int* nsn, int* sn_c0, int* sn_nrows,
+                             long long* sn_lx, int* sn_ld, int* sn_wd, int* sn_level, long long* diagpos, long long* augpos,
+                             long long* lx_size, int* compact);
+
 int  dlg_sparse_region_probe(int N, int M, const int* colptr, const int* rowidx, int ncu, long* stats, int nstats);
 
 int  dlg_sparse_schedule(dlg_backend_t* b, int* n_levels, int* persist_level0, int* persist_items);
diff --git a/libdogleg_amd/capi.py b/libdogleg_amd/capi.py
--- a/libdogleg_amd/capi.py
+++ b/libdogleg_amd/capi.py
@@ -39,6 +39,7 @@
     "dlg_covariance_blocks", "dlg_marginal_variances", "dlg_covariance_stats", "dlg_covariance_plan_seconds",
     "dlg_covariance_plan_probe", "dlg_covariance_entries", "dlg_covariance_entries_stats", "dlg_covariance_entries_probe",
     "dlg_query_covariance", "dlg_query_covariance_stats", "dlg_query_covariance_plan_seconds", "dlg_query_covariance_plan_probe",
+    "dlg_sparse_leaf_layout", "dlg_sparse_layout_probe",
 ]
 PROF_NAMES = ["K1_jtx", "K3K8_norm2Jv", "K4_kernel", "K4_total", "K5_factor", "K6_solve", "K7_step", "vec"]
 DOGLEG_SYMBOLS = [
@@ -204,6 +205,10 @@
     L.dlg_backend_device.argtypes = [V]
     L.dlg_sparse_pattern_matches.argtypes = [V, I, I]
     L.dlg_sparse_drop_pattern.argtypes = [V]
+    if hasattr(L, "dlg_sparse_leaf_layout"):
+        LL = C.POINTER(C.c_longlong)
+        L.dlg_sparse_leaf_layout.argtypes = [V]
+        L.dlg_sparse_layout_probe.argtypes = [C.c_int, C.c_int, I, I, C.c_int, I, I, I, LL, I, I, I, LL, LL, LL, I]
     L.dogleg_amd_release_cache.restype = None
     if hasattr(L, "dogleg_amd_optimize_dense_batch"):
         L.dogleg_amd_optimize_dense_batch.argtypes = [D, C.c_uint, C.c_uint, C.c_uint, V, V, PP, C.POINTER(BatchResult)]
@@ -435,6 +440,23 @@
                      "schedule_hash", "level_params_hash"]
 
 
+def layout_probe(N, M, Jp, Ji):
+    L = lib()
+    Jp = np.ascontiguousarray(Jp, dtype=np.int32)
+    Ji = np.ascontiguousarray(Ji, dtype=np.int32)
+    cap = N + 1
+    i32 = lambda n: np.zeros(n, dtype=np.int32)
+    i64 = lambda n: np.zeros(n, dtype=np.int64)
+    nsn, lxs, cmp = C.c_int(), C.c_longlong(), C.c_int()
+    c0, nr, ld, wd, lvl, lx, dp, ap = i32(cap), i32(cap), i32(cap), i32(cap), i32(cap), i64(cap), i64(N), i64(N)
+    ll = lambda a: a.ctypes.data_as(C.POINTER(C.c_longlong))
+    _ck(L.dlg_sparse_layout_probe(N, M, iptr(Jp), iptr(Ji), cap, C.byref(nsn), iptr(c0), iptr(nr), ll(lx), iptr(ld), iptr(wd),
+                                  iptr(lvl), ll(dp), ll(ap), C.byref(lxs), C.byref(cmp)), "layout probe")
+    n = nsn.value
+    return dict(compact=cmp.value, lx_size=lxs.value, c0=np.append(c0[:n], N), nrows=nr[:n], lx=lx[:n], ld=ld[:n], wd=wd[:n],
+                level=lvl[:n], diagpos=dp, augpos=ap)
+
+
 def region_probe(N, M, Jp, Ji, ncu=256):
     L = lib()
     Jp = np.ascontiguousarray(Jp, dtype=np.int32)
@@ -600,7 +622,8 @@
         _ck(self.L.dlg_sparse_stats(self.h, C.byref(a), C.byref(b), C.byref(c), C.byref(d), C.byref(e)),
             "stats")
         return dict(nnz_JtJ_lower=a.value, nnz_L=b.value, n_supernodes=c.value, n_levels=d.value,
-                    factor_flops=e.value)
+                    factor_flops=e.value,
+                    leaf_layout=self.L.dlg_sparse_leaf_layout(self.h) if hasattr(self.L, "dlg_sparse_leaf_layout") else 0)
 
     def schedule(self):
         a, b, c = C.c_int(), C.c_int(), C.c_int()
diff --git a/libdogleg_amd/csrc/panel_factor.h b/libdogleg_amd/csrc/panel_factor.h
--- a/libdogleg_amd/csrc/panel_factor.h
+++ b/libdogleg_amd/csrc/panel_factor.h
@@ -1032,14 +1032,14 @@
 }
 
 template <int NB, int DS = 8>
-__device__ __forceinline__ int bd_factor_member_g(double* __restrict__ G, int ldg, int c0, double* rdiag,
+__device__ __forceinline__ int bd_factor_member_g(double* __restrict__ Gm, int ldg, int c0, double* rdiag,
                                                   double* __restrict__ Dg)
 {
   double D[NB][NB];
 #pragma unroll
   for(int c = 0; c < NB; c++)
 #pragma unroll
-    for(int q = 0; q <= c; q++) D[c][q] = G[(c0 + c) + (size_t)(c0 + q)*ldg];
+    for(int q = 0; q <= c; q++) D[c][q] = Gm[c + (size_t)q*ldg];
   int badcol = -1;
 #pragma unroll
   for(int c = 0; c < NB; c++)
@@ -1059,7 +1059,7 @@
 #pragma unroll
   for(int c = 0; c < NB; c++)
 #pragma unroll
-    for(int q = 0; q <= c; q++) { G[(c0 + c) + (size_t)(c0 + q)*ldg] = D[c][q]; if(q < DS) Dg[(c0 + c)*DS + q] = D[c][q]; }
+    for(int q = 0; q <= c; q++) { Gm[c + (size_t)q*ldg] = D[c][q]; if(q < DS) Dg[(c0 + c)*DS + q] = D[c][q]; }
   return badcol;
 }
 template <int NB, int DS = 8>
@@ -1089,24 +1089,25 @@
 __device__ __forceinline__ void bd_compact_members(double* __restrict__ G, int ldg, int w, int tid,
                                                    const int* __restrict__ mcol_g, int nmem, int bdw,
                                                    int* mcol, double* rdiag, double* __restrict__ Dg,
-                                                   int* __restrict__ info, int col0)
+                                                   int* __restrict__ info, int col0, bool hbm_c = false)
 {
   for(int m = tid; m <= nmem; m += NT) mcol[m] = (m < nmem) ? (bdw > 0 ? m*bdw : mcol_g[m]) : w;
   for(int m = tid; m < nmem; m += NT)
   {
     const int c0 = bdw > 0 ? m*bdw : mcol_g[m];
     const int nb = (m + 1 < nmem ? (bdw > 0 ? (m + 1)*bdw : mcol_g[m + 1]) : w) - c0;
+    double* Gm = G + (size_t)c0*ldg + (hbm_c ? 0 : c0);
     int badcol;
     switch(nb)
     {
-      case 1: badcol = bd_factor_member_g<1, DS>(G, ldg, c0, rdiag, Dg); break;
-      case 2: badcol = bd_factor_member_g<2, DS>(G, ldg, c0, rdiag, Dg); break;
-      case 3: badcol = bd_factor_member_g<3, DS>(G, ldg, c0, rdiag, Dg); break;
-      case 4: badcol = bd_factor_member_g<4, DS>(G, ldg, c0, rdiag, Dg); break;
-      case 5: badcol = bd_factor_member_g<5, DS>(G, ldg, c0, rdiag, Dg); break;
-      case 6: badcol = bd_factor_member_g<6, DS>(G, ldg, c0, rdiag, Dg); break;
-      case 7: badcol = bd_factor_member_g<7, DS>(G, ldg, c0, rdiag, Dg); break;
-      default: badcol = bd_factor_member_g<8, DS>(G, ldg, c0, rdiag, Dg); break;
+      case 1: badcol = bd_factor_member_g<1, DS>(Gm, ldg, c0, rdiag, Dg); break;
+      case 2: badcol = bd_factor_member_g<2, DS>(Gm, ldg, c0, rdiag, Dg); break;
+      case 3: badcol = bd_factor_member_g<3, DS>(Gm, ldg, c0, rdiag, Dg); break;
+      case 4: badcol = bd_factor_member_g<4, DS>(Gm, ldg, c0, rdiag, Dg); break;
+      case 5: badcol = bd_factor_member_g<5, DS>(Gm, ldg, c0, rdiag, Dg); break;
+      case 6: badcol = bd_factor_member_g<6, DS>(Gm, ldg, c0, rdiag, Dg); break;
+      case 7: badcol = bd_factor_member_g<7, DS>(Gm, ldg, c0, rdiag, Dg); break;
+      default: badcol = bd_factor_member_g<8, DS>(Gm, ldg, c0, rdiag, Dg); break;
     }
     if(badcol >= 0) atomicMin(info, col0 + c0 + badcol);
   }
diff --git a/libdogleg_amd/csrc/sparse_factor.hip b/libdogleg_amd/csrc/sparse_factor.hip
--- a/libdogleg_amd/csrc/sparse_factor.hip
+++ b/libdogleg_amd/csrc/sparse_factor.hip
@@ -226,6 +226,7 @@
 #endif
   const bool stage_leaf_u = (mode & 4) != 0;
   const bool b16 = (mode & 16) != 0;
+  const bool hbm_c = LEAF && (mode & 32) != 0;
   mode &= 3;
   const FwItem it = items[blockIdx.x];
   const int r0 = it.r0, w = it.w, nrows = it.nrows;
@@ -237,6 +238,7 @@
   const int mb = nloc - w, ntri = mb*(mb + 1)/2;
   const bool cmp = it.nbd > 0 && top < 0;
   const int ldp = cmp ? ((mb + 1) & ~1) : ((nloc + 1) & ~1);
+  const int ldg = hbm_c ? ((it.bdw + mb + 1) & ~1) : nrows, gbl = hbm_c ? it.bdw : w;
   double* Pb = cmp ? P - w : P;
   const int row0c = cmp ? w : 0;
   const bool has_u = mode != 0 && top < 0;
@@ -266,21 +268,21 @@
       if(pr_flag && tid == 0) __hip_atomic_store(pr_flag + blockIdx.x, pr_epoch, __ATOMIC_RELAXED, __HIP_MEMORY_SCOPE_AGENT);
       return;
     }
-    bd_compact_members<NT, DS>(G, nrows, w, tid, sn_bd_col + it.bd0, it.nbd, it.bdw, s_mcol, s_rdiag, Dg, &sbad, it.col0);
+    bd_compact_members<NT, DS>(G, ldg, w, tid, sn_bd_col + it.bd0, it.nbd, it.bdw, s_mcol, s_rdiag, Dg, &sbad, it.col0, hbm_c);
   }
   const int cp_rows = min(NT, (nloc - row0c + 63) & ~63), cp_ng = NT/cp_rows, cp_g = tid/cp_rows;
 #ifndef DLG_LEAF_NO_GLDS
   if((LEAF && cmp) || (!LEAF && !cmp && !sliced && shift == 0))
   {
     const int ntot = ldp*w;
-    const double* g0 = cmp ? G + (w + shift) : G;
+    const double* g0 = cmp ? G + (gbl + shift) : G;
     for(int k = tid >> 6; 128*k < ntot; k += NT/64)
     {
       const int e = 128*k + 2*lane;
       if(e < ntot)
       {
         const int j = e / ldp, r = e - j*ldp;
-        __builtin_amdgcn_global_load_lds((const __attribute__((address_space(1))) void*)(g0 + (size_t)j*nrows + r),
+        __builtin_amdgcn_global_load_lds((const __attribute__((address_space(1))) void*)(g0 + (size_t)j*ldg + r),
                                          (__attribute__((address_space(3))) void*)(P + 128*k), 16, 0, 0);
       }
     }
@@ -290,12 +292,12 @@
   {
   for(int i = row0c + tid - cp_g*cp_rows; i < nloc && cp_g < cp_ng; i += cp_rows)
   {
-    const double* gp = G + (i < w ? i : i + shift);
+    const double* gp = G + (i < w ? i : i + shift + (gbl - w));
     for(int j0 = cp_g; j0 < w; j0 += CP_FLIGHT*cp_ng)
     {
       double v[CP_FLIGHT];
 #pragma unroll
-      for(int u = 0; u < CP_FLIGHT; u++) v[u] = (j0 + u*cp_ng < w) ? gp[(size_t)(j0 + u*cp_ng)*nrows] : 0.0;
+      for(int u = 0; u < CP_FLIGHT; u++) v[u] = (j0 + u*cp_ng < w) ? gp[(size_t)(j0 + u*cp_ng)*ldg] : 0.0;
 #pragma unroll
       for(int u = 0; u < CP_FLIGHT; u++) if(j0 + u*cp_ng < w) Pb[i + (j0 + u*cp_ng)*ldp] = v[u];
     }
@@ -421,7 +423,7 @@
   for(int i = row0c + tid - cp_g*cp_rows; i < nloc && cp_g < cp_ng && store_panel; i += cp_rows)
   {
     double* gp; size_t gs;
-    if(i >= w)        { gp = G + (i + shift); gs = (size_t)nrows; }
+    if(i >= w)        { gp = G + (i + shift + (gbl - w)); gs = (size_t)ldg; }
     else if(top < 0)  { gp = G + i; gs = (size_t)nrows; }
     else if(r0 == 0)  { gp = top_scr + top + i; gs = (size_t)w; }
     else continue;
@@ -1078,6 +1080,7 @@
   hipStream_t st = b->stream;
   const bool split = Y->top.level0 > 0 && H.nlevels >= 2 && H.part_nranks <= 1 && H.fw_lvl_ptr[1] > H.fw_lvl_ptr[0];
   if(part == 2 && !split) return DLG_OK;
+  if(part != 2) Y->fac_gen++;
   if(part != 2)
   {
   if(H.part_nranks > 1 && H.cut_level < 0) DLG_CHECK(sparse_partition_reduce(b));
@@ -1114,13 +1117,17 @@
     }
     if(n > 0 && !launched_before)
     {
-      const int fmode = ((l >= H.mf_level0) ? 2 : Y->fac.syrk_fused[l]) + 4*Y->fac.stage[l] + FMODE_B16 + 256*(l & 31);
+      const bool hbm_c = l == 0 && H.leaf_compact && Y->fac.leaf[l] && Y->fac.nt[l] == 256;
+      if(l == 0 && H.leaf_compact && !hbm_c) { dlg_set_error("internal error: compact leaf panels without the leaf kernel"); return DLG_ERR_STATE; }
+      const int fmode = ((l >= H.mf_level0) ? 2 : Y->fac.syrk_fused[l]) + 4*Y->fac.stage[l] + FMODE_B16 + (hbm_c ? 32 : 0) + 256*(l & 31);
       launch_factor_level(Y->fac.nt[l], Y->fac.leaf[l], n, Y->fac.lds[l], st, Y, Y->fw_item + H.fw_lvl_ptr[l], Y->mf_rec, Y->mf_dst,
                           fmode, (int*)nullptr, 0, DlgHandoff{nullptr, 0, 0}, (int64_t)0);
     }
     if(part == 1 && split && l == 0) { Y->fac_pending = true; DLG_LAUNCH_CHECK(); return DLG_OK; }
     const int nu = H.uw_lvl_ptr[l+1] - H.uw_lvl_ptr[l];
     const bool gather_next = nu > 0 && H.upd_syrk[l] && Y->fac.upd_nw[l] > 0;
+    if(l == 0 && H.leaf_compact && nu > 0 && !(gather_next && Y->fac.syrk_fused[l]))
+    { dlg_set_error("internal error: compact leaf panels without the fused two-phase update"); return DLG_ERR_STATE; }
     const int fin_ep = (l == 0 && gather_next) ? Y->fin_side_owed : 0;
     if(fin_ep) Y->fin_side_owed = 0;
     if(l == 0) DLG_CHECK(sparse_fin_side_gate(b));
diff --git a/libdogleg_amd/csrc/sparse_host.hip b/libdogleg_amd/csrc/sparse_host.hip
--- a/libdogleg_amd/csrc/sparse_host.hip
+++ b/libdogleg_amd/csrc/sparse_host.hip
@@ -162,6 +162,12 @@
   const bool partition = H.part_nranks > 1;
   if(partition) b->mloc = (int)H.part_rows.size();
   UP(sn_c0); UP(sn_rowptr); UP(sn_rows); UP(sn_scr); UP(lvl_sn); UP(sn_lx); UP(diagpos);
+  Y->sn_lx_u = Y->sn_lx;
+  if(H.leaf_compact)
+  {
+    UP(sn_ldc); UP(sn_ldc_wd);
+    DLG_CHECK(upload(Y->sn_lx_u, H.sn_lx_cl)); Y->allocs.push_back(Y->sn_lx_u);
+  }
   UP(ui_t); UP(ui_col); UP(ui_nc); UP(ui_ptr); UP(usub); UP(relpos); UP(u_off); UP(usub_u); UP(fw_item); UP(mf_rec); UP(mf_dst);
   UP(uw_item); UP(uw_s0); UP(uw_s1); UP(uw_part); UP(uf_item); UP(uf_n); UP(uf_off);
   UP(oblk); UP(contrib); UP(jtx_task); UP(jtx_fin_ptr); UP(jtx_fin_blk);
@@ -258,8 +264,8 @@
     for(int k = 0; k < H.N; k++)
     {
       const int s2 = H.col_sn[k];
-      const int64_t nrows = H.sn_rowptr[s2+1] - H.sn_rowptr[s2];
-      ap[k] = H.sn_lx[s2] + (nrows - 1) + (int64_t)(k - H.sn_c0[s2])*nrows;
+      const int nrows = H.sn_rowptr[s2+1] - H.sn_rowptr[s2];
+      ap[k] = H.lx_at(s2, nrows - 1, k - H.sn_c0[s2]);
     }
     DLG_CHECK(upload(Y->augpos, ap)); Y->allocs.push_back(Y->augpos);
     std::vector<int64_t> av((size_t)H.N);
@@ -566,6 +572,51 @@
   *n = b->sym ? b->sym->n_diag_mm : 0;
   return (b->sym && b->sym->n_diag_mm > 0) ? b->sym->diag_mm : nullptr;
 }
+namespace {
+__global__ void __launch_bounds__(TPB) k_user_image(const int* __restrict__ sn_c0, const int* __restrict__ sn_rowptr,
+                                                    const int64_t* __restrict__ sn_lx, const int64_t* __restrict__ sn_lx_cl,
+                                                    const int* __restrict__ sn_ldc, const int* __restrict__ sn_ldc_wd,
+                                                    const double* __restrict__ Lx, double* __restrict__ img)
+{
+  const int s = blockIdx.x;
+  const int w = sn_c0[s+1] - sn_c0[s], nrows = sn_rowptr[s+1] - sn_rowptr[s], ldc = sn_ldc[s], wd = sn_ldc_wd[s];
+  const double* src = Lx + sn_lx[s];
+  double* dst = img + sn_lx_cl[s];
+  const int n = nrows*w;
+  for(int e = threadIdx.x; e < n; e += TPB)
+  {
+    double v;
+    if(!ldc) v = src[e];
+    else
+    {
+      const int j = e / nrows, i = e - j*nrows, m0 = (j/wd)*wd;
+      v = (i >= w) ? src[(size_t)j*ldc + wd + (i - w)] : ((i >= m0 && i < m0 + wd) ? src[(size_t)j*ldc + (i - m0)] : 0.0);
+    }
+    dst[e] = v;
+  }
+}
+}
+int sparse_user_factor(dlg_backend* b)
+{
+  SparseSym* Y = b->sym;
+  if(!Y) return DLG_OK;
+  const SymHost& H = Y->H;
+  if(!H.leaf_compact) { Y->Lu = Y->Lx; return DLG_OK; }
+  if(!Y->Lu_img)
+  {
+    DLG_HIP(hipMalloc(&Y->Lu_img, sizeof(double)*((size_t)H.lx_size_cl + 8))); Y->allocs.push_back(Y->Lu_img);
+    DLG_HIP(hipMemsetAsync(Y->Lu_img + H.lx_size_cl, 0, sizeof(double)*8, b->stream));
+    Y->Lu_src = nullptr;
+  }
+  Y->Lu = Y->Lu_img;
+  if(Y->Lu_src == Y->Lx && Y->Lu_gen == Y->fac_gen) return DLG_OK;
+  hipLaunchKernelGGL(k_user_image, dim3(H.nsn), dim3(TPB), 0, b->stream, Y->sn_c0, Y->sn_rowptr, Y->sn_lx, Y->sn_lx_u,
+                     Y->sn_ldc, Y->sn_ldc_wd, Y->Lx, Y->Lu_img);
+  DLG_LAUNCH_CHECK();
+  Y->Lu_src = Y->Lx; Y->Lu_gen = Y->fac_gen;
+  return DLG_OK;
+}
+
 void sparse_hold_factor(dlg_backend* b)
 {
   SparseSym* Y = b->sym;
@@ -600,6 +651,30 @@
   hipLaunchKernelGGL(k_lower_word, dim3(1), dim3(64), 0, b->stream, Y->d_info, 0x7fffffff);
   DLG_LAUNCH_CHECK();
   Y->info_clean = false; Y->info_armed = false; Y->fac_pending = false;
+  return DLG_OK;
+}
+
+extern "C" int dlg_sparse_leaf_layout(dlg_backend_t* b) { return (b && b->sym) ? b->sym->H.leaf_compact : -1; }
+
+extern "C" int dlg_sparse_layout_probe(int N, int M, const int* colptr, const int* rowidx, int cap, int* nsn, int* sn_c0, int* sn_nrows,
+                                       long long* sn_lx, int* sn_ld, int* sn_wd, int* sn_level, long long* diagpos, long long* augpos,
+                                       long long* lx_size, int* compact)
+{
+  SymHost H;
+  char err[512];
+  if(sym_analyze(H, N, M, colptr, rowidx, 0, M, err, sizeof(err))) { dlg_set_error("symbolic analysis: %s", err); return DLG_ERR_ARG; }
+  if(H.nsn > cap) { dlg_set_error("layout probe: %d supernodes, room for %d", H.nsn, cap); return DLG_ERR_ARG; }
+  *nsn = H.nsn; *lx_size = H.lx_size; *compact = H.leaf_compact;
+  for(int s = 0; s < H.nsn; s++)
+  {
+    sn_c0[s] = H.sn_c0[s]; sn_nrows[s] = H.sn_rowptr[s+1] - H.sn_rowptr[s]; sn_lx[s] = H.sn_lx[s]; sn_ld[s] = H.lx_ld(s);
+    sn_wd[s] = H.sn_ldc[s] ? H.sn_ldc_wd[s] : 0; sn_level[s] = H.sn_level[s];
+  }
+  for(int k = 0; k < N; k++)
+  {
+    const int s = H.col_sn[k];
+    diagpos[k] = H.diagpos[k]; augpos[k] = H.lx_at(s, H.sn_rowptr[s+1] - H.sn_rowptr[s] - 1, k - H.sn_c0[s]);
+  }
   return DLG_OK;
 }
 
diff --git a/libdogleg_amd/csrc/sparse_internal.h b/libdogleg_amd/csrc/sparse_internal.h
--- a/libdogleg_amd/csrc/sparse_internal.h
+++ b/libdogleg_amd/csrc/sparse_internal.h
@@ -58,6 +58,8 @@
   uint64_t pat_key = 0;
   int *sn_c0 = nullptr, *sn_rowptr = nullptr, *sn_rows = nullptr, *sn_scr = nullptr, *lvl_sn = nullptr;
   int64_t *sn_lx = nullptr, *diagpos = nullptr;
+  int64_t* sn_lx_u = nullptr; int *sn_ldc = nullptr, *sn_ldc_wd = nullptr;
+  double *Lu = nullptr, *Lu_img = nullptr; const double* Lu_src = nullptr; uint64_t fac_gen = 0, Lu_gen = 0;
   int *ui_t = nullptr, *ui_col = nullptr, *ui_nc = nullptr, *ui_ptr = nullptr;
   SymSub* usub = nullptr; int* relpos = nullptr;
   int *uw_item = nullptr, *uw_s0 = nullptr, *uw_s1 = nullptr, *uf_item = nullptr, *uf_n = nullptr;
@@ -136,3 +138,4 @@
 int sparse_factor_setup(dlg_backend* b);
 int sparse_factor_levels(dlg_backend* b, int part = 0);
 int sparse_solve_setup(dlg_backend* b);
+int sparse_user_factor(dlg_backend* b);
diff --git a/libdogleg_amd/csrc/sparse_multi.hip b/libdogleg_amd/csrc/sparse_multi.hip
--- a/libdogleg_amd/csrc/sparse_multi.hip
+++ b/libdogleg_amd/csrc/sparse_multi.hip
@@ -474,6 +474,7 @@
   if(!Y) { dlg_set_error("dlg_sparse_set_pattern must be called first"); return DLG_ERR_STATE; }
   const SymHost& H = Y->H;
   hipStream_t st = b->stream;
+  DLG_CHECK(sparse_user_factor(b));
   if(!Y->ms_scr)
   {
     DLG_HIP(hipMalloc(&Y->ms_scr, sizeof(double)*((size_t)H.scr_size + 1)*MR)); Y->allocs.push_back(Y->ms_scr);
@@ -489,14 +490,14 @@
     const int n = H.xl_ptr[l+1] - H.xl_ptr[l];
     if(n > 0)
       hipLaunchKernelGGL(k_msolve_fwd_level, dim3(n), dim3(TPB), Y->ms_lds_f, st, Y->xl_sn + H.xl_ptr[l], Y->sn_c0,
-                         Y->sn_rowptr, Y->sn_lx, Y->sn_scr, Y->rl_ptr, Y->rl_pos, Y->perm, Y->Lx, d_il, Y->ms_scr, Y->ms_y);
+                         Y->sn_rowptr, Y->sn_lx_u, Y->sn_scr, Y->rl_ptr, Y->rl_pos, Y->perm, Y->Lu, d_il, Y->ms_scr, Y->ms_y);
   }
   for(int l = H.nlevels - 1; l >= 0; l--)
   {
     const int n = H.xl_ptr[l+1] - H.xl_ptr[l];
     if(n > 0)
       hipLaunchKernelGGL(k_msolve_bwd_level, dim3(n), dim3(TPB), Y->ms_lds_b, st, Y->xl_sn + H.xl_ptr[l], Y->sn_c0,
-                         Y->sn_rowptr, Y->sn_rows, Y->sn_lx, Y->perm, Y->Lx, Y->ms_y, d_il);
+                         Y->sn_rowptr, Y->sn_rows, Y->sn_lx_u, Y->perm, Y->Lu, Y->ms_y, d_il);
   }
   DLG_LAUNCH_CHECK();
   return DLG_OK;
@@ -656,11 +657,12 @@
 template <class Rhs> int reach_run(dlg_backend* b, CovPlan& P, const Rhs& rhs)
 {
   SparseSym* Y = b->sym;
+  DLG_CHECK(sparse_user_factor(b));
   DLG_CHECK(reach_setup(b));
   const ReachPlan& R = P.R;
   reach_for_each_level(R, Y->H.nlevels, [&](const int* wl, int n) {
     hipLaunchKernelGGL(k_cov_fwd_level<Rhs>, dim3(n), dim3(TPB), Y->lev_lds, b->stream, wl, R.pair_sn, R.pair_ch, R.pair_off,
-                       R.cp_ptr, Y->sn_c0, Y->sn_rowptr, Y->sn_rows, Y->sn_lx, Y->Lx, rhs, P.pptr, P.prod, P.goff, R.scr, P.gram);
+                       R.cp_ptr, Y->sn_c0, Y->sn_rowptr, Y->sn_rows, Y->sn_lx_u, Y->Lu, rhs, P.pptr, P.prod, P.goff, R.scr, P.gram);
   });
   DLG_LAUNCH_CHECK();
   return DLG_OK;
@@ -973,11 +975,12 @@
   SparseSym* Y = b->sym;
   if(!Y) { dlg_set_error("dlg_sparse_set_pattern must be called first"); return DLG_ERR_STATE; }
   DLG_CHECK(lev_plan_build(b, fs, nf));
+  DLG_CHECK(sparse_user_factor(b));
   SparseSym::LevPlan& P = Y->lev[fs - 1];
   reach_for_each_level(P, Y->H.nlevels, [&](const int* wl, int n) {
     hipLaunchKernelGGL(k_lev_fwd_level, dim3(n), dim3(TPB), Y->lev_lds, b->stream, wl, P.pair_sn, P.pair_ch, P.pair_off,
-                       P.cp_ptr, Y->sn_c0, Y->sn_rowptr, Y->sn_rows, Y->sn_lx, Y->lev_iperm, Y->Jp, Y->Ji, b->slot[s].Jin(),
-                       Y->Lx, nf*fs, fs, P.scr, P.gram);
+                       P.cp_ptr, Y->sn_c0, Y->sn_rowptr, Y->sn_rows, Y->sn_lx_u, Y->lev_iperm, Y->Jp, Y->Ji, b->slot[s].Jin(),
+                       Y->Lu, nf*fs, fs, P.scr, P.gram);
   });
   DLG_LAUNCH_CHECK();
   *d_gram = P.gram; *d_slot_ptr = P.cp_ptr;
diff --git a/libdogleg_amd/csrc/sparse_region.cpp b/libdogleg_amd/csrc/sparse_region.cpp
--- a/libdogleg_amd/csrc/sparse_region.cpp
+++ b/libdogleg_amd/csrc/sparse_region.cpp
@@ -284,7 +284,7 @@
                                     first, count, R.rec, R.dst);
           }
         }
-        R.item.push_back(it);
+        R.item.push_back(it); R.lx_cl.push_back(H.sn_lx_cl.empty() ? it.lx : H.sn_lx_cl[it.s]);
       }
     }
   }
@@ -360,9 +360,12 @@
 {
   Fnv f;
   f.add(R.level0, R.lds, R.stage, R.nwg);
-  for(const FwItem& it : R.item)
-    f.add(it.s, it.r0, it.r1, it.w, it.nrows, it.col0, it.bd0, it.nbd, it.lx, it.top, it.u_off, it.ch0, it.nch, it.bdw, it.jsp,
+  for(size_t g = 0; g < R.item.size(); g++)
+  {
+    const FwItem& it = R.item[g];
+    f.add(it.s, it.r0, it.r1, it.w, it.nrows, it.col0, it.bd0, it.nbd, g < R.lx_cl.size() ? R.lx_cl[g] : it.lx, it.top, it.u_off, it.ch0, it.nch, it.bdw, it.jsp,
           it.rep, it.tj0, it.tj1, it.pad, it.sliced, it.eA, it.eB, it.rsv2);
+  }
   for(const MfChild& r : R.rec) f.add(r.u_off, r.dst_off, r.npad, r.rsv);
   for(uint16_t d : R.dst) f.add(d);
   return f.h;
diff --git a/libdogleg_amd/csrc/sparse_region.h b/libdogleg_amd/csrc/sparse_region.h
--- a/libdogleg_amd/csrc/sparse_region.h
+++ b/libdogleg_amd/csrc/sparse_region.h
@@ -18,6 +18,7 @@
   int level0 = 0, level1 = -1, lds = 0, stage = 0, nwg = 0;
   bool acc_any = false;
   std::vector<FwItem> item;
+  std::vector<int64_t> lx_cl;
   std::vector<MfChild> rec;
   std::vector<uint16_t> dst;
 };
diff --git a/libdogleg_amd/csrc/sparse_selinv.hip b/libdogleg_amd/csrc/sparse_selinv.hip
--- a/libdogleg_amd/csrc/sparse_selinv.hip
+++ b/libdogleg_amd/csrc/sparse_selinv.hip
@@ -190,7 +190,7 @@
     if(it == rows + nrows - 1 || *it != rr) return -1;
     ir = (int)(it - rows);
   }
-  return H.sn_lx[s] + ir + (int64_t)jc*nrows;
+  return H.sn_lx_cl[s] + ir + (int64_t)jc*nrows;
 }
 
 int sel_lookup(const dlg_backend* b, long n, const int* row, const int* col, std::vector<int64_t>& pos, const char* who)
@@ -268,7 +268,7 @@
   DLG_HIP(hipFuncSetAttribute(reinterpret_cast<const void*>(&k_selinv_prep), hipFuncAttributeMaxDynamicSharedMemorySize, X.prep_lds));
   DLG_CHECK(upload(X.prep, prep)); DLG_CHECK(upload(X.task, task));
   DLG_CHECK(upload(X.par, parent)); DLG_CHECK(upload(X.prel, prel)); DLG_CHECK(upload(X.foff, foff));
-  X.sx_n = H.lx_size;
+  X.sx_n = H.lx_size_cl;
   DLG_HIP(hipMalloc(&X.Sx, sizeof(double)*(size_t)std::max<int64_t>(X.sx_n, 1)));
   DLG_HIP(hipMalloc(&X.Yb, sizeof(double)*(size_t)std::max<int64_t>(X.sx_n, 1)));
   for(int i = 0; i < 2; i++) DLG_HIP(hipMalloc(&X.F[i], sizeof(double)*(size_t)std::max<int64_t>(X.fsize[i], 1)));
@@ -280,17 +280,18 @@
 {
   SparseSym* Y = b->sym;
   hipStream_t st = b->stream;
-  hipLaunchKernelGGL(k_selinv_prep, dim3(X.nprep), dim3(TPB), X.prep_lds, st, X.prep, Y->sn_c0, Y->sn_rowptr, Y->sn_lx, Y->Lx, X.Yb);
+  DLG_CHECK(sparse_user_factor(b));
+  hipLaunchKernelGGL(k_selinv_prep, dim3(X.nprep), dim3(TPB), X.prep_lds, st, X.prep, Y->sn_c0, Y->sn_rowptr, Y->sn_lx_u, Y->Lu, X.Yb);
   for(int d = 0; d < X.ndepth; d++)
   {
     const int nb = X.tb_ptr[d+1] - X.tc_ptr[d], nc = X.tc_ptr[d+1] - X.tb_ptr[d+1];
     const int wpg = TPB/64;
     if(nb > 0)
       hipLaunchKernelGGL(k_selinv_level, dim3(dlg_cdiv(nb, wpg)), dim3(TPB), 0, st, X.task + X.tc_ptr[d], nb, 0, Y->sn_c0,
-                         Y->sn_rowptr, Y->sn_lx, Y->relpos, X.par, X.prel, X.foff, X.F[(d + 1) & 1], X.F[d & 1], X.Yb, X.Sx);
+                         Y->sn_rowptr, Y->sn_lx_u, Y->relpos, X.par, X.prel, X.foff, X.F[(d + 1) & 1], X.F[d & 1], X.Yb, X.Sx);
     if(nc > 0)
       hipLaunchKernelGGL(k_selinv_level, dim3(dlg_cdiv(nc, wpg)), dim3(TPB), 0, st, X.task + X.tb_ptr[d+1], nc, 1, Y->sn_c0,
-                         Y->sn_rowptr, Y->sn_lx, Y->relpos, X.par, X.prel, X.foff, X.F[(d + 1) & 1], X.F[d & 1], X.Yb, X.Sx);
+                         Y->sn_rowptr, Y->sn_lx_u, Y->relpos, X.par, X.prel, X.foff, X.F[(d + 1) & 1], X.F[d & 1], X.Yb, X.Sx);
   }
   DLG_LAUNCH_CHECK();
   return DLG_OK;
diff --git a/libdogleg_amd/csrc/sparse_solve.hip b/libdogleg_amd/csrc/sparse_solve.hip
--- a/libdogleg_amd/csrc/sparse_solve.hip
+++ b/libdogleg_amd/csrc/sparse_solve.hip
@@ -119,6 +119,7 @@
     return __longlong_as_double((long long)u); };
 
   const int prof_lvl = top_lds >> 8; (void)prof_lvl;
+  const bool hbm_c = BD_ONLY && (top_lds & 2) != 0;
   top_lds &= 1;
   BW_STAMP(0);
   const SolveItem it = items[blockIdx.x];
@@ -128,6 +129,7 @@
   const double* L = Lx + it.lx;
   const int tid = threadIdx.x, lane = tid & 63, wv = tid >> 6;
   const int r = nrows - w - 1;
+  const int ldg = hbm_c ? ((it.rsv + r + 2) & ~1) : nrows, gbl = hbm_c ? it.rsv : w;
   const int nblk = (w + 7) >> 3;
   const bool xb_lds = r <= xb_cap;
   double* xb = lds;
@@ -142,7 +144,7 @@
   const int nmem = BD_ONLY ? max(it.nbd, 1) : it.nbd;
   const int myrow = (tid < r) ? rows[w + tid] : 0;
   double myrhs = 0.0; int myperm = 0;
-  if(tid < w) { myrhs = use_aug ? L[(nrows - 1) + (size_t)tid*nrows] : ywork[c0 + tid]; myperm = perm[c0 + tid]; }
+  if(tid < w) { myrhs = use_aug ? L[(gbl + r) + (size_t)tid*ldg] : ywork[c0 + tid]; myperm = perm[c0 + tid]; }
   constexpr bool LEAN = BWD_NT == 256;
   constexpr int MV_SLOTS = LEAN ? 20 : 24;
   const int mv_cols = min(BWD_NT, max(w, 64)), mv_parts = BWD_NT/mv_cols;
@@ -151,7 +153,7 @@
   const int mv_i0 = mv_p*mv_len, mv_i1 = min(r, mv_i0 + mv_len);
   const bool mv_thread = mv_len <= MV_SLOTS && xb_lds;
   const bool mv_on = mv_thread && mv_j < w && mv_p < mv_parts;
-  const double* mv_L = L + (size_t)min(mv_j, w - 1)*nrows + w;
+  const double* mv_L = L + (size_t)min(mv_j, w - 1)*ldg + gbl;
   double mv[MV_SLOTS];
   {
     typedef double bw_v2d __attribute__((ext_vector_type(2)));
@@ -202,7 +204,7 @@
 #pragma unroll
     for(int a = 0; a < 8; a++)
 #pragma unroll
-      for(int b = 0; b <= a; b++) Lm[a][b] = (a < nbm) ? L[(m0 + a) + (size_t)(m0 + b)*nrows] : (a == b ? 1.0 : 0.0);
+      for(int b = 0; b <= a; b++) Lm[a][b] = (a < nbm) ? L[((hbm_c ? 0 : m0) + a) + (size_t)(m0 + b)*ldg] : (a == b ? 1.0 : 0.0);
     if(mm)
     {
 #pragma unroll
@@ -340,7 +342,7 @@
     for(int e = 256 + tid; e < mv_parts*256; e += BWD_NT) xp[e] = 0.0;
     for(int jg = 4*wv; jg < w; jg += 4*NW)
     {
-      const double* Lj = L + (size_t)jg*nrows + w;
+      const double* Lj = L + (size_t)jg*ldg + gbl;
       const int nc = min(4, w - jg);
       double acc[4] = {0.0, 0.0, 0.0, 0.0};
 #pragma unroll 2
@@ -348,7 +350,7 @@
       {
         const double x = xb_lds ? xb[i] : ldx(ywork + rows[w + i]);
 #pragma unroll
-        for(int c = 0; c < 4; c++) acc[c] += ((c < nc) ? Lj[i + (size_t)c*nrows] : 0.0)*x;
+        for(int c = 0; c < 4; c++) acc[c] += ((c < nc) ? Lj[i + (size_t)c*ldg] : 0.0)*x;
       }
 #pragma unroll
       for(int c = 0; c < 4; c++)
@@ -381,7 +383,7 @@
       if(tid < nmem)
         for(int a = nbm - 1; a >= 0; a--)
         {
-          const double* Lc = L + (size_t)(m0 + a)*nrows + m0;
+          const double* Lc = L + (size_t)(m0 + a)*ldg + (hbm_c ? 0 : m0);
           double v = xs[m0 + a];
           for(int b = a + 1; b < nbm; b++) v -= Lc[b]*xs[m0 + b];
           xs[m0 + a] = v/Lc[a];
@@ -644,10 +646,12 @@
       }
       if(pm > 0 && !getenv("DOGLEG_AMD_NO_PREMUL") && (long)Y->bwd_lds[l] + pm*8 <= LDS_BUDGET) Y->bwd_pmx[l] = (int)(pm*8);
     }
-    Y->bwd_nt[l] = (maxw <= 128 && H.lvl_ptr[l+1] - H.lvl_ptr[l] >= 512) ? 256 : 512;
+    Y->bwd_nt[l] = SymHost::bwd_level_lean(maxw, H.lvl_ptr[l+1] - H.lvl_ptr[l]) ? 256 : 512;
     bool allbd = true;
     for(int i = H.lvl_ptr[l]; i < H.lvl_ptr[l+1]; i++) { const int s = H.lvl_sn[i]; if(H.sn_bd_ptr[s+1] == H.sn_bd_ptr[s]) allbd = false; }
     Y->bwd_bd[l] = allbd ? 1 : 0;
+    if(l == 0 && H.leaf_compact && !(Y->bwd_nt[l] == 256 && allbd))
+    { dlg_set_error("internal error: compact leaf panels without the block-diagonal backward kernel"); return DLG_ERR_STATE; }
     if(Y->bwd_nt[l] != 512 || Y->bwd_bd[l]) Y->bwd_pmx[l] = 0;
     Y->bwd_lds[l] += Y->bwd_pmx[l];
   }
@@ -679,7 +683,7 @@
     for(int i = H.lvl_ptr[0]; i < H.lvl_ptr[1]; i++)
     {
       const int s = H.lvl_sn[i];
-      const int64_t a = H.sn_lx[s], e = a + (int64_t)(H.sn_rowptr[s+1] - H.sn_rowptr[s])*(H.sn_c0[s+1] - H.sn_c0[s]);
+      const int64_t a = H.sn_lx[s], e = a + (int64_t)H.lx_ld(s)*(H.sn_c0[s+1] - H.sn_c0[s]);
       if(lo < 0 || a < lo) lo = a;
       if(e > hi) hi = e;
     }
@@ -748,8 +752,9 @@
 {
   SparseSym* Y = b->sym;
   double* mm = bwd_diag_mm(b, l);
+  const int hbm_c = (Y->H.leaf_compact && l == 0 && !flag) ? 2 : 0;
 #define DLG_BW_LAUNCH(...) hipLaunchKernelGGL(HIP_KERNEL_NAME(k_solve_bwd_level<__VA_ARGS__>), dim3(grid), dim3(nt), lds, b->stream, \
-                                              items, Y->sn_rows, Y->perm, Y->Lx, Y->ywork, out, use_aug, Y->sn_bd_col, 256*l, Y->bwd_xb_cap, \
+                                              items, Y->sn_rows, Y->perm, Y->Lx, Y->ywork, out, use_aug, Y->sn_bd_col, 256*l + hbm_c, Y->bwd_xb_cap, \
                                               flag, epoch, Y->d_info, dlg_handoff(b, 1 << 21), xh, nxh, mm)
   if(nt == 256 && bd) DLG_BW_LAUNCH(256, true);
   else if(nt == 256) DLG_BW_LAUNCH(256, false);
@@ -766,13 +771,14 @@
   const int use_aug = (Y->aug_rhs != nullptr && Y->aug_rhs == rhs) ? 1 : 0;
   if(H.part_nranks > 1 && !use_aug)
   { dlg_set_error("with a subtree partition only the right-hand side that rode along with the factorisation (Jt x) can be solved for"); return DLG_ERR_STATE; }
+  if(!use_aug) DLG_CHECK(sparse_user_factor(b));
   for(int l = 0; l < H.nlevels && !use_aug; l++)
   {
     const int n = H.xl_ptr[l+1] - H.xl_ptr[l];
     if(n > 0)
       hipLaunchKernelGGL(k_solve_fwd_level, dim3(n), dim3(TPB), Y->slv_lds[l], st, Y->xl_sn + H.xl_ptr[l],
-                         Y->sn_c0, Y->sn_rowptr, Y->sn_lx, Y->sn_scr, Y->rl_ptr, Y->rl_pos, Y->perm,
-                         Y->Lx, rhs, Y->scr, Y->ywork);
+                         Y->sn_c0, Y->sn_rowptr, Y->sn_lx_u, Y->sn_scr, Y->rl_ptr, Y->rl_pos, Y->perm,
+                         Y->Lu, rhs, Y->scr, Y->ywork);
   }
   if(H.part_nranks > 1) DLG_HIP(hipMemsetAsync(out, 0, sizeof(double)*(size_t)H.N, st));
   int ltop = H.nlevels - 1;
diff --git a/libdogleg_amd/csrc/sparse_symbolic.cpp b/libdogleg_amd/csrc/sparse_symbolic.cpp
--- a/libdogleg_amd/csrc/sparse_symbolic.cpp
+++ b/libdogleg_amd/csrc/sparse_symbolic.cpp
@@ -1,4 +1,5 @@
 #include "sparse_symbolic.h"
+#include "sparse_region.h"
 #include <algorithm>
 #include <cstdio>
 #include <cstdlib>
@@ -228,8 +229,8 @@
 
 #define SYM_FAIL(...) do { snprintf(err, errlen, __VA_ARGS__); return 1; } while(0)
 
-int sym_analyze(SymHost& S, int N, int M, const int* cp, const int* ri, int row0, int row1,
-                char* err, int errlen, int part_rank, int part_nranks)
+static int sym_analyze_once(SymHost& S, int N, int M, const int* cp, const int* ri, int row0, int row1,
+                            char* err, int errlen, int part_rank, int part_nranks, bool compact_allowed)
 {
   const bool partition = part_nranks > 1;
   if(partition) { row0 = 0; row1 = M; }
@@ -765,6 +766,36 @@
     }
   }
 
+  S.sn_lx_cl = S.sn_lx; S.lx_size_cl = S.lx_size;
+  S.sn_ldc.assign(nsn, 0); S.sn_ldc_wd.assign(nsn, 0); S.leaf_compact = 0;
+  if(compact_allowed && !partition && row0 == 0 && row1 == M && S.nlevels >= 2)
+  {
+    bool ok = true;
+    for(int i = S.lvl_ptr[0]; i < S.lvl_ptr[1] && ok; i++)
+    {
+      const int s = S.lvl_sn[i], w = S.sn_c0[s+1] - S.sn_c0[s], nbd = S.sn_bd_ptr[s+1] - S.sn_bd_ptr[s];
+      if(nbd <= 0 || S.sn_top[s] >= 0 || w > 64 || w % nbd != 0 || w/nbd > 4) { ok = false; break; }
+      const int wd = w/nbd;
+      for(int m = 0; m < nbd; m++) if(S.sn_bd_col[S.sn_bd_ptr[s] + m] != m*wd) ok = false;
+    }
+    for(int s = 0; s < nsn && ok; s++) if(S.sn_level[s] > 0 && S.sn_bd_ptr[s+1] > S.sn_bd_ptr[s]) ok = false;
+    if(ok)
+    {
+      S.leaf_compact = 1;
+      for(int i = S.lvl_ptr[0]; i < S.lvl_ptr[1]; i++)
+      {
+        const int s = S.lvl_sn[i], w = S.sn_c0[s+1] - S.sn_c0[s], nrows = S.sn_rowptr[s+1] - S.sn_rowptr[s];
+        S.sn_ldc_wd[s] = w/(S.sn_bd_ptr[s+1] - S.sn_bd_ptr[s]);
+        S.sn_ldc[s] = (S.sn_ldc_wd[s] + (nrows - w) + 1) & ~1;
+      }
+      for(int s = 0; s < nsn; s++)
+        S.sn_lx[s+1] = S.sn_lx[s] + (int64_t)S.lx_ld(s)*(S.sn_c0[s+1] - S.sn_c0[s]);
+      S.lx_size = S.sn_lx[nsn];
+      for(int s = 0; s < nsn; s++)
+        for(int c = 0, w = S.sn_c0[s+1] - S.sn_c0[s]; c < w; c++) S.diagpos[S.sn_c0[s] + c] = S.lx_at(s, c, c);
+    }
+  }
+
   auto step8 = [&](char* err, int errlen) -> int {
   {
     struct Sub { int lvl, t, q, d, ka, rel; };
@@ -972,7 +1003,7 @@
       }
       const int nrows_d = S.sn_rowptr[u.d+1] - S.sn_rowptr[u.d];
       SymSub ss;
-      ss.src = S.sn_lx[u.d] + u.ka; ss.rel = u.rel; ss.nrows_d = nrows_d;
+      ss.src = S.sn_ldc[u.d] ? -1 : S.sn_lx[u.d] + u.ka; ss.rel = u.rel; ss.nrows_d = nrows_d;
       ss.wd = S.sn_c0[u.d+1] - S.sn_c0[u.d]; ss.m = nrows_d - u.ka;
       S.usub.push_back(ss);
       if(S.upd_syrk[u.lvl])
@@ -1051,10 +1082,10 @@
     for(int v = 0; v < nvb; v++)
     {
       const int q = bpos[v], t = sn_of_b[q];
-      const int ld = S.sn_rowptr[t+1] - S.sn_rowptr[t];
+      const int ld = S.lx_ld(t);
       const int lc = colstart[q] - S.sn_c0[t];
       SymOutBlock o; memset(&o, 0, sizeof(o));
-      o.dest = S.sn_lx[t] + lc + (int64_t)lc*ld; o.ld = ld; o.var0 = S.vb_start[v];
+      o.dest = S.lx_at(t, lc, lc); o.ld = ld; o.var0 = S.vb_start[v];
       o.nI = o.nJ = (uint8_t)G.w[v]; o.diag = 1;
       S.oblk[v] = o;
     }
@@ -1394,7 +1425,7 @@
         {
           if(fin_lists.empty())
           {
-            AsmFin2 F; F.dest = S.sn_lx[t] + lc + (int64_t)lc*ld; F.ld = ld; F.list0 = 0; F.nlist = 0;
+            AsmFin2 F; F.dest = S.lx_at(t, lc, lc); F.ld = ld; F.list0 = 0; F.nlist = 0;
             F.nI = F.nJ = (uint8_t)nJ; F.diag = 1; F.to_part = 0;
             S.asm_fin2.push_back(F); fin_lists.emplace_back();
           }
@@ -1416,7 +1447,7 @@
       const int r0 = rptr[J], r1 = rptr[J+1];
       if(r0 == r1 || (int)is_rider_blk[J] != pass) continue;
       const int qJ = bpos[J], t = sn_of_b[qJ];
-      const int ld = S.sn_rowptr[t+1] - S.sn_rowptr[t];
+      const int ld = S.lx_ld(t);
       const int lc = colstart[qJ] - S.sn_c0[t];
       const int nJ = G.w[J];
       slots.clear();
@@ -1429,12 +1460,13 @@
           if(bpos[I] < qJ || slot_stamp[I] == J) continue;
           slot_stamp[I] = J; slot_of[I] = (int)slots.size();
           int64_t dest;
-          if(I == J) dest = S.sn_lx[t] + lc + (int64_t)lc*ld;
+          if(I == J) dest = S.lx_at(t, lc, lc);
           else
           {
             const int ro = rowoff_in(t, bpos[I]);
             if(ro < 0) SYM_FAIL("internal error: JtJ block (%d,%d) missing from the factor structure", bpos[I], qJ);
-            dest = S.sn_lx[t] + ro + (int64_t)lc*ld;
+            dest = S.lx_at(t, ro, lc);
+            if(dest < 0) SYM_FAIL("internal error: JtJ block (%d,%d) couples two members of a merged leaf", bpos[I], qJ);
           }
           slots.push_back({I, dest, G.w[I], I == J ? 1 : 0});
         }
@@ -1685,3 +1717,23 @@
   SYM_TICK("done");
   return 0;
 }
+
+static bool sym_leaf_kernels_compact(const SymHost& S)
+{
+  FacLevels L;
+  char e[256];
+  if(fac_level_params(S, L, e, sizeof(e))) return false;
+  if(!(L.leaf[0] && L.nt[0] == 256 && L.syrk_fused[0] == 1 && 0 < S.mf_level0)) return false;
+  int maxw = 0;
+  for(int i = S.lvl_ptr[0]; i < S.lvl_ptr[1]; i++) maxw = std::max(maxw, S.sn_c0[S.lvl_sn[i]+1] - S.sn_c0[S.lvl_sn[i]]);
+  return SymHost::bwd_level_lean(maxw, S.lvl_ptr[1] - S.lvl_ptr[0]);
+}
+
+int sym_analyze(SymHost& S, int N, int M, const int* cp, const int* ri, int row0, int row1,
+                char* err, int errlen, int part_rank, int part_nranks, int leaf_compact)
+{
+  const bool want = leaf_compact < 0 ? env_int("DOGLEG_AMD_LEAF_COMPACT", 1) != 0 : leaf_compact != 0;
+  const int rc = sym_analyze_once(S, N, M, cp, ri, row0, row1, err, errlen, part_rank, part_nranks, want);
+  if(rc || !S.leaf_compact || sym_leaf_kernels_compact(S)) return rc;
+  return sym_analyze_once(S, N, M, cp, ri, row0, row1, err, errlen, part_rank, part_nranks, false);
+}
diff --git a/libdogleg_amd/csrc/sparse_symbolic.h b/libdogleg_amd/csrc/sparse_symbolic.h
--- a/libdogleg_amd/csrc/sparse_symbolic.h
+++ b/libdogleg_amd/csrc/sparse_symbolic.h
@@ -145,6 +145,20 @@
   std::vector<int>     sn_rowptr;
   std::vector<int>     sn_rows;
   std::vector<int64_t> sn_lx;
+  int leaf_compact = 0;
+  std::vector<int>     sn_ldc, sn_ldc_wd;
+  std::vector<int64_t> sn_lx_cl;
+  int64_t lx_size_cl = 0;
+  static bool bwd_level_lean(long maxw, long count) { return maxw <= 128 && count >= 512; }
+  int lx_ld(int s) const { return (!sn_ldc.empty() && sn_ldc[s]) ? sn_ldc[s] : sn_rowptr[s+1] - sn_rowptr[s]; }
+  int lx_row(int s, int i, int j) const
+  {
+    if(sn_ldc.empty() || !sn_ldc[s]) return i;
+    const int w = sn_c0[s+1] - sn_c0[s], wd = sn_ldc_wd[s], m0 = (j/wd)*wd;
+    if(i >= w) return wd + i - w;
+    return (i >= m0 && i < m0 + wd) ? i - m0 : -1;
+  }
+  int64_t lx_at(int s, int i, int j) const { const int r = lx_row(s, i, j); return r < 0 ? -1 : sn_lx[s] + r + (int64_t)j*lx_ld(s); }
   std::vector<int>     sn_scr;
   std::vector<int>     sn_level;
   int nlevels = 0;
@@ -215,4 +229,4 @@
 };
 
 int sym_analyze(SymHost& S, int N, int M, const int* colptr, const int* rowidx, int row0, int row1,
-                char* err, int errlen, int part_rank = 0, int part_nranks = 1);
+                char* err, int errlen, int part_rank = 0, int part_nranks = 1, int leaf_compact = -1);
```

After: 1827, median of 6. 1.2% higher.
